# LuZWCHA/MLIC

Hardware: AMD Instinct MI355X
Metric: images/sec (enc+dec) at 1920×1088 MLICPP_L, 1/2/4/8 GPU; bpp/PSNR Δ vs ref (higher is better)
Workload: dtype f32 (dense convs: f32 via split-fp16 MFMA, 3 terms); 1 GPU; config 2: MLICPP_L compress+decompress of 1920x1088 images (full rANS bitstreams, inputs resident in HBM); model=MLICPP_L, global_batch=32, per_gpu_images=32, weights=rate set(s) [1] of synthetic.RATE_LAMBDAS, parallelism=image-sharded x1 (no cross-GPU context), request_streams=4, schedule=each request stream runs its K steps back to back (no per-step join)

## Files before the change

### include/mlic_hip.h

```cpp
#ifndef MLIC_HIP_H
#define MLIC_HIP_H
#include <stddef.h>
#include <stdint.h>

#ifdef __cplusplus
extern "C" {
#endif

typedef struct mlic_model mlic_model;

const char* mlic_last_error(void);
const char* mlic_version(void);

int mlic_create(const char* model_name, int n, const char* const* names, const float* const* ptrs,
                const int64_t* shapes, const int* ndims, void* stream, mlic_model** out);
int mlic_destroy(mlic_model* m);

int mlic_forward(mlic_model* m, void* stream, const float* x, int B, int H, int W, float* x_hat, float* y_lik,
                 float* z_lik, float vbr_scale);
int mlic_forward_v(mlic_model* m, void* stream, const float* x, int B, int H, int W, float* x_hat, float* y_lik,
                   float* z_lik, const float* vbr_scales);

int mlic_set_entropy_tables(mlic_model* m, const int32_t* gc_cdf, const int32_t* gc_len, const int32_t* gc_off,
                            int gc_n, int gc_stride, const int32_t* eb_cdf, const int32_t* eb_len,
                            const int32_t* eb_off, int eb_n, int eb_stride);

int mlic_set_lanes(mlic_model* m, int lanes);
int mlic_set_priority_base(mlic_model* m, int base);
int mlic_compress(mlic_model* m, void* stream, const float* x, int B, int H, int W, float vbr_scale);
int mlic_compress_v(mlic_model* m, void* stream, const float* x, int B, int H, int W, const float* vbr_scales);
int mlic_encoded_size(mlic_model* m, int b, size_t* y_len, size_t* z_len);
int mlic_encoded_copy(mlic_model* m, int b, uint8_t* y, uint8_t* z);
int mlic_encoded_streams(mlic_model* m, int b, int64_t* n_y, int64_t* n_z, int32_t* y_sym, int32_t* y_idx,
                         int32_t* z_sym);
int mlic_encoded_bits(mlic_model* m, int b, double* y_bits, double* z_bits);
int mlic_batch_stream(mlic_model* m, int first, int count, uint8_t* out, size_t cap, size_t* len);
int mlic_decompress_batch_stream(mlic_model* m, void* stream, const uint8_t* y, size_t y_len, const uint8_t* const* z,
                                 const size_t* z_len, int B, int hz, int wz, float* x_hat, const float* vbr_scales);
int mlic_decompress(mlic_model* m, void* stream, const uint8_t* const* y, const size_t* y_len,
                    const uint8_t* const* z, const size_t* z_len, int B, int hz, int wz, float* x_hat,
                    float vbr_scale);
int mlic_decompress_v(mlic_model* m, void* stream, const uint8_t* const* y, const size_t* y_len,
                      const uint8_t* const* z, const size_t* z_len, int B, int hz, int wz, float* x_hat,
                      const float* vbr_scales);

int mlic_layer_streams(mlic_model* m, int b, const uint8_t** ptrs, size_t* lens, int cap, int* n);
int mlic_decompress_prefix(mlic_model* m, void* stream, const uint8_t* const* y, const size_t* y_len,
                           int strings_per_image, const uint8_t* const* z, const size_t* z_len, int B, int hz, int wz,
                           int slices, int fill, const float* vbr_scales, float* x_hat);

int mlic_forward_g(mlic_model* m, void* stream, const float* x, int B, int H, int W, float* x_hat, float* y_lik,
                   float* z_lik, const float* gain_plane);
int mlic_compress_g(mlic_model* m, void* stream, const float* x, int B, int H, int W, const float* gain_plane);
int mlic_decompress_g(mlic_model* m, void* stream, const uint8_t* const* y, const size_t* y_len,
                      const uint8_t* const* z, const size_t* z_len, int B, int hz, int wz, float* x_hat,
                      const float* gain_plane);
int mlic_image_roi_levels_u8(void* stream, const uint8_t* mask, const int64_t* mask_strides, int B, int H, int W, int lo,
                             int hi, uint8_t* levels);
int mlic_roi_gain_plane(void* stream, const uint8_t* levels, int B, int hz, int wz, const float* gains_host,
                        int n_levels, float* g);
int mlic_image_sq_err_roi_u8(void* stream, const uint8_t* a, const int64_t* a_strides, const uint8_t* b,
                             const int64_t* b_strides, const uint8_t* mask, const int64_t* mask_strides, int B, int H,
                             int W, uint64_t* out);

int mlic_rate_map_run(void* stream, const float* y_lik, int64_t y_bs, const float* z_lik, int64_t z_bs, int B, int M,
                      int S, int h, int w, int N, double* y_map, double* z_map, double* cell_bits, double* slice_bits);
int mlic_image_sq_err_blocks_u8(void* stream, const uint8_t* a, const int64_t* a_strides, const uint8_t* b,
                                const int64_t* b_strides, int B, int H, int W, int block, uint32_t* out);
int mlic_image_heat_u8(void* stream, const double* plane, int B, int ph, int pw, int cell, double lo, double hi,
                       int cmap, int H, int W, uint8_t* dst, const int64_t* dst_strides, const uint8_t* under,
                       const int64_t* under_strides, int alpha);

int mlic_run_module(mlic_model* m, void* stream, const char* which, int idx, const float* in0, const float* in1,
                    int B, int Cin, int H, int W, float* out);
int mlic_workspace_bytes(mlic_model* m, size_t* arena, size_t* weights);

int mlic_set_precision(mlic_model* m, int precision);
int mlic_set_synthesis_precision(mlic_model* m, int mode);
int mlic_set_poison(mlic_model* m, int on);
int mlic_set_kernel_option(const char* name, int value);
int mlic_get_kernel_option(const char* name, int* value);
int mlic_ab_families(int* built);
int mlic_range_fallbacks(mlic_model* m, int64_t* forward_full, int64_t* forward_gs, int64_t* decompress_gs,
                         int reset);
int mlic_set_profiling(mlic_model* m, int on);
int mlic_profile_read(mlic_model* m, int cat, int64_t* launches, double* ms, double* flops, double* bytes);
int mlic_profile_layers(mlic_model* m, char* buf, size_t cap, size_t* written);

int mlic_profile_categories(int* n);
int mlic_host_stats(mlic_model* m, double* enc_ms, double* dec_ms, double* wait_ms, int reset);
int mlic_profile_category_name(int cat, char* buf, size_t cap);

int mlic_conv_run(void* stream, int impl, const float* x, const float* w, const float* bias, float* y, int B, int Cin,
                  int Cout, int H, int W, int K, int stride, int epi, const float* aux, const float* res);
int mlic_conv_choice(int B, int Cin, int Cout, int H, int W, int K, int stride, int epi, int* impl);
int mlic_dw_run(void* stream, const float* x, const float* w, const float* bias, float* y, int B, int C, int H, int W,
                int stride, int gelu);
int mlic_dwpw_run(void* stream, const float* x, const float* dww, const float* dwb, const float* w, const float* bias,
                  float* y, int B, int C, int Cout, int H, int W, int epi, const float* res);
int mlic_bench_conv(int impl, int B, int Cin, int Cout, int H, int W, int K, int stride, int epi, int iters,
                    double* ms_per, double* tflops);
int mlic_local_attn_mask(void* stream, float* out, int H, int W);
int mlic_local_attn_run(void* stream, int impl, const float* qkv, const float* rel_table, const int32_t* rel_index,
                        float* out, int C, int H, int W, int B, float scale);
int mlic_local_attn_packed_run(void* stream, const float* qkv, const float* rel_table, const int32_t* rel_index,
                               uint16_t* out, int H, int W, int B, float scale);
int mlic_local_attn_packed_half_run(void* stream, const float* qkv, const float* rel_table, const int32_t* rel_index,
                                    uint16_t* out, int H, int W, int B, float scale, int ckbd);
int mlic_linatt_splits(int HW, int* nsplit);
int mlic_linear_attention_run(void* stream, const float* k, const float* v, const float* q, float* out, float* ctx_out,
                              int B, int heads, int hd, int H, int W, int nsplit, int kmask, int qmask);
int mlic_linatt_pack_run(void* stream, const float* q, const float* ctx, uint16_t* out_halves, int B, int heads, int hd,
                         int H, int W, int K, int qmask);
int mlic_ln_channels_run(void* stream, const float* x, const float* gamma, const float* beta, float* y, int B, int C,
                         int HW);
int mlic_taps_gather_run(void* stream, const float* part, const float* bias, float* out, int B, int H, int W);

typedef struct mlic_quant_desc {
  const float* y;
  int64_t y_bs;
  const float* params;
  int64_t params_bs;
  const float* params_a;
  int64_t params_a_bs;
  float* yh;
  int64_t yh_bs;
  float* lik;
  int64_t lik_bs;
  int32_t* sym;
  int32_t* idx;
  int16_t* sym16;
  uint8_t* idx8;
  int32_t* ovf;
  int32_t nlim;
  int32_t ntable;
  const float* table;
  int32_t phase;
  int32_t vbr;
  const float* sc;
  const float* rs;
  const float* scp;
  const float* rsp;
  int32_t B, C, H, W;
} mlic_quant_desc;
int mlic_quant_phase_run(void* stream, const mlic_quant_desc* d);
int mlic_phase_indexes_run(void* stream, const mlic_quant_desc* d);
int mlic_phase_dequant_run(void* stream, const mlic_quant_desc* d);
int mlic_phase_fill_run(void* stream, const mlic_quant_desc* d);
int mlic_recip_plane_run(void* stream, const float* g, float* r, int64_t n);
int mlic_eb_forward_run(void* stream, const float* z, float* z_hat, float* lik, int32_t* sym, const float* quantiles,
                        const float* m0, const float* m1, const float* m2, const float* m3, const float* m4,
                        const float* b0, const float* b1, const float* b2, const float* b3, const float* b4,
                        const float* f0, const float* f1, const float* f2, const float* f3, int B, int C, int H,
                        int W);
int mlic_eb_dequant_run(void* stream, const int32_t* sym, const float* quantiles, float* z_hat, int B, int C, int H,
                        int W);
int mlic_ckbd_mask_run(void* stream, const float* x, int64_t x_bs, float* y, int64_t y_bs, int B, int C, int H, int W,
                       int keep_anchor);
int mlic_image_sq_err_u8(void* stream, const float* a, const float* b, int B, int64_t n_per, double* out);
int mlic_ms_ssim_scratch_bytes(int B, int C, int H, int W, size_t* bytes);
int mlic_image_ms_ssim_u8(void* stream, const float* a, const int64_t* a_strides, const float* b,
                          const int64_t* b_strides, int B, int C, int H, int W, void* scratch,
                          size_t scratch_bytes, double* out, double* terms);

typedef struct mlic_lpips mlic_lpips;
int mlic_lpips_create(int n, const char* const* names, const float* const* ptrs, const int64_t* shapes,
                      const int* ndims, void* stream, mlic_lpips** out);
int mlic_lpips_destroy(mlic_lpips* h);
int mlic_lpips_set_precision(mlic_lpips* h, int precision);
int mlic_lpips_scratch_bytes(int B, int H, int W, size_t* bytes);
int mlic_image_lpips_u8(mlic_lpips* h, void* stream, const float* a, const int64_t* a_strides, const float* b,
                        const int64_t* b_strides, int B, int H, int W, void* scratch, size_t scratch_bytes,
                        double* out, double* terms);
int mlic_lpips_profile(mlic_lpips* h, int on, double* ms3);
int mlic_lpips_range_fallbacks(mlic_lpips* h, int64_t* count, int reset);

typedef struct mlic_dists mlic_dists;
int mlic_dists_create(int n, const char* const* names, const float* const* ptrs, const int64_t* shapes,
                      const int* ndims, void* stream, mlic_dists** out);
int mlic_dists_destroy(mlic_dists* h);
int mlic_dists_set_precision(mlic_dists* h, int precision);
int mlic_dists_scratch_bytes(int B, int H, int W, size_t* bytes);
int mlic_image_dists_u8(mlic_dists* h, void* stream, const float* a, const int64_t* a_strides, const float* b,
                        const int64_t* b_strides, int B, int H, int W, void* scratch, size_t scratch_bytes,
                        double* out, double* terms);
int mlic_dists_profile(mlic_dists* h, int on, double* ms3);
int mlic_dists_range_fallbacks(mlic_dists* h, int64_t* count, int reset);

int mlic_image_ingest_u8(void* stream, const uint8_t* src, const int64_t* src_strides, int B, int H, int W, float* dst,
                         int Hp, int Wp);
int mlic_image_egress_u8(void* stream, const float* src, const int64_t* src_strides, int B, int H, int W, uint8_t* dst,
                         const int64_t* dst_strides, const uint8_t* ref, const int64_t* ref_strides, uint64_t* sq_err);
int mlic_image_blur3_pad(void* stream, const float* src, const int32_t* src_index, int n, int H, int W, int Hp, int Wp,
                         const float* w9, float* dst);

typedef struct mlic_container_info {
  uint32_t H, W;
  uint32_t hz, wz;
  int32_t level;
  int32_t reserved;
  uint64_t y_off, y_len;
  uint64_t z_off, z_len;
} mlic_container_info;
int mlic_container_bytes(size_t y_len, size_t z_len, int vbr, size_t* bytes);
int mlic_container_write(uint32_t H, uint32_t W, int level, uint32_t hz, uint32_t wz, const uint8_t* y, size_t y_len,
                         const uint8_t* z, size_t z_len, uint8_t* out, size_t cap, size_t* len);
int mlic_container_parse(const uint8_t* data, size_t n, int vbr, int n_levels, uint64_t max_pixels,
                         mlic_container_info* info);

typedef struct mlic_container_roi_info {
  mlic_container_info file;
  uint64_t map_off, map_len;
} mlic_container_roi_info;
int mlic_container_write_roi(uint32_t H, uint32_t W, int level, uint32_t hz, uint32_t wz, const uint8_t* y,
                             size_t y_len, const uint8_t* z, size_t z_len, const uint8_t* levels, uint8_t* out,
                             size_t cap, size_t* len);
int mlic_container_parse_roi(const uint8_t* data, size_t n, int n_levels, uint64_t max_pixels,
                             mlic_container_roi_info* info, uint8_t* levels, size_t levels_cap);

int mlic_tile_grid(uint32_t H, uint32_t W, uint32_t T, uint32_t V, uint32_t* ny, uint32_t* nx, uint32_t* rects,
                   size_t rects_cap);
int mlic_image_tile_blend_u8(void* stream, const float* const* tiles_dev, const float* const* tiles_host, int H, int W,
                             int T, int V, int y0, int x0, int h, int w, uint8_t* dst, const int64_t* dst_strides,
                             const uint8_t* ref, const int64_t* ref_strides, uint64_t* sq_err);
typedef struct mlic_container_tiled_info {
  uint32_t H, W, T, V, ny, nx;
  int32_t vbr;
  int32_t reserved;
  uint64_t table_off, payload_off, payload_len;
} mlic_container_tiled_info;
int mlic_container_write_tiled(uint32_t H, uint32_t W, uint32_t T, uint32_t V, int vbr, const uint8_t* payload,
                               const uint64_t* lens, size_t n_tiles, uint8_t* out, size_t cap, size_t* len);
int mlic_container_parse_tiled(const uint8_t* data, size_t n, uint64_t max_pixels, mlic_container_tiled_info* info);
int mlic_container_tiled_tile(const uint8_t* data, size_t n, const mlic_container_tiled_info* info, uint64_t k,
                              uint64_t* off, uint64_t* len);

int mlic_encode_image_u8(mlic_model* m, void* stream, const uint8_t* rgb_dev, const int64_t* strides, int H, int W,
                         float vbr_scale, int level, uint8_t* out, size_t cap, size_t* len);
int mlic_encode_image_u8_budget(mlic_model* m, void* stream, const uint8_t* rgb_dev, const int64_t* strides, int H,
                                int W, float vbr_scale, int level, double max_bpp, int max_passes, uint8_t* out,
                                size_t cap, size_t* len, int* passes);
int mlic_decode_image_u8(mlic_model* m, void* stream, const uint8_t* file, size_t n, int n_levels, uint64_t max_pixels,
                         const float* vbr_gains, uint8_t* rgb_dev, const int64_t* strides, size_t cap_bytes, int* H,
                         int* W, int* level);

int mlic_resample_table(int filter, int Li, int Lo, int32_t* start, int32_t* count, float* weights, int stride,
                        int* taps);
int mlic_image_ingest_u8_scaled(void* stream, const uint8_t* src, const int64_t* src_strides, int B, int Hi, int Wi,
                                int filter, int h, int w, float* dst, int Hp, int Wp);
int mlic_image_egress_u8_scaled(void* stream, const float* src, const int64_t* src_strides, int B, int h, int w,
                                int filter, int Ho, int Wo, uint8_t* dst, const int64_t* dst_strides, const uint8_t* ref,
                                const int64_t* ref_strides, uint64_t* sq_err);
typedef struct mlic_container_scaled_info {
  uint32_t H, W;
  int32_t filter;
  int32_t vbr;
  uint64_t inner_off, inner_len;
  mlic_container_info inner;
} mlic_container_scaled_info;
int mlic_container_write_scaled(uint32_t H, uint32_t W, int vbr, int filter, const uint8_t* inner, size_t inner_len,
                                uint8_t* out, size_t cap, size_t* len);
int mlic_container_parse_scaled(const uint8_t* data, size_t n, int n_levels, uint64_t max_pixels,
                                mlic_container_scaled_info* info);
typedef struct mlic_container_layered_info {
  uint32_t H, W, hz, wz;
  int32_t level;
  uint32_t S, layers_present;
  uint64_t z_off, z_len;
  uint64_t layer_off[32], layer_len[32];
} mlic_container_layered_info;
int mlic_container_layered_bytes(size_t z_len, const size_t* layer_lens, int S, int vbr, size_t* bytes);
int mlic_container_write_layered(uint32_t H, uint32_t W, int level, uint32_t hz, uint32_t wz, const uint8_t* z,
                                 size_t z_len, const uint8_t* const* layers, const size_t* layer_lens, int S,
                                 uint8_t* out, size_t cap, size_t* len);
int mlic_container_parse_layered(const uint8_t* data, size_t n, int n_levels, uint64_t max_pixels, int allow_truncated,
                                 mlic_container_layered_info* info);
int mlic_encode_image_u8_scaled(mlic_model* m, void* stream, const uint8_t* rgb_dev, const int64_t* strides, int H,
                                int W, int coded_H, int coded_W, int filter, float vbr_scale, int level, uint8_t* out,
                                size_t cap, size_t* len);
int mlic_decode_image_u8_sized(mlic_model* m, void* stream, const uint8_t* file, size_t n, int n_levels,
                               uint64_t max_pixels, const float* vbr_gains, int out_H, int out_W, int filter,
                               uint8_t* rgb_dev, const int64_t* strides, size_t cap_bytes, int* H, int* W, int* level,
                               int* coded_H, int* coded_W);

typedef struct mlic_yuv_desc {
  int32_t sub_x, sub_y;
  int32_t matrix;
  int32_t full_range;
  int32_t site_x;
  int32_t reserved[3];
} mlic_yuv_desc;
int mlic_image_ingest_yuv8(void* stream, const uint8_t* y, const int64_t* y_strides, const uint8_t* cb,
                           const int64_t* cb_strides, const uint8_t* cr, const int64_t* cr_strides,
                           const mlic_yuv_desc* desc, int B, int H, int W, float* dst, int Hp, int Wp);
int mlic_image_egress_yuv8(void* stream, const float* src, const int64_t* src_strides, int B, int H, int W,
                           const mlic_yuv_desc* desc, uint8_t* y, const int64_t* y_strides, uint8_t* cb,
                           const int64_t* cb_strides, uint8_t* cr, const int64_t* cr_strides, const uint8_t* ref_y,
                           const int64_t* ref_y_strides, const uint8_t* ref_cb, const int64_t* ref_cb_strides,
                           const uint8_t* ref_cr, const int64_t* ref_cr_strides, uint64_t* sq_err);
int mlic_encode_image_yuv8(mlic_model* m, void* stream, const uint8_t* y_dev, const int64_t* y_strides,
                           const uint8_t* cb_dev, const int64_t* cb_strides, const uint8_t* cr_dev,
                           const int64_t* cr_strides, const mlic_yuv_desc* desc, int H, int W, float vbr_scale,
                           int level, uint8_t* out, size_t cap, size_t* len);
int mlic_decode_image_yuv8(mlic_model* m, void* stream, const uint8_t* file, size_t n, int n_levels,
                           uint64_t max_pixels, const float* vbr_gains, const mlic_yuv_desc* desc, uint8_t* y_dev,
                           const int64_t* y_strides, size_t y_cap, uint8_t* cb_dev, const int64_t* cb_strides,
                           size_t cb_cap, uint8_t* cr_dev, const int64_t* cr_strides, size_t cr_cap, int* H, int* W,
                           int* level);

int mlic_image_ingest_u16(void* stream, const uint16_t* src, const int64_t* src_strides, int depth, int msb, int B,
                          int H, int W, float* dst, int Hp, int Wp);
int mlic_image_egress_u16(void* stream, const float* src, const int64_t* src_strides, int B, int H, int W, int depth,
                          int msb, uint16_t* dst, const int64_t* dst_strides, const uint16_t* ref,
                          const int64_t* ref_strides, uint64_t* sq_err);
int mlic_image_ingest_yuv16(void* stream, const uint16_t* y, const int64_t* y_strides, const uint16_t* cb,
                            const int64_t* cb_strides, const uint16_t* cr, const int64_t* cr_strides,
                            const mlic_yuv_desc* desc, int depth, int msb, int B, int H, int W, float* dst, int Hp,
                            int Wp);
int mlic_image_egress_yuv16(void* stream, const float* src, const int64_t* src_strides, int B, int H, int W,
                            const mlic_yuv_desc* desc, int depth, int msb, uint16_t* y, const int64_t* y_strides,
                            uint16_t* cb, const int64_t* cb_strides, uint16_t* cr, const int64_t* cr_strides,
                            const uint16_t* ref_y, const int64_t* ref_y_strides, const uint16_t* ref_cb,
                            const int64_t* ref_cb_strides, const uint16_t* ref_cr, const int64_t* ref_cr_strides,
                            uint64_t* sq_err);
int mlic_encode_image_yuv16(mlic_model* m, void* stream, const uint16_t* y_dev, const int64_t* y_strides,
                            const uint16_t* cb_dev, const int64_t* cb_strides, const uint16_t* cr_dev,
                            const int64_t* cr_strides, const mlic_yuv_desc* desc, int depth, int msb, int H, int W,
                            float vbr_scale, int level, uint8_t* out, size_t cap, size_t* len);
int mlic_decode_image_yuv16(mlic_model* m, void* stream, const uint8_t* file, size_t n, int n_levels,
                            uint64_t max_pixels, const float* vbr_gains, const mlic_yuv_desc* desc, int depth, int msb,
                            uint16_t* y_dev, const int64_t* y_strides, size_t y_cap, uint16_t* cb_dev,
                            const int64_t* cb_strides, size_t cb_cap, uint16_t* cr_dev, const int64_t* cr_strides,
                            size_t cr_cap, int* H, int* W, int* level);
int mlic_neglog2_sum(void* stream, const float* lik, int B, int64_t n_per, double* out);
int mlic_gaussian_likelihood(void* stream, const float* y, const float* scales, const float* means, int64_t n,
                             float vbr_scale, float* lik);
int mlic_scale_indexes(void* stream, const float* scales, int64_t n, const float* table, int ntable, int32_t* out);

int mlic_pmf_to_quantized_cdf(const float* pmf, int n, int precision, int32_t* cdf_out );
int mlic_rans_encode(const int32_t* symbols, const int32_t* indexes, int64_t n, const int32_t* cdf,
                     const int32_t* cdf_len, const int32_t* offset, int n_tables, int stride, uint8_t* out,
                     size_t cap, size_t* written);
int mlic_rans_decode(const uint8_t* data, size_t nbytes, const int32_t* indexes, int64_t n, const int32_t* cdf,
                     const int32_t* cdf_len, const int32_t* offset, int n_tables, int stride, int32_t* out);
int mlic_rans_decode_narrow(const uint8_t* data, size_t nbytes, const uint8_t* indexes, int64_t n, int nparts,
                            const int32_t* cdf, const int32_t* cdf_len, const int32_t* offset, int n_tables,
                            int stride, int32_t* out, int* widened);

#ifdef __cplusplus
}
#endif
#endif
```

### mlic_amd/_lib.py

```python
from __future__ import annotations

import ctypes as C
import os
import threading

_HERE = os.path.dirname(os.path.abspath(__file__))
LIB_PATH = os.environ.get("MLIC_HIP_LIB", os.path.join(_HERE, "libmlic_hip.so"))

_lock = threading.Lock()
_lib = None


class MlicError(RuntimeError):
    pass


class ContainerInfo(C.Structure):
    _fields_ = [("H", C.c_uint32), ("W", C.c_uint32), ("hz", C.c_uint32), ("wz", C.c_uint32), ("level", C.c_int32),
                ("reserved", C.c_int32), ("y_off", C.c_uint64), ("y_len", C.c_uint64), ("z_off", C.c_uint64),
                ("z_len", C.c_uint64)]


class ContainerRoiInfo(C.Structure):
    _fields_ = [("file", ContainerInfo), ("map_off", C.c_uint64), ("map_len", C.c_uint64)]


class ContainerTiledInfo(C.Structure):
    _fields_ = [("H", C.c_uint32), ("W", C.c_uint32), ("T", C.c_uint32), ("V", C.c_uint32), ("ny", C.c_uint32),
                ("nx", C.c_uint32), ("vbr", C.c_int32), ("reserved", C.c_int32), ("table_off", C.c_uint64),
                ("payload_off", C.c_uint64), ("payload_len", C.c_uint64)]


class ContainerScaledInfo(C.Structure):
    _fields_ = [("H", C.c_uint32), ("W", C.c_uint32), ("filter", C.c_int32), ("vbr", C.c_int32),
                ("inner_off", C.c_uint64), ("inner_len", C.c_uint64), ("inner", ContainerInfo)]


class ContainerLayeredInfo(C.Structure):
    _fields_ = [("H", C.c_uint32), ("W", C.c_uint32), ("hz", C.c_uint32), ("wz", C.c_uint32), ("level", C.c_int32),
                ("S", C.c_uint32), ("layers_present", C.c_uint32), ("z_off", C.c_uint64), ("z_len", C.c_uint64),
                ("layer_off", C.c_uint64 * 32), ("layer_len", C.c_uint64 * 32)]


class YuvDesc(C.Structure):
    _fields_ = [("sub_x", C.c_int32), ("sub_y", C.c_int32), ("matrix", C.c_int32), ("full_range", C.c_int32),
                ("site_x", C.c_int32), ("reserved", C.c_int32 * 3)]


class QuantDesc(C.Structure):
    _fields_ = [("y", C.c_void_p), ("y_bs", C.c_int64), ("params", C.c_void_p), ("params_bs", C.c_int64),
                ("params_a", C.c_void_p), ("params_a_bs", C.c_int64), ("yh", C.c_void_p), ("yh_bs", C.c_int64),
                ("lik", C.c_void_p), ("lik_bs", C.c_int64), ("sym", C.c_void_p), ("idx", C.c_void_p),
                ("sym16", C.c_void_p), ("idx8", C.c_void_p), ("ovf", C.c_void_p), ("nlim", C.c_int32),
                ("ntable", C.c_int32), ("table", C.c_void_p), ("phase", C.c_int32), ("vbr", C.c_int32),
                ("sc", C.c_void_p), ("rs", C.c_void_p), ("scp", C.c_void_p), ("rsp", C.c_void_p),
                ("B", C.c_int32), ("C", C.c_int32), ("H", C.c_int32), ("W", C.c_int32)]


def _sig(lib):
    p, i, i64, f, sz = C.c_void_p, C.c_int, C.c_int64, C.c_float, C.c_size_t
    P = C.POINTER
    lib.mlic_last_error.restype = C.c_char_p
    lib.mlic_version.restype = C.c_char_p
    sigs = {
        "mlic_create": [C.c_char_p, i, P(C.c_char_p), P(p), P(i64), P(i), p, P(p)],
        "mlic_destroy": [p],
        "mlic_forward": [p, p, p, i, i, i, p, p, p, f],
        "mlic_forward_v": [p, p, p, i, i, i, p, p, p, p],
        "mlic_compress_v": [p, p, p, i, i, i, p],
        "mlic_decompress_v": [p, p, P(p), P(sz), P(p), P(sz), i, i, i, p, p],
        "mlic_set_entropy_tables": [p, p, p, p, i, i, p, p, p, i, i],
        "mlic_compress": [p, p, p, i, i, i, f],
        "mlic_encoded_size": [p, i, P(sz), P(sz)],
        "mlic_encoded_copy": [p, i, p, p],
        "mlic_encoded_streams": [p, i, P(i64), P(i64), p, p, p],
        "mlic_decompress": [p, p, P(p), P(sz), P(p), P(sz), i, i, i, p, f],
        "mlic_run_module": [p, p, C.c_char_p, i, p, p, i, i, i, i, p],
        "mlic_workspace_bytes": [p, P(sz), P(sz)],
        "mlic_local_attn_mask": [p, p, i, i],
        "mlic_set_profiling": [p, i],
        "mlic_set_lanes": [p, i],
        "mlic_set_priority_base": [p, i],
        "mlic_set_precision": [p, i],
        "mlic_set_synthesis_precision": [p, i],
        "mlic_set_poison": [p, i],
        "mlic_set_kernel_option": [C.c_char_p, i],
        "mlic_get_kernel_option": [C.c_char_p, P(i)],
        "mlic_ab_families": [P(i)],
        "mlic_batch_stream": [p, i, i, p, sz, P(sz)],
        "mlic_decompress_batch_stream": [p, p, p, sz, P(p), P(sz), i, i, i, p, p],
        "mlic_range_fallbacks": [p, P(i64), P(i64), P(i64), i],
        "mlic_profile_layers": [p, p, sz, P(sz)],
        "mlic_bench_conv": [i, i, i, i, i, i, i, i, i, i, P(C.c_double), P(C.c_double)],
        "mlic_profile_read": [p, i, P(i64), P(C.c_double), P(C.c_double), P(C.c_double)],
        "mlic_profile_categories": [P(i)],
        "mlic_host_stats": [p, P(C.c_double), P(C.c_double), P(C.c_double), i],
        "mlic_profile_category_name": [i, p, sz],
        "mlic_conv_run": [p, i, p, p, p, p, i, i, i, i, i, i, i, i, p, p],
        "mlic_conv_choice": [i, i, i, i, i, i, i, i, P(i)],
        "mlic_dw_run": [p, p, p, p, p, i, i, i, i, i, i],
        "mlic_dwpw_run": [p, p, p, p, p, p, p, i, i, i, i, i, i, p],
        "mlic_local_attn_run": [p, i, p, p, p, p, i, i, i, i, f],
        "mlic_local_attn_packed_run": [p, p, p, p, p, i, i, i, f],
        "mlic_local_attn_packed_half_run": [p, p, p, p, p, i, i, i, f, i],
        "mlic_linatt_splits": [i, P(i)],
        "mlic_linear_attention_run": [p, p, p, p, p, p, i, i, i, i, i, i, i, i],
        "mlic_linatt_pack_run": [p, p, p, p, i, i, i, i, i, i, i],
        "mlic_ln_channels_run": [p, p, p, p, p, i, i, i],
        "mlic_taps_gather_run": [p, p, p, p, i, i, i],
        "mlic_quant_phase_run": [p, P(QuantDesc)],
        "mlic_phase_indexes_run": [p, P(QuantDesc)],
        "mlic_phase_dequant_run": [p, P(QuantDesc)],
        "mlic_phase_fill_run": [p, P(QuantDesc)],
        "mlic_layer_streams": [p, i, P(p), P(sz), i, P(i)],
        "mlic_decompress_prefix": [p, p, P(p), P(sz), i, P(p), P(sz), i, i, i, i, i, p, p],
        "mlic_container_layered_bytes": [sz, P(sz), i, i, P(sz)],
        "mlic_container_write_layered": [C.c_uint32, C.c_uint32, i, C.c_uint32, C.c_uint32, p, sz, P(p), P(sz), i, p,
                                         sz, P(sz)],
        "mlic_container_parse_layered": [p, sz, i, C.c_uint64, i, P(ContainerLayeredInfo)],
        "mlic_recip_plane_run": [p, p, p, i64],
        "mlic_eb_forward_run": [p] * 20 + [i, i, i, i],
        "mlic_eb_dequant_run": [p, p, p, p, i, i, i, i],
        "mlic_ckbd_mask_run": [p, p, i64, p, i64, i, i, i, i, i],
        "mlic_image_sq_err_u8": [p, p, p, i, i64, p],
        "mlic_ms_ssim_scratch_bytes": [i, i, i, i, P(sz)],
        "mlic_image_ms_ssim_u8": [p, p, P(i64), p, P(i64), i, i, i, i, p, sz, p, p],
        "mlic_lpips_create": [i, P(C.c_char_p), P(p), P(i64), P(i), p, P(p)],
        "mlic_lpips_destroy": [p],
        "mlic_lpips_set_precision": [p, i],
        "mlic_lpips_scratch_bytes": [i, i, i, P(sz)],
        "mlic_image_lpips_u8": [p, p, p, P(i64), p, P(i64), i, i, i, p, sz, p, p],
        "mlic_lpips_range_fallbacks": [p, P(i64), i],
        "mlic_lpips_profile": [p, i, P(C.c_double)],
        "mlic_dists_create": [i, P(C.c_char_p), P(p), P(i64), P(i), p, P(p)],
        "mlic_dists_destroy": [p],
        "mlic_dists_set_precision": [p, i],
        "mlic_dists_scratch_bytes": [i, i, i, P(sz)],
        "mlic_image_dists_u8": [p, p, p, P(i64), p, P(i64), i, i, i, p, sz, p, p],
        "mlic_dists_range_fallbacks": [p, P(i64), i],
        "mlic_dists_profile": [p, i, P(C.c_double)],
        "mlic_image_ingest_u8": [p, p, P(i64), i, i, i, p, i, i],
        "mlic_image_egress_u8": [p, p, P(i64), i, i, i, p, P(i64), p, P(i64), p],
        "mlic_image_blur3_pad": [p, p, p, i, i, i, i, i, p, p],
        "mlic_container_bytes": [sz, sz, i, P(sz)],
        "mlic_container_write": [C.c_uint32, C.c_uint32, i, C.c_uint32, C.c_uint32, p, sz, p, sz, p, sz, P(sz)],
        "mlic_container_parse": [p, sz, i, i, C.c_uint64, P(ContainerInfo)],
        "mlic_forward_g": [p, p, p, i, i, i, p, p, p, p],
        "mlic_compress_g": [p, p, p, i, i, i, p],
        "mlic_decompress_g": [p, p, P(p), P(sz), P(p), P(sz), i, i, i, p, p],
        "mlic_image_roi_levels_u8": [p, p, P(i64), i, i, i, i, i, p],
        "mlic_roi_gain_plane": [p, p, i, i, i, P(f), i, p],
        "mlic_image_sq_err_roi_u8": [p, p, P(i64), p, P(i64), p, P(i64), i, i, i, p],
        "mlic_rate_map_run": [p, p, i64, p, i64, i, i, i, i, i, i, p, p, p, p],
        "mlic_image_sq_err_blocks_u8": [p, p, P(i64), p, P(i64), i, i, i, i, p],
        "mlic_image_heat_u8": [p, p, i, i, i, i, C.c_double, C.c_double, i, i, i, p, P(i64), p, P(i64), i],
        "mlic_container_write_roi": [C.c_uint32, C.c_uint32, i, C.c_uint32, C.c_uint32, p, sz, p, sz, p, p, sz, P(sz)],
        "mlic_container_parse_roi": [p, sz, i, C.c_uint64, P(ContainerRoiInfo), p, sz],
        "mlic_tile_grid": [C.c_uint32, C.c_uint32, C.c_uint32, C.c_uint32, P(C.c_uint32), P(C.c_uint32), p, sz],
        "mlic_image_tile_blend_u8": [p, p, p, i, i, i, i, i, i, i, i, p, P(i64), p, P(i64), p],
        "mlic_container_write_tiled": [C.c_uint32, C.c_uint32, C.c_uint32, C.c_uint32, i, p, p, sz, p, sz, P(sz)],
        "mlic_container_parse_tiled": [p, sz, C.c_uint64, P(ContainerTiledInfo)],
        "mlic_container_tiled_tile": [p, sz, P(ContainerTiledInfo), C.c_uint64, P(C.c_uint64), P(C.c_uint64)],
        "mlic_encode_image_u8": [p, p, p, P(i64), i, i, f, i, p, sz, P(sz)],
        "mlic_encode_image_u8_budget": [p, p, p, P(i64), i, i, f, i, C.c_double, i, p, sz, P(sz), P(i)],
        "mlic_decode_image_u8": [p, p, p, sz, i, C.c_uint64, p, p, P(i64), sz, P(i), P(i), P(i)],
        "mlic_resample_table": [i, i, i, p, p, p, i, P(i)],
        "mlic_image_ingest_u8_scaled": [p, p, P(i64), i, i, i, i, i, i, p, i, i],
        "mlic_image_egress_u8_scaled": [p, p, P(i64), i, i, i, i, i, i, p, P(i64), p, P(i64), p],
        "mlic_container_write_scaled": [C.c_uint32, C.c_uint32, i, i, p, sz, p, sz, P(sz)],
        "mlic_container_parse_scaled": [p, sz, i, C.c_uint64, P(ContainerScaledInfo)],
        "mlic_encode_image_u8_scaled": [p, p, p, P(i64), i, i, i, i, i, f, i, p, sz, P(sz)],
        "mlic_decode_image_u8_sized": [p, p, p, sz, i, C.c_uint64, p, i, i, i, p, P(i64), sz, P(i), P(i), P(i), P(i),
                                       P(i)],
        "mlic_image_ingest_yuv8": [p, p, P(i64), p, P(i64), p, P(i64), P(YuvDesc), i, i, i, p, i, i],
        "mlic_image_egress_yuv8": [p, p, P(i64), i, i, i, P(YuvDesc), p, P(i64), p, P(i64), p, P(i64), p, P(i64), p,
                                   P(i64), p, P(i64), p],
        "mlic_encode_image_yuv8": [p, p, p, P(i64), p, P(i64), p, P(i64), P(YuvDesc), i, i, f, i, p, sz, P(sz)],
        "mlic_decode_image_yuv8": [p, p, p, sz, i, C.c_uint64, p, P(YuvDesc), p, P(i64), sz, p, P(i64), sz, p, P(i64),
                                   sz, P(i), P(i), P(i)],
        "mlic_image_ingest_u16": [p, p, P(i64), i, i, i, i, i, p, i, i],
        "mlic_image_egress_u16": [p, p, P(i64), i, i, i, i, i, p, P(i64), p, P(i64), p],
        "mlic_image_ingest_yuv16": [p, p, P(i64), p, P(i64), p, P(i64), P(YuvDesc), i, i, i, i, i, p, i, i],
        "mlic_image_egress_yuv16": [p, p, P(i64), i, i, i, P(YuvDesc), i, i, p, P(i64), p, P(i64), p, P(i64), p,
                                    P(i64), p, P(i64), p, P(i64), p],
        "mlic_encode_image_yuv16": [p, p, p, P(i64), p, P(i64), p, P(i64), P(YuvDesc), i, i, i, i, f, i, p, sz, P(sz)],
        "mlic_decode_image_yuv16": [p, p, p, sz, i, C.c_uint64, p, P(YuvDesc), i, i, p, P(i64), sz, p, P(i64), sz, p,
                                    P(i64), sz, P(i), P(i), P(i)],
        "mlic_neglog2_sum": [p, p, i, i64, p],
        "mlic_gaussian_likelihood": [p, p, p, p, i64, f, p],
        "mlic_scale_indexes": [p, p, i64, p, i, p],
        "mlic_encoded_bits": [p, i, P(C.c_double), P(C.c_double)],
        "mlic_pmf_to_quantized_cdf": [p, i, i, p],
        "mlic_rans_encode": [p, p, i64, p, p, p, i, i, p, sz, P(sz)],
        "mlic_rans_decode": [p, sz, p, i64, p, p, p, i, i, p],
        "mlic_rans_decode_narrow": [p, sz, p, i64, i, p, p, p, i, i, p, P(i)],
    }
    for name, args in sigs.items():
        fn = getattr(lib, name)
        fn.argtypes = args
        fn.restype = C.c_int
    return lib


def _check_build_record():
    import json
    from . import build as _build
    if os.environ.get("MLIC_HIP_LIB"):
        return
    rec_path = _build.RECORD
    if not os.path.exists(rec_path):
        raise MlicError(f"{rec_path} missing: rebuild with `python -m mlic_amd.build` (records the sources the "
                        f"library was built from)")
    with open(rec_path) as f:
        rec = json.load(f)
    if rec.get("sources_sha256") != _build.source_digest():
        raise MlicError("libmlic_hip.so was built from other sources than the ones in this tree (stale build): "
                        "rebuild with `python -m mlic_amd.build`")


def lib():
    global _lib
    with _lock:
        if _lib is None:
            if not os.path.exists(LIB_PATH):
                raise MlicError(f"libmlic_hip.so not found at {LIB_PATH}: build it with "
                                f"`python -c 'import __graft_entry__ as g; g.build()'` (hipcc, gfx950)")
            _check_build_record()
            _lib = _sig(C.CDLL(LIB_PATH))
    return _lib


def poison() -> bool:
    return os.environ.get("MLIC_POISON", "0") not in ("", "0")


def ab_families() -> bool:
    v = C.c_int()
    call("mlic_ab_families", C.byref(v))
    return bool(v.value)


def check(rc: int, what: str = ""):
    if rc != 0:
        msg = lib().mlic_last_error().decode(errors="replace")
        raise MlicError(f"{what}: {msg}" if what else msg)


def call(name: str, *args):
    check(getattr(lib(), name)(*args), name)
```

### mlic_amd/csrc/capi.cpp

```cpp
#include "../../include/mlic_hip.h"

#include <algorithm>
#include <cmath>
#include <cstring>
#include <string>
#include <vector>

#include "container.h"
#include "model.h"
#include "options.h"
#include "resample_table.h"

using namespace mlic;

struct mlic_model {
  Model* impl;
  float* stage = nullptr;
  size_t stage_bytes = 0;
  float* stage2 = nullptr;
  size_t stage2_bytes = 0;
  int enc_H = 0, enc_W = 0, enc_level = -1;
  int enc_passes = 0;
  int sc_H = 0, sc_W = 0, sc_filter = 0;
};
// ... 368 lines not shown
    *value = opt_get(name);
  });
}

int mlic_set_poison(mlic_model* m, int on) {
  return guard([&] { impl(m).set_poison(on != 0); });
}

int mlic_range_fallbacks(mlic_model* m, int64_t* forward_full, int64_t* forward_gs, int64_t* decompress_gs,
                         int reset) {
  return guard([&] {
    Model::Fallbacks& f = impl(m).fallbacks();
    if (forward_full) *forward_full = f.forward_full.load();
    if (forward_gs) *forward_gs = f.forward_gs.load();
    if (decompress_gs) *decompress_gs = f.decompress_gs.load();
    if (reset) {
      f.forward_full = 0;
      f.forward_gs = 0;
      f.decompress_gs = 0;
    }
  });
}

int mlic_set_synthesis_precision(mlic_model* m, int mode) {
  return guard([&] {
    MLIC_CHECK(mode == 0 || mode == 1, "synthesis precision must be 0 (fp32-faithful) or 1 (fp16 operands)");
    impl(m).set_synthesis_precision(mode);
  });
}

int mlic_set_lanes(mlic_model* m, int lanes) {
  return guard([&] { impl(m).set_lanes(lanes); });
}

int mlic_set_priority_base(mlic_model* m, int base) {
  return guard([&] {
    MLIC_CHECK(base >= 0, "priority base must be >= 0");
    impl(m).set_priority_base(base);
  });
}

int mlic_set_profiling(mlic_model* m, int on) {
  return guard([&] { impl(m).set_profiling(on != 0); });
}

int mlic_profile_read(mlic_model* m, int cat, int64_t* launches, double* ms, double* flops, double* bytes) {
  return guard([&] {
    MLIC_CHECK(cat >= 0 && cat < PCAT_COUNT, "profile category");
    ProfStat s = impl(m).profile_read(cat);
    *launches = s.launches;
    *ms = s.ms;
    *flops = s.flops;
    *bytes = s.bytes;
  });
}

int mlic_profile_layers(mlic_model* m, char* buf, size_t cap, size_t* written) {
  return guard([&] {
    std::string s = impl(m).profile_layers();
    *written = s.size();
    if (buf && cap) {
      const size_t n = std::min(cap - 1, s.size());
      std::memcpy(buf, s.data(), n);
      buf[n] = 0;
    }
  });
}

int mlic_bench_conv(int impl, int B, int Cin, int Cout, int H, int W, int K, int stride, int epi, int iters,
                    double* ms_per, double* tflops) {
  return guard([&] {
    const int pad = K / 2;
    const int Ho = (H + 2 * pad - K) / stride + 1, Wo = (W + 2 * pad - K) / stride + 1;
    const int64_t nx = (int64_t)B * Cin * H * W, ny = (int64_t)B * Cout * Ho * Wo, nw = (int64_t)Cout * Cin * K * K;
    const int cin_pad = (Cin + 31) / 32 * 32;
    const int64_t nh = (int64_t)Cout * K * K * cin_pad;
    float *x, *y, *w, *wp, *bias;
    _Float16 *wh, *wl;
    HIP_OK(hipMalloc(&x, nx * 4));
    HIP_OK(hipMalloc(&y, ny * 4));
    HIP_OK(hipMalloc(&w, nw * 4));
    HIP_OK(hipMalloc(&wp, nw * 4));
    HIP_OK(hipMalloc(&bias, Cout * 4));
    HIP_OK(hipMalloc(&wh, nh * 2));
    HIP_OK(hipMalloc(&wl, nh * 2));
    {
      std::vector<float> hx(std::max(nx, nw));
      uint32_t st = 12345;
      for (auto& v : hx) { st = st * 1664525u + 1013904223u; v = ((st >> 9) * (1.0f / 8388608.0f)) - 0.5f; }
      HIP_OK(hipMemcpy(x, hx.data(), nx * 4, hipMemcpyHostToDevice));
      HIP_OK(hipMemcpy(w, hx.data(), nw * 4, hipMemcpyHostToDevice));
      HIP_OK(hipMemset(bias, 0, Cout * 4));
    }
    pack_conv(w, wp, Cout, Cin, K * K, nullptr);
    const int wexp = split_weights(w, wh, wl, Cout, Cin, K * K, cin_pad, true, nullptr);
    ConvParams P{};
    P.nseg = 1;
    P.seg[0] = {x, Cin, (int64_t)Cin * H * W};
    P.Cin = Cin; P.H = H; P.W = W; P.Cout = Cout; P.Ho = Ho; P.Wo = Wo; P.K = K; P.stride = stride; P.pad = pad;
    P.wpk = wp; P.bias = bias; P.out = y; P.B = B;
    P.out_bs = (int64_t)Cout * Ho * Wo;
    P.out_cs = (int64_t)Ho * Wo;
    P.epi = epi;
    MLIC_CHECK(!(epi & (EPI_GDN | EPI_IGDN | EPI_SHUFFLE)) || !(epi & EPI_RES), "bench: unsupported epilogue");
    if (epi & (EPI_GDN | EPI_IGDN)) {
      MLIC_CHECK(Cin == Cout && stride == 1, "bench: GDN needs Cin == Cout");
      P.aux = x;
      P.aux_bs = (int64_t)Cin * H * W;
    }
    if (epi & EPI_RES) {
      P.res = y;
      P.res_bs = P.out_bs;
    }
    _Float16 *wx = nullptr, *wxh = nullptr;
    if (conv_x4_ok(P, cin_pad)) {
      HIP_OK(hipMalloc((void**)&wx, x4_weight_halves(Cout, K * K, cin_pad) * 2));
      x4_pack_weights(wh, wl, Cout, K * K, cin_pad, wx, nullptr);
      if (impl == CONV_X4H) {
        HIP_OK(hipMalloc((void**)&wxh, x4_weight_halves(Cout, K * K, cin_pad, true) * 2));
        x4_pack_weights(wh, wl, Cout, K * K, cin_pad, wxh, nullptr, true);
      }
    }
    ConvWeights cw{wp, wh, wl, cin_pad, wx, wexp};
    cw.wx4h = wxh;
    const int which = impl < 0 ? conv_select(P, cw, 2) : impl;
    if (which == CONV_X4H) MLIC_CHECK(conv_x4_ok(P, cin_pad), "x4: unsupported shape");
    if (which == CONV_PW) MLIC_CHECK(pw_resident_ok(P, cin_pad), "pw_resident: unsupported shape");
    if (which == CONV_X4) MLIC_CHECK(conv_x4_ok(P, cin_pad), "x4: unsupported shape");
    void* ws = nullptr;
    const int64_t wsb = conv_ws_bytes(which, P, cw);
    if (wsb > 0) HIP_OK(hipMalloc(&ws, wsb));
    auto launch = [&] { conv_run(which, P, cw, nullptr, ws); };
    launch();
    HIP_OK(hipDeviceSynchronize());
    hipEvent_t a, b;
    HIP_OK(hipEventCreate(&a));
    HIP_OK(hipEventCreate(&b));
    HIP_OK(hipEventRecord(a, nullptr));
    for (int i = 0; i < iters; ++i) launch();
    HIP_OK(hipEventRecord(b, nullptr));
    HIP_OK(hipEventSynchronize(b));
    float ms = 0;
    HIP_OK(hipEventElapsedTime(&ms, a, b));
    *ms_per = ms / iters;
    *tflops = 2.0 * (double)B * Cout * Ho * Wo * Cin * K * K / (*ms_per * 1e-3) / 1e12;
    (void)hipEventDestroy(a);
    (void)hipEventDestroy(b);
    for (void* p : {(void*)x, (void*)y, (void*)w, (void*)wp, (void*)bias, (void*)wh, (void*)wl, (void*)wx, (void*)wxh, ws})
      if (p) (void)hipFree(p);
  });
}

int mlic_host_stats(mlic_model* m, double* enc_ms, double* dec_ms, double* wait_ms, int reset) {
  return guard([&] {
    HostStats& h = impl(m).host_stats();
    *enc_ms = h.enc_ns.load() * 1e-6;
    *dec_ms = h.dec_ns.load() * 1e-6;
    *wait_ms = h.wait_ns.load() * 1e-6;
    if (reset) {
      h.enc_ns = 0;
      h.dec_ns = 0;
      h.wait_ns = 0;
    }
  });
}

int mlic_profile_categories(int* n) {
  return guard([&] { *n = PCAT_COUNT; });
}

int mlic_profile_category_name(int cat, char* buf, size_t cap) {
  return guard([&] {
    MLIC_CHECK(cat >= 0 && cat < PCAT_COUNT, "profile category");
    const std::string nm = prof_cat_name(cat);
    MLIC_CHECK(cap > nm.size(), "buffer too small");
    std::memcpy(buf, nm.c_str(), nm.size() + 1);
  });
}

int mlic_conv_choice(int B, int Cin, int Cout, int H, int W, int K, int stride, int epi, int* impl) {
  return guard([&] {
    MLIC_CHECK(impl && B > 0 && Cin > 0 && Cout > 0 && H > 0 && W > 0 && (K == 1 || K == 3 || K == 5) && stride > 0,
               "conv_choice: bad arguments");
    const int pad = K / 2;
    ConvParams P{};
    P.nseg = 1;
    P.seg[0] = {nullptr, Cin, (int64_t)Cin * H * W};
    P.Cin = Cin; P.H = H; P.W = W; P.Cout = Cout; P.K = K; P.stride = stride; P.pad = pad;
    P.Ho = (H + 2 * pad - K) / stride + 1;
    P.Wo = (W + 2 * pad - K) / stride + 1;
    P.B = B;
    P.epi = epi;
    const int cin_pad = (Cin + 31) / 32 * 32;
    static const _Float16 tag = 0;
    const bool split = Cin >= 16;
    const bool x4 = split && Cout >= 64;
    const ConvWeights cw{nullptr, split ? &tag : nullptr, split ? &tag : nullptr, cin_pad, x4 ? &tag : nullptr, 0};
    *impl = conv_select(P, cw, 2);
  });
}

int mlic_conv_run(void* stream, int impl, const float* x, const float* w, const float* bias, float* y, int B, int Cin,
                  int Cout, int H, int W, int K, int stride, int epi, const float* aux, const float* res) {
  return guard([&] {
    hipStream_t st = (hipStream_t)stream;
    const int pad = K / 2;
    const int Ho = (H + 2 * pad - K) / stride + 1, Wo = (W + 2 * pad - K) / stride + 1;
    const int cin_pad = (Cin + 31) / 32 * 32;
    const int64_t nw = (int64_t)Cout * Cin * K * K, nh = (int64_t)Cout * K * K * cin_pad;
    float* wp = nullptr;
    _Float16 *wh = nullptr, *wl = nullptr;
    HIP_OK(hipMallocAsync((void**)&wp, nw * 4, st));
    HIP_OK(hipMallocAsync((void**)&wh, nh * 2, st));
    HIP_OK(hipMallocAsync((void**)&wl, nh * 2, st));
    pack_conv(w, wp, Cout, Cin, K * K, st);
    const int wexp = split_weights(w, wh, wl, Cout, Cin, K * K, cin_pad, true, st);
    ConvParams P{};
    P.nseg = 1;
    P.seg[0] = {x, Cin, (int64_t)Cin * H * W};
    P.Cin = Cin; P.H = H; P.W = W; P.Cout = Cout; P.Ho = Ho; P.Wo = Wo; P.K = K; P.stride = stride; P.pad = pad;
    P.wpk = wp; P.bias = bias; P.out = y; P.B = B; P.epi = epi;
    const bool shuffle = (epi & EPI_SHUFFLE) != 0;
    MLIC_CHECK(!shuffle || Cout % 4 == 0, "shuffle needs Cout % 4 == 0");
    P.out_cs = shuffle ? (int64_t)4 * Ho * Wo : (int64_t)Ho * Wo;
    P.out_bs = (int64_t)Cout * Ho * Wo;
    MLIC_CHECK(!(epi & (EPI_GDN | EPI_IGDN)) || aux, "GDN epilogue needs aux");
    MLIC_CHECK(!(epi & EPI_RES) || res, "residual epilogue needs res");
    P.aux = aux; P.aux_bs = (int64_t)Cout * Ho * Wo;
    P.res = res; P.res_bs = P.out_bs;
    _Float16 *wx = nullptr, *wxh = nullptr;
    if (conv_x4_ok(P, cin_pad)) {
      HIP_OK(hipMallocAsync((void**)&wx, x4_weight_halves(Cout, K * K, cin_pad) * 2, st));
      x4_pack_weights(wh, wl, Cout, K * K, cin_pad, wx, st);
      if (impl == CONV_X4H) {
        HIP_OK(hipMallocAsync((void**)&wxh, x4_weight_halves(Cout, K * K, cin_pad, true) * 2, st));
        x4_pack_weights(wh, wl, Cout, K * K, cin_pad, wxh, st, true);
      }
    }
    ConvWeights cw{wp, wh, wl, cin_pad, wx, wexp};
    cw.wx4h = wxh;
    const int which = impl < 0 ? conv_select(P, cw, 2) : impl;
    if (which == CONV_X4H) MLIC_CHECK(conv_x4_ok(P, cin_pad), "x4: unsupported shape");
    if (which == CONV_PW) MLIC_CHECK(pw_resident_ok(P, cin_pad), "pw_resident: unsupported shape");
    if (which == CONV_NARROW) MLIC_CHECK(conv_narrow_ok(P), "narrow: unsupported shape");
    if (which == CONV_SMALLCIN) MLIC_CHECK(conv_smallcin_ok(P), "smallcin: unsupported shape");
    if (which == CONV_HALO) MLIC_CHECK(conv_halo_ok(P, cin_pad), "halo: unsupported shape");
    if (which == CONV_X4) MLIC_CHECK(conv_x4_ok(P, cin_pad), "x4: unsupported shape");
    void* ws = nullptr;
    const int64_t wsb = conv_ws_bytes(which, P, cw);
    if (wsb > 0) HIP_OK(hipMallocAsync(&ws, wsb, st));
    conv_run(which, P, cw, st, ws);
    if (ws) HIP_OK(hipFreeAsync(ws, st));
    if (wx) HIP_OK(hipFreeAsync(wx, st));
    if (wxh) HIP_OK(hipFreeAsync(wxh, st));
    HIP_OK(hipFreeAsync(wp, st));
    HIP_OK(hipFreeAsync(wh, st));
    HIP_OK(hipFreeAsync(wl, st));
    HIP_OK(hipStreamSynchronize(st));
  });
}

int mlic_dw_run(void* stream, const float* x, const float* w, const float* bias, float* y, int B, int C, int H, int W,
                int stride, int gelu) {
  return guard([&] {
    DwParams P{};
    P.nseg = 1;
    P.seg[0] = {x, C, (int64_t)C * H * W};
    P.C = C; P.H = H; P.W = W; P.stride = stride;
    P.Ho = (H - 1) / stride + 1;
    P.Wo = (W - 1) / stride + 1;
    P.w = w; P.bias = bias; P.out = y; P.out_bs = (int64_t)C * P.Ho * P.Wo; P.gelu = gelu; P.B = B;
    dw3x3(P, (hipStream_t)stream);
    HIP_OK(hipStreamSynchronize((hipStream_t)stream));
  });
}

int mlic_dwpw_run(void* stream, const float* x, const float* dww, const float* dwb, const float* w, const float* bias,
                  float* y, int B, int C, int Cout, int H, int W, int epi, const float* res) {
  return guard([&] {
    hipStream_t st = (hipStream_t)stream;
    const int cin_pad = (C + 31) / 32 * 32;
    const int64_t nh = (int64_t)Cout * cin_pad;
    _Float16 *wh = nullptr, *wl = nullptr;
    HIP_OK(hipMallocAsync((void**)&wh, nh * 2, st));
    HIP_OK(hipMallocAsync((void**)&wl, nh * 2, st));
    const int wexp = split_weights(w, wh, wl, Cout, C, 1, cin_pad, true, st);
    ConvParams P{};
    P.nseg = 1;
    P.seg[0] = {x, C, (int64_t)C * H * W};
    P.Cin = C; P.H = H; P.W = W; P.Cout = Cout; P.Ho = H; P.Wo = W; P.K = 1; P.stride = 1; P.pad = 0;
    P.wexp = wexp; P.bias = bias; P.out = y; P.B = B; P.epi = epi;
    P.out_cs = (int64_t)H * W;
    P.out_bs = (int64_t)Cout * H * W;
    MLIC_CHECK(!(epi & EPI_RES) || res, "residual epilogue needs res");
    P.res = res; P.res_bs = P.out_bs;
    MLIC_CHECK(dwpw_ok(P, cin_pad), "dwpw: unsupported shape");
    dwpw_forward(P, wh, wl, cin_pad, dww, dwb, st);
    HIP_OK(hipFreeAsync(wh, st));
    HIP_OK(hipFreeAsync(wl, st));
    HIP_OK(hipStreamSynchronize(st));
  });
}

int mlic_local_attn_run(void* stream, int impl, const float* qkv, const float* rel_table, const int32_t* rel_index,
                        float* out, int C, int H, int W, int B, float scale) {
  return guard([&] {
    LocalAttnParams A{};
    A.qkv = qkv;
    A.qkv_bs = (int64_t)3 * C * H * W;
    A.out = out;
    A.out_bs = (int64_t)25 * C * H * W;
    A.rel_table = rel_table;
    A.rel_index = rel_index;
    A.scale = scale;
    A.C = C; A.H = H; A.W = W; A.B = B;
    if (impl == 0) local_attn_valu(A, (hipStream_t)stream);
    else local_attn_mfma(A, (hipStream_t)stream);
    HIP_OK(hipStreamSynchronize((hipStream_t)stream));
  });
}

int mlic_local_attn_packed_run(void* stream, const float* qkv, const float* rel_table, const int32_t* rel_index,
                               uint16_t* out, int H, int W, int B, float scale) {
  return guard([&] {
    LocalAttnParams A{};
    A.qkv = qkv;
    A.qkv_bs = (int64_t)3 * 32 * H * W;
    A.rel_table = rel_table;
    A.rel_index = rel_index;
    A.scale = scale;
    A.C = 32; A.H = H; A.W = W; A.B = B;
    local_attn_packed(A, reinterpret_cast<_Float16*>(out), (H * W + 31) / 32 * 32, (hipStream_t)stream);
    HIP_OK(hipStreamSynchronize((hipStream_t)stream));
  });
}

int mlic_local_attn_packed_half_run(void* stream, const float* qkv, const float* rel_table, const int32_t* rel_index,
                                    uint16_t* out, int H, int W, int B, float scale, int ckbd) {
  return guard([&] {
    MLIC_CHECK(ckbd == 1 || ckbd == 2, "ckbd: 1 (anchors) or 2 (non-anchors)");
    LocalAttnParams A{};
    A.qkv = qkv;
    A.qkv_bs = (int64_t)3 * 32 * H * W;
    A.rel_table = rel_table;
    A.rel_index = rel_index;
    A.scale = scale;
    A.C = 32; A.H = H; A.W = W; A.B = B;
    A.ckbd = ckbd;
    local_attn_packed(A, reinterpret_cast<_Float16*>(out), (H * W / 2 + 31) / 32 * 32, (hipStream_t)stream);
    HIP_OK(hipStreamSynchronize((hipStream_t)stream));
  });
}

static void check_grid(int B, int H, int W, int rows) {
  MLIC_CHECK(B >= 1 && B <= 65535, "B must be in 1..65535");
  MLIC_CHECK(H >= 1 && W >= 1 && (int64_t)H * W <= (int64_t)1 << 30, "H, W must be >= 1 and H * W <= 2^30");
  MLIC_CHECK(rows >= 1 && (int64_t)rows * B <= 65535, "too many (image, head) rows for one launch");
}

int mlic_linatt_splits(int HW, int* nsplit) {
  return guard([&] {
    MLIC_CHECK(nsplit != nullptr, "null nsplit");
    MLIC_CHECK(HW >= 1, "HW must be >= 1");
    *nsplit = ctx_splits(HW);
  });
}

int mlic_linear_attention_run(void* stream, const float* k, const float* v, const float* q, float* out, float* ctx_out,
                              int B, int heads, int hd, int H, int W, int nsplit, int kmask, int qmask) {
  return guard([&] {
    MLIC_CHECK(k && v && q && out, "null tensor");
    MLIC_CHECK(hd == 16 || hd == 32, "hd must be 16 or 32");
    MLIC_CHECK(heads >= 1, "heads must be >= 1");
    check_grid(B, H, W, heads);
    MLIC_CHECK(nsplit <= 64, "nsplit must be <= 64 (<= 0: the model's choice)");
    MLIC_CHECK((kmask == 0 || kmask == 1) && (qmask == 0 || qmask == 1), "kmask, qmask must be 0 or 1");
    hipStream_t st = (hipStream_t)stream;
    const int HW = H * W;
    const int ns = nsplit <= 0 ? ctx_splits(HW) : nsplit;
    const int64_t bs = (int64_t)heads * hd * HW, nctx = (int64_t)B * heads * hd * hd;
    float *part = nullptr, *ctx = nullptr;
    HIP_OK(hipMallocAsync((void**)&part, linear_attention_part_floats(heads, hd, B, ns) * 4, st));
    HIP_OK(hipMallocAsync((void**)&ctx, nctx * 4, st));
    linear_attention(k, bs, v, bs, q, bs, out, bs, part, ctx, heads, hd, H, W, B, ns, kmask, qmask, st);
    if (ctx_out) HIP_OK(hipMemcpyAsync(ctx_out, ctx, nctx * 4, hipMemcpyDeviceToDevice, st));
    HIP_OK(hipFreeAsync(part, st));
    HIP_OK(hipFreeAsync(ctx, st));
    HIP_OK(hipStreamSynchronize(st));
  });
}

int mlic_linatt_pack_run(void* stream, const float* q, const float* ctx, uint16_t* out_halves, int B, int heads, int hd,
                         int H, int W, int K, int qmask) {
  return guard([&] {
    MLIC_CHECK(q && ctx && out_halves, "null tensor");
    MLIC_CHECK(hd == 16 || hd == 32, "hd must be 16 or 32");
    MLIC_CHECK(heads >= 1 && (heads * (int64_t)hd) % 32 == 0, "heads * hd must be a multiple of 32");
    MLIC_CHECK(K == 3 || K == 5, "K must be 3 or 5");
    check_grid(B, H, W, heads * hd / 32);
    check_grid(B, H + K - 1, W + K - 1, 1);
    MLIC_CHECK(qmask == 0 || qmask == 1, "qmask must be 0 or 1");
    ConvParams P{};
    P.nseg = 1;
    P.seg[0] = {nullptr, heads * hd, (int64_t)heads * hd * H * W};
    P.Cin = heads * hd; P.H = H; P.W = W; P.Cout = P.Cin; P.Ho = H; P.Wo = W; P.K = K; P.stride = 1; P.pad = K / 2;
    P.B = B;
    P.rflag = nullptr;
    linatt_pack(q, P.seg[0].bs, ctx, heads, hd, qmask, P, reinterpret_cast<_Float16*>(out_halves), (hipStream_t)stream);
    HIP_OK(hipStreamSynchronize((hipStream_t)stream));
  });
}

int mlic_ln_channels_run(void* stream, const float* x, const float* gamma, const float* beta, float* y, int B, int C,
                         int HW) {
  return guard([&] {
    MLIC_CHECK(x && gamma && beta && y, "null tensor");
    MLIC_CHECK(C == 32 || C == 64 || C == 128, "C must be 32, 64 or 128");
    check_grid(B, 1, HW, 1);
    ln_channels(x, (int64_t)C * HW, y, (int64_t)C * HW, gamma, beta, C, HW, B, (hipStream_t)stream);
    HIP_OK(hipStreamSynchronize((hipStream_t)stream));
  });
}

int mlic_taps_gather_run(void* stream, const float* part, const float* bias, float* out, int B, int H, int W) {
  return guard([&] {
    MLIC_CHECK(part && out, "null tensor");
    check_grid(B, H, W, 1);
    MLIC_CHECK((H + 3) / 4 <= 65535, "H too large for one launch");
    taps_gather(part, (int64_t)108 * H * W, bias, out, (int64_t)12 * H * W, H, W, B, (hipStream_t)stream);
    HIP_OK(hipStreamSynchronize((hipStream_t)stream));
  });
}

static QuantParams quant_params(const mlic_quant_desc* d) {
  MLIC_CHECK(d != nullptr, "null descriptor");
  MLIC_CHECK(d->params && d->table, "null tensor");
  check_grid(d->B, d->H, d->W, 1);
  MLIC_CHECK(d->C >= 1 && (int64_t)d->C * d->H * d->W <= (int64_t)1 << 30, "C must be >= 1 and C * H * W <= 2^30");
  MLIC_CHECK(d->W % 2 == 0, "W must be even");
  MLIC_CHECK(d->phase == 0 || d->phase == 1, "phase must be 0 (anchor) or 1 (non-anchor)");
  MLIC_CHECK(d->ntable >= 2 && d->ntable <= 256, "ntable must be in 2..256");
  MLIC_CHECK(d->vbr == 0 || d->vbr == 1, "vbr must be 0 or 1");
  MLIC_CHECK(d->vbr || (!d->scp && !d->rsp), "gain planes need vbr");
  const int64_t n = (int64_t)d->C * d->H * d->W;
  MLIC_CHECK(d->params_bs >= 2 * n, "params_bs smaller than [2C][H][W]");
  QuantParams Q{};
  Q.y = d->y; Q.y_bs = d->y_bs;
  Q.params = d->params; Q.params_bs = d->params_bs;
  Q.params_a = d->params_a; Q.params_a_bs = d->params_a_bs;
  Q.yh = d->yh; Q.yh_bs = d->yh_bs;
  Q.lik = d->lik; Q.lik_bs = d->lik_bs;
  Q.sym = d->sym; Q.idx = d->idx;
  Q.sym16 = d->sym16; Q.idx8 = d->idx8; Q.ovf = d->ovf;
  Q.nlim = d->nlim;
  Q.table = d->table; Q.ntable = d->ntable;
  Q.phase = d->phase; Q.vbr = d->vbr;
  Q.sc = d->sc; Q.rs = d->rs;
  Q.C = d->C; Q.H = d->H; Q.W = d->W; Q.B = d->B;
  Q.scp = d->scp; Q.rsp = d->rsp;
  return Q;
}

int mlic_quant_phase_run(void* stream, const mlic_quant_desc* d) {
  return guard([&] {
    const QuantParams Q = quant_params(d);
    const int64_t n = (int64_t)Q.C * Q.H * Q.W;
    MLIC_CHECK(Q.y && Q.yh, "null tensor");
    MLIC_CHECK(Q.y_bs >= n, "y_bs smaller than [C][H][W]");
    MLIC_CHECK(Q.yh_bs >= n, "yh_bs smaller than [C][H][W]");
    MLIC_CHECK(!Q.lik || Q.params_a, "lik needs params_a");
    MLIC_CHECK(!Q.lik || Q.lik_bs >= n, "lik_bs smaller than [C][H][W]");
    MLIC_CHECK(!Q.params_a || Q.params_a_bs >= 2 * n, "params_a_bs smaller than [2C][H][W]");
    MLIC_CHECK(!Q.sym16 || (Q.idx8 && Q.ovf), "sym16 needs idx8 and ovf");
    MLIC_CHECK(Q.sym16 || (!Q.idx8 && !Q.ovf), "idx8 and ovf need sym16");
    MLIC_CHECK(!Q.idx || Q.sym || Q.sym16, "idx needs sym or sym16");
    MLIC_CHECK((Q.scp != nullptr) == (Q.rsp != nullptr), "scp and rsp: both or neither");
    MLIC_CHECK(!Q.vbr || Q.scp || (Q.sc && Q.rs), "vbr needs sc and rs, or gain planes");
    MLIC_CHECK(Q.nlim >= 1 && Q.nlim <= 32767, "nlim must be in 1..32767");
    quant_phase(Q, (hipStream_t)stream);
    HIP_OK(hipStreamSynchronize((hipStream_t)stream));
  });
}

int mlic_phase_indexes_run(void* stream, const mlic_quant_desc* d) {
  return guard([&] {
    const QuantParams Q = quant_params(d);
    MLIC_CHECK(Q.idx8 || Q.idx, "null output: idx8 or idx");
    MLIC_CHECK(!Q.vbr || Q.scp || Q.sc, "vbr needs sc, or the gain plane scp");
    phase_indexes(Q, (hipStream_t)stream);
    HIP_OK(hipStreamSynchronize((hipStream_t)stream));
  });
}

int mlic_phase_dequant_run(void* stream, const mlic_quant_desc* d) {
  return guard([&] {
    const QuantParams Q = quant_params(d);
    const int64_t n = (int64_t)Q.C * Q.H * Q.W;
    MLIC_CHECK(Q.yh, "null tensor");
    MLIC_CHECK(Q.yh_bs >= n, "yh_bs smaller than [C][H][W]");
    MLIC_CHECK(Q.sym16 || Q.sym, "null input: sym16 or sym");
    MLIC_CHECK(!Q.vbr || Q.rsp || Q.rs, "vbr needs rs, or the reciprocal plane rsp");
    phase_dequant(Q, (hipStream_t)stream);
    HIP_OK(hipStreamSynchronize((hipStream_t)stream));
  });
}

int mlic_phase_fill_run(void* stream, const mlic_quant_desc* d) {
  return guard([&] {
    const QuantParams Q = quant_params(d);
    const int64_t n = (int64_t)Q.C * Q.H * Q.W;
    MLIC_CHECK(Q.yh, "null tensor");
    MLIC_CHECK(Q.yh_bs >= n, "yh_bs smaller than [C][H][W]");
    phase_fill(Q, (hipStream_t)stream);
    HIP_OK(hipStreamSynchronize((hipStream_t)stream));
  });
}

int mlic_recip_plane_run(void* stream, const float* g, float* r, int64_t n) {
  return guard([&] {
    MLIC_CHECK(g && r, "null tensor");
    MLIC_CHECK(n >= 1 && n <= (int64_t)1 << 31, "n must be in 1..2^31");
    recip_plane(g, r, n, (hipStream_t)stream);
    HIP_OK(hipStreamSynchronize((hipStream_t)stream));
  });
}

static void check_eb_grid(int B, int C, int H, int W) {
  check_grid(B, H, W, 1);
  MLIC_CHECK(C >= 1 && (int64_t)B * C * H * W <= (int64_t)1 << 31, "C must be >= 1 and B * C * H * W <= 2^31");
}

int mlic_eb_forward_run(void* stream, const float* z, float* z_hat, float* lik, int32_t* sym, const float* quantiles,
                        const float* m0, const float* m1, const float* m2, const float* m3, const float* m4,
                        const float* b0, const float* b1, const float* b2, const float* b3, const float* b4,
                        const float* f0, const float* f1, const float* f2, const float* f3, int B, int C, int H,
                        int W) {
  return guard([&] {
    MLIC_CHECK(z && quantiles, "null tensor");
    MLIC_CHECK(m0 && m1 && m2 && m3 && m4 && b0 && b1 && b2 && b3 && b4 && f0 && f1 && f2 && f3, "null parameter");
    MLIC_CHECK(z_hat || lik || sym, "null outputs: at least one of z_hat, lik, sym");
    check_eb_grid(B, C, H, W);
    EbParams P{};
    P.z = z; P.z_hat = z_hat; P.lik = lik; P.sym = sym;
    P.quantiles = quantiles;
    P.m0 = m0; P.m1 = m1; P.m2 = m2; P.m3 = m3; P.m4 = m4;
    P.b0 = b0; P.b1 = b1; P.b2 = b2; P.b3 = b3; P.b4 = b4;
    P.f0 = f0; P.f1 = f1; P.f2 = f2; P.f3 = f3;
    P.C = C; P.H = H; P.W = W; P.B = B;
    eb_forward(P, (hipStream_t)stream);
    HIP_OK(hipStreamSynchronize((hipStream_t)stream));
  });
}

int mlic_eb_dequant_run(void* stream, const int32_t* sym, const float* quantiles, float* z_hat, int B, int C, int H,
                        int W) {
  return guard([&] {
    MLIC_CHECK(sym && quantiles && z_hat, "null tensor");
    check_eb_grid(B, C, H, W);
    eb_dequant(sym, quantiles, z_hat, C, H * W, B, (hipStream_t)stream);
    HIP_OK(hipStreamSynchronize((hipStream_t)stream));
  });
}

int mlic_ckbd_mask_run(void* stream, const float* x, int64_t x_bs, float* y, int64_t y_bs, int B, int C, int H, int W,
                       int keep_anchor) {
  return guard([&] {
    MLIC_CHECK(x && y, "null tensor");
    check_grid(B, H, W, 1);
    MLIC_CHECK(C >= 1 && (int64_t)C * H * W <= (int64_t)1 << 30, "C must be >= 1 and C * H * W <= 2^30");
    MLIC_CHECK(keep_anchor == 0 || keep_anchor == 1, "keep_anchor must be 0 or 1");
    MLIC_CHECK(x_bs >= (int64_t)C * H * W, "x_bs smaller than [C][H][W]");
    MLIC_CHECK(y_bs >= (int64_t)C * H * W, "y_bs smaller than [C][H][W]");
    ckbd_mask(x, x_bs, y, y_bs, C, H, W, B, keep_anchor, (hipStream_t)stream);
    HIP_OK(hipStreamSynchronize((hipStream_t)stream));
  });
}

int mlic_local_attn_mask(void* stream, float* out, int H, int W) {
  return guard([&] { local_mask(out, H, W, (hipStream_t)stream); });
}

int mlic_image_sq_err_u8(void* stream, const float* a, const float* b, int B, int64_t n_per, double* out) {
  return guard([&] { sq_err_u8(a, n_per, b, n_per, out, n_per, B, (hipStream_t)stream); });
}

int mlic_ms_ssim_scratch_bytes(int B, int C, int H, int W, size_t* bytes) {
  return guard([&] {
    MLIC_CHECK(bytes != nullptr, "ms_ssim_scratch_bytes: null bytes");
    *bytes = ms_ssim_scratch_bytes(B, C, H, W);
  });
}

int mlic_image_ms_ssim_u8(void* stream, const float* a, const int64_t* a_strides, const float* b,
                          const int64_t* b_strides, int B, int C, int H, int W, void* scratch,
                          size_t scratch_bytes, double* out, double* terms) {
  return guard([&] {
    const size_t need = ms_ssim_scratch_bytes(B, C, H, W);
    MLIC_CHECK(a && b && a_strides && b_strides && out, "ms_ssim: null argument");
    MLIC_CHECK(scratch != nullptr && scratch_bytes >= need, "ms_ssim: scratch too small (mlic_ms_ssim_scratch_bytes)");
    MLIC_CHECK(reinterpret_cast<uintptr_t>(scratch) % 8 == 0, "ms_ssim: scratch must be 8-byte aligned");
    ms_ssim_u8(a, a_strides, b, b_strides, B, C, H, W, scratch, out, terms, (hipStream_t)stream);
  });
}

int mlic_lpips_create(int n, const char* const* names, const float* const* ptrs, const int64_t* shapes,
                      const int* ndims, void* stream, mlic_lpips** out) {
// ... 887 lines not shown
```

### mlic_amd/csrc/common.h

```cpp
#pragma once
#include <hip/hip_runtime.h>

#include <atomic>
#include <cstdint>
#include <cstdio>
#include <stdexcept>
#include <string>

namespace mlic {

struct Error : std::runtime_error {
  using std::runtime_error::runtime_error;
};

#define MLIC_CHECK(cond, msg)                                                                  \
  do {                                                                                          \
    if (!(cond)) throw ::mlic::Error(std::string("mlic: ") + (msg) + " [" #cond "] at " +       \
                                     __FILE__ + ":" + std::to_string(__LINE__));               \
  } while (0)

#define HIP_OK(expr)                                                                            \
  do {                                                                                          \
    hipError_t _e = (expr);                                                                     \
    if (_e != hipSuccess)                                                                       \
      throw ::mlic::Error(std::string("hip: ") + hipGetErrorString(_e) + " in " #expr " at " + \
                          __FILE__ + ":" + std::to_string(__LINE__));                           \
  } while (0)

struct View {
  float* p = nullptr;
  int C = 0, H = 0, W = 0;
  int64_t bs = 0;
  int64_t hw() const { return (int64_t)H * W; }
  View ch(int c0, int nc) const {
    View v = *this;
    v.p = p + (int64_t)c0 * hw();
    v.C = nc;
    return v;
  }
};

enum Epi : int {
  EPI_NONE = 0,
  EPI_GELU = 1,
  EPI_GDN = 2,
  EPI_IGDN = 4,
  EPI_TANH_HALF = 8,
  EPI_MASK_ANCHOR = 16,
  EPI_MASK_NONANCHOR = 32,
  EPI_RES = 64,
  EPI_SHUFFLE = 128,
  EPI_SQUARE_IN = 256,
  EPI_RELU_IN = 512,
};

constexpr int MAXSEG = 6;

struct Seg {
  const float* p;
  int C;
  int64_t bs;
};

struct ConvParams {
  Seg seg[MAXSEG];
  int nseg;
  int Cin, H, W;
  int Cout, Ho, Wo;
  int K, stride, pad;
  const float* wpk;
  int wexp;
  const float* bias;
  float* out;
  int64_t out_bs;
  int64_t out_cs;
  int epi;
  const float* aux;
  int64_t aux_bs;
  const float* res;
  int64_t res_bs;
  int B;
  int* rflag;
  int in_mask;
  int scatter;
  const float* skx;
  int64_t skx_bs;
  int sk_cin, sk_H, sk_W;
  const float* skw;
  const float* skb;
};

__device__ __forceinline__ float softmax_exp(float x) { return __builtin_amdgcn_exp2f(x * 1.44269504088896341f); }

template <int HD>
__device__ __forceinline__ void query_softmax(const float* qp, int HW, float (&q)[HD]) {
  float mx = -3.0e38f;
#pragma unroll
  for (int c = 0; c < HD; ++c) {
    q[c] = qp[(int64_t)c * HW];
    mx = fmaxf(mx, q[c]);
  }
  float sum = 0.0f;
#pragma unroll
  for (int c = 0; c < HD; ++c) {
    q[c] = softmax_exp(q[c] - mx);
    sum += q[c];
  }
  const float inv = 1.0f / sum;
#pragma unroll
  for (int c = 0; c < HD; ++c) q[c] *= inv;
}

__device__ __forceinline__ bool f16_unsafe(float v) { return (__float_as_uint(v) & 0x7fffffffu) >= 0x477ff000u; }
__device__ __forceinline__ void range_report(int* flag, bool bad) {
  if (bad && flag) atomicOr(flag, 1);
}
__device__ __forceinline__ float gelu_erf(float x) {
  const float ax = __builtin_fabsf(x);
  const float z = ax * 0.70710678118654752440f;
  const float t = __builtin_amdgcn_rcpf(__builtin_fmaf(0.3275911f, z, 1.0f));
  float q = __builtin_fmaf(0.5307027101516724f, t, -0.726576030254364f);
  q = __builtin_fmaf(q, t, 0.710706889629364f);
  q = __builtin_fmaf(q, t, -0.14224836230278015f);
  q = __builtin_fmaf(q, t, 0.1274147927761078f);
  q = q * t;
  const float e = __builtin_amdgcn_exp2f(z * (z * -1.44269504088896341f));
  return __builtin_fmaxf(x, 0.0f) - ax * (q * e);
}
typedef float mlic_float2 __attribute__((ext_vector_type(2)));
__device__ __forceinline__ mlic_float2 gelu_erf2(mlic_float2 x) {
  const mlic_float2 ax = {__builtin_fabsf(x.x), __builtin_fabsf(x.y)};
  const mlic_float2 z = ax * 0.70710678118654752440f;
  const mlic_float2 d = __builtin_elementwise_fma(mlic_float2{0.3275911f, 0.3275911f}, z, mlic_float2{1.0f, 1.0f});
  const mlic_float2 t = {__builtin_amdgcn_rcpf(d.x), __builtin_amdgcn_rcpf(d.y)};
  mlic_float2 q = __builtin_elementwise_fma(mlic_float2{0.5307027101516724f, 0.5307027101516724f}, t,
                                            mlic_float2{-0.726576030254364f, -0.726576030254364f});
  q = __builtin_elementwise_fma(q, t, mlic_float2{0.710706889629364f, 0.710706889629364f});
  q = __builtin_elementwise_fma(q, t, mlic_float2{-0.14224836230278015f, -0.14224836230278015f});
  q = __builtin_elementwise_fma(q, t, mlic_float2{0.1274147927761078f, 0.1274147927761078f});
  q = q * t;
  const mlic_float2 zz = z * (z * -1.44269504088896341f);
  const mlic_float2 e = {__builtin_amdgcn_exp2f(zz.x), __builtin_amdgcn_exp2f(zz.y)};
  const mlic_float2 m = {__builtin_fmaxf(x.x, 0.0f), __builtin_fmaxf(x.y, 0.0f)};
  return m - ax * (q * e);
}
__device__ __forceinline__ float gelu_erff(float x) { return 0.5f * x * (1.0f + erff(x * 0.70710678118654752440f)); }
__device__ __forceinline__ float gelu_epi(float x) {
#ifndef MLIC_GELU_EPI_ERFF
  return gelu_erf(x);
#else
  return gelu_erff(x);
#endif
}

__device__ __forceinline__ float gdn_apply(float x, float v, bool inverse) {
  return inverse ? x * __builtin_amdgcn_sqrtf(v) : x * __builtin_amdgcn_rsqf(v);
}

__device__ __forceinline__ bool is_anchor(int h, int w) { return ((h + w) & 1) == 1; }

__device__ __forceinline__ void conv_store(const ConvParams& P, int b, int co, int p, float v) {
  const int epi = P.epi;
  const int HWo = P.Ho * P.Wo;
  v = ldexpf(v, -P.wexp);
  if (P.bias) v += P.bias[co];
  if (epi & EPI_GELU) v = gelu_epi(v);
  if (epi & (EPI_GDN | EPI_IGDN)) {
    const float x = P.aux[(int64_t)b * P.aux_bs + (int64_t)co * HWo + p];
    v = gdn_apply(x, v, (epi & EPI_GDN) == 0);
  }
  if (epi & EPI_TANH_HALF) v = 0.5f * tanhf(v);
  int oh = 0, ow = 0;
  if (epi & (EPI_MASK_ANCHOR | EPI_MASK_NONANCHOR | EPI_SHUFFLE)) {
    oh = p / P.Wo;
    ow = p - oh * P.Wo;
  }
  if (epi & EPI_MASK_ANCHOR) v = is_anchor(oh, ow) ? v : 0.0f;
  if (epi & EPI_MASK_NONANCHOR) v = is_anchor(oh, ow) ? 0.0f : v;
  int64_t off;
  if (epi & EPI_SHUFFLE) {
    const int oc = co >> 2;
    const int y2 = 2 * oh + ((co >> 1) & 1), x2 = 2 * ow + (co & 1);
    off = (int64_t)oc * P.out_cs + (int64_t)y2 * (2 * P.Wo) + x2;
  } else {
    off = (int64_t)co * P.out_cs + p;
  }
  if (epi & EPI_RES) v = P.res[(int64_t)b * P.res_bs + off] + v;
  P.out[(int64_t)b * P.out_bs + off] = v;
}

__host__ __device__ __forceinline__ bool conv_vec_ok(const ConvParams& P) {
  const uintptr_t a = reinterpret_cast<uintptr_t>(P.out) | reinterpret_cast<uintptr_t>(P.aux) |
                      reinterpret_cast<uintptr_t>(P.res);
  return (a & 15) == 0 && ((P.out_bs | P.out_cs | P.aux_bs | P.res_bs) & 3) == 0 && (P.Wo & 3) == 0;
}

__device__ __forceinline__ void conv_store4(const ConvParams& P, int b, int co, int p, float4 v) {
  const int epi = P.epi;
  float a[4] = {v.x, v.y, v.z, v.w};
  const float bi = P.bias ? P.bias[co] : 0.0f;
#pragma unroll
  for (int e = 0; e < 4; ++e) {
    a[e] = ldexpf(a[e], -P.wexp) + bi;
    if (epi & EPI_GELU) a[e] = gelu_epi(a[e]);
  }
  if (epi & (EPI_GDN | EPI_IGDN)) {
    const float4 x = *reinterpret_cast<const float4*>(P.aux + (int64_t)b * P.aux_bs + (int64_t)co * P.Ho * P.Wo + p);
    const float xs[4] = {x.x, x.y, x.z, x.w};
#pragma unroll
    for (int e = 0; e < 4; ++e) a[e] = gdn_apply(xs[e], a[e], (epi & EPI_GDN) == 0);
  }
  if (epi & EPI_TANH_HALF) {
#pragma unroll
    for (int e = 0; e < 4; ++e) a[e] = 0.5f * tanhf(a[e]);
  }
  if (epi & (EPI_MASK_ANCHOR | EPI_MASK_NONANCHOR)) {
    const int oh = p / P.Wo, ow = p - oh * P.Wo;
#pragma unroll
    for (int e = 0; e < 4; ++e) {
      const bool anc = is_anchor(oh, ow + e);
      if ((epi & EPI_MASK_ANCHOR) && !anc) a[e] = 0.0f;
      if ((epi & EPI_MASK_NONANCHOR) && anc) a[e] = 0.0f;
    }
  }
  const int64_t off = (int64_t)co * P.out_cs + p;
  if (epi & EPI_RES) {
    const float4 r = *reinterpret_cast<const float4*>(P.res + (int64_t)b * P.res_bs + off);
    a[0] = r.x + a[0]; a[1] = r.y + a[1]; a[2] = r.z + a[2]; a[3] = r.w + a[3];
  }
  *reinterpret_cast<float4*>(P.out + (int64_t)b * P.out_bs + off) = make_float4(a[0], a[1], a[2], a[3]);
}

__device__ __forceinline__ void conv_store_shuf4(const ConvParams& P, int b, int co0, int p, float4 v) {
  const int epi = P.epi;
  float a[4] = {v.x, v.y, v.z, v.w};
  const float b0 = P.bias ? P.bias[co0] : 0.0f, b1 = P.bias ? P.bias[co0 + 1] : 0.0f;
  a[0] = ldexpf(a[0], -P.wexp) + b0; a[1] = ldexpf(a[1], -P.wexp) + b1;
  a[2] = ldexpf(a[2], -P.wexp) + b0; a[3] = ldexpf(a[3], -P.wexp) + b1;
#pragma unroll
  for (int e = 0; e < 4; ++e) {
    if (epi & EPI_GELU) a[e] = gelu_epi(a[e]);
    if (epi & EPI_TANH_HALF) a[e] = 0.5f * tanhf(a[e]);
  }
  const int oh = p / P.Wo, ow = p - oh * P.Wo;
  const int64_t off = (int64_t)(co0 >> 2) * P.out_cs + (int64_t)(2 * oh + ((co0 >> 1) & 1)) * (2 * P.Wo) + 2 * ow;
  if (epi & EPI_RES) {
    const float4 r = *reinterpret_cast<const float4*>(P.res + (int64_t)b * P.res_bs + off);
    a[0] = r.x + a[0]; a[1] = r.y + a[1]; a[2] = r.z + a[2]; a[3] = r.w + a[3];
  }
  *reinterpret_cast<float4*>(P.out + (int64_t)b * P.out_bs + off) = make_float4(a[0], a[1], a[2], a[3]);
}

inline int device_cu_count() {
  static std::atomic<int> cache[64];
  int dev = 0;
  HIP_OK(hipGetDevice(&dev));
  MLIC_CHECK(dev >= 0 && dev < 64, "device id");
  int n = cache[dev].load(std::memory_order_relaxed);
  if (n == 0) {
    HIP_OK(hipDeviceGetAttribute(&n, hipDeviceAttributeMultiprocessorCount, dev));
    cache[dev].store(n, std::memory_order_relaxed);
  }
  return n;
}

}
```

### mlic_amd/csrc/conv_dwpw.hip

```cpp
#include "common.h"
#include "kernels.h"

#include <type_traits>

namespace mlic {

namespace {
typedef float floatx16 __attribute__((ext_vector_type(16)));
typedef _Float16 half8 __attribute__((ext_vector_type(8)));
typedef unsigned int u32x4 __attribute__((ext_vector_type(4)));
typedef unsigned int u32x2 __attribute__((ext_vector_type(2)));

constexpr int DR_DWP = 12;
constexpr uint32_t DR_OOB = 0x80000000u;

__device__ __forceinline__ __amdgpu_buffer_rsrc_t dr_rsrc(const float* base, uint32_t bytes) {
  const uint64_t a = reinterpret_cast<uint64_t>(base);
  const uint32_t lo = __builtin_amdgcn_readfirstlane((uint32_t)a);
  const uint32_t hi = __builtin_amdgcn_readfirstlane((uint32_t)(a >> 32));
  float* pb = reinterpret_cast<float*>(((uint64_t)hi << 32) | lo);
  return __builtin_amdgcn_make_buffer_rsrc(pb, 0, bytes, 0x00020000);
}

__device__ __forceinline__ void dr_opaque(uint32_t& v) { asm volatile("" : "+s"(v)); }
// ... 28 lines not shown
  constexpr int KS = CIN / 16;
  constexpr int ROWS = CT * 32;
  constexpr int TAPB = CIN * DR_DWP * 4 + ROWS * 4;
  constexpr int LDS = TAPB + KS * ROWS * 64;
  static_assert(CIN % 16 == 0 && LDS <= 160 * 1024, "dwpw: LDS");
  __shared__ __attribute__((aligned(16))) char sm[LDS];
  float* sdw = reinterpret_cast<float*>(sm);
  float* sbias = sdw + CIN * DR_DWP;
  char* sa = sm + TAPB;

  const int tid = threadIdx.x;
  {
    constexpr int NG = KS * ROWS * 4;
    constexpr int NIT = (NG + DP_THREADS - 1) / DP_THREADS;
    u32x4 st[NIT];
#pragma unroll
    for (int it = 0; it < NIT; ++it) {
      const int id = tid + it * DP_THREADS;
      const int q = id & 3, row = (id >> 2) % ROWS, j = (id >> 2) / ROWS;
      st[it] = u32x4{0u, 0u, 0u, 0u};
      if (id < NG && row < P.Cout)
        st[it] = *reinterpret_cast<const u32x4*>((q < 2 ? wh : wl) + (int64_t)row * cin_pad + 16 * j + 8 * (q & 1));
    }
#pragma unroll
    for (int it = 0; it < NIT; ++it) {
      const int id = tid + it * DP_THREADS;
      const int q = id & 3, row = (id >> 2) % ROWS, j = (id >> 2) / ROWS;
      if (id < NG) *reinterpret_cast<u32x4*>(sa + (j * ROWS + row) * 64 + ((q ^ dr_swz(row)) << 4)) = st[it];
    }
  }
  for (int i = tid; i < CIN * DR_DWP; i += DP_THREADS) {
    const int c = i / DR_DWP, k = i - c * DR_DWP;
    sdw[i] = k < 9 ? dww[c * 9 + k] : (k == 9 && dwb ? dwb[c] : 0.0f);
  }
  for (int r = tid; r < ROWS; r += DP_THREADS) sbias[r] = (P.bias && r < P.Cout) ? P.bias[r] : 0.0f;
  __syncthreads();

  const int lane = tid & 63;
  const int wave = __builtin_amdgcn_readfirstlane(tid >> 6);
  const int n = lane & 31, h = lane >> 5;
  const int H = P.H, W = P.W, HW = H * W;
  const int nseg = (W + DP_SEG - 1) / DP_SEG;
  const int nyb = (H + DP_WAVES - 1) / DP_WAVES;
  const int tpi = nseg * nyb;
  const int ntiles = tpi * P.B;
  const int xcd = (int)blockIdx.x & 7, nslot = (int)gridDim.x >> 3;
  const int t_end = (int)((int64_t)(xcd + 1) * ntiles / 8);
  int tile = (int)((int64_t)xcd * ntiles / 8) + ((int)blockIdx.x >> 3);
  if (tile >= t_end) return;

  const uint32_t hw4 = (uint32_t)HW * 4u;
  const uint32_t img_bytes = (uint32_t)CIN * hw4;
  const float* xbase = P.seg[0].p;
  const int64_t xbs = P.seg[0].bs;

  struct Seg2 {
    __amdgpu_buffer_rsrc_t rs;
    uint32_t vo[3];
  };
  auto seg_of = [&](int t) {
    Seg2 s;
    const int b = t / tpi;
    const int r = t - b * tpi;
    const int yb = r / nseg;
    const int y = yb * DP_WAVES + wave;
    const int xl = (r - yb * nseg) * DP_SEG - 2 + 2 * n;
    s.rs = dr_rsrc(xbase + (int64_t)b * xbs, img_bytes);
    const uint32_t ch = (uint32_t)(8 * h) * hw4;
#pragma unroll
    for (int dy = 0; dy < 3; ++dy) {
      const int yy = y + dy - 1;
      s.vo[dy] = yy >= 0 && yy < H && xl >= 0 && xl < W ? (uint32_t)(yy * W + xl) * 4u + ch : DR_OOB;
    }
    if (MLIC_DPABL & 16) s.vo[0] = s.vo[2] = s.vo[1];
    return s;
  };
  auto load_ks = [&](float2v (&r)[8][3], const Seg2& s, uint32_t so) {
#pragma unroll
    for (int i = 0; i < 8; ++i) {
#pragma unroll
      for (int dy = 0; dy < 3; ++dy)
        r[i][dy] = __builtin_bit_cast(float2v, __builtin_amdgcn_raw_buffer_load_b64(s.rs, s.vo[dy], so, 0));
      so += hw4;
      dr_opaque(so);
    }
  };

  uint32_t tapo = 8 * h * DR_DWP;
  uint32_t abo = n * 64;
  auto dw_channel = [&](float2v (&rk)[3], int j, int i, const Seg2& s, uint32_t so) {
    const float4* tq = reinterpret_cast<const float4*>(sdw + tapo + (16 * j + i) * DR_DWP);
    const float4 w0 = tq[0], w1 = tq[1];
    const float2 w2 = *reinterpret_cast<const float2*>(tq + 2);
    const float tw[10] = {w0.x, w0.y, w0.z, w0.w, w1.x, w1.y, w1.z, w1.w, w2.x, w2.y};
    float a0 = 0.0f, a1 = 0.0f;
#pragma unroll
    for (int dy = 0; dy < 3; ++dy) {
      const float p0 = rk[dy].x, p1 = rk[dy].y;
      a0 = fmaf(tw[3 * dy + 0], wave_nb<DPP_WAVE_SHR1>(p1), a0);
      a0 = fmaf(tw[3 * dy + 1], p0, a0);
      a0 = fmaf(tw[3 * dy + 2], p1, a0);
      a1 = fmaf(tw[3 * dy + 0], p0, a1);
      a1 = fmaf(tw[3 * dy + 1], p1, a1);
      a1 = fmaf(tw[3 * dy + 2], wave_nb<DPP_WAVE_SHL1>(p0), a1);
    }
    float2v v = float2v{a0 + tw[9], a1 + tw[9]};
    if (MLIC_DPABL & 2) v = rk[1];
    __builtin_amdgcn_sched_barrier(0);
#pragma unroll
    for (int dy = 0; dy < 3; ++dy)
      rk[dy] = __builtin_bit_cast(float2v, __builtin_amdgcn_raw_buffer_load_b64(s.rs, s.vo[dy], so, 0));
    return v;
  };
  auto dw_pair = [&](float2v (&r0)[3], float2v (&r1)[3], int j, int i, half8 (&bh)[2], half8 (&bl)[2], const Seg2& s,
                     uint32_t so) {
    uint32_t so1 = so + hw4;
    dr_opaque(so1);
    const float2v c0 = dw_channel(r0, j, i, s, so);
    const float2v c1 = dw_channel(r1, j, i + 1, s, so1);
#pragma unroll
    for (int e = 0; e < 2; ++e) {
      const float2v v = {c0[e], c1[e]};
      const half2v hv = __builtin_convertvector(v, half2v);
      const half2v lv = __builtin_convertvector(v - __builtin_convertvector(hv, float2v), half2v);
      bh[e][i] = hv[0];
      bh[e][i + 1] = hv[1];
      bl[e][i] = lv[0];
      bl[e][i + 1] = lv[1];
    }
  };

  float2v ring[8][3];
  Seg2 cur = seg_of(tile);
  int nt = tile + nslot < t_end ? tile + nslot : tile;
  Seg2 nxt = seg_of(nt);
  load_ks(ring, cur, 0);
  half8 bh[2], bl[2];
#pragma unroll
  for (int i = 0; i < 8; i += 2)
    dw_pair(ring[i], ring[i + 1], 0, i, bh, bl, KS > 1 ? cur : nxt, (uint32_t)(KS > 1 ? 16 + i : i) * hw4);

  const int swz = dr_swz(n);
  const int gh = (h ^ swz) << 4, gl = ((2 + h) ^ swz) << 4;
  bool bad = false;
  floatx16 acc[CT][2];
  auto kstep = [&](int j, auto first) {
    const int j1 = (j + 1) % KS, j2 = j + 2;
    const Seg2& s2 = j2 < KS ? cur : nxt;
    const uint32_t so2 = (uint32_t)(16 * (j2 < KS ? j2 : j2 - KS)) * hw4;
    half8 nbh[2], nbl[2];
    if (MLIC_DPABL & 8) __builtin_amdgcn_s_barrier();
    asm volatile("" : "+v"(tapo), "+v"(abo));
    const char* ab = sa + abo + j * ROWS * 64;
    constexpr int NM = MLIC_DPABL & 1 ? 1 : CT * 6;
#pragma unroll
    for (int i = 0; i < 8; i += 2) {
      dw_pair(ring[i], ring[i + 1], j1, i, nbh, nbl, s2, so2 + (uint32_t)i * hw4);
#pragma unroll
      for (int t = (i / 2) * NM / 4; t < (i / 2 + 1) * NM / 4; ++t) {
        const int c = (MLIC_DPABL & 1) ? 0 : t / 6, r = t % 6, e = r & 1;
        const half8 av = *reinterpret_cast<const half8*>(ab + c * 32 * 64 + (r < 2 ? gl : gh));
        half8 bv = r >= 2 && r < 4 ? bl[e] : bh[e];
        if (MLIC_DPABL & 1) bv = bh[0] + bl[0] + bh[1] + bl[1];
        const bool zero = decltype(first)::value && r < 2;
        acc[c][e] = __builtin_amdgcn_mfma_f32_32x32x16_f16(av, bv, zero ? floatx16{} : acc[c][e], 0, 0, 0);
      }
    }
#pragma unroll
    for (int e = 0; e < 2; ++e) {
      bh[e] = nbh[e];
      bl[e] = nbl[e];
    }
  };
  for (;;) {
    kstep(0, std::true_type{});
    if constexpr (MODE == 0 && !RES && !MLIC_DWPW_ROLLED_ALL) {
#pragma unroll
      for (int j = 1; j < KS; ++j) kstep(j, std::false_type{});
    } else {
#pragma nounroll
      for (int j = 1; j < KS; ++j) kstep(j, std::false_type{});
    }

    {
      const int b = tile / tpi;
      const int r = tile - b * tpi;
      const int yb = r / nseg;
      const int y = yb * DP_WAVES + wave;
      const int xl = (r - yb * nseg) * DP_SEG - 2 + 2 * n;
      if (n >= 1 && n <= 30 && xl < W && y < H) {
        const uint32_t cs4 = (uint32_t)P.out_cs * 4u;
        const uint32_t vo_out = (uint32_t)(y * W + xl) * 4u + (uint32_t)(4 * h) * cs4;
        const auto rs_out = dr_rsrc(P.out + (int64_t)b * P.out_bs, (uint32_t)P.Cout * cs4);
        const auto rs_res = dr_rsrc(RES ? P.res + (int64_t)b * P.res_bs : P.out, RES ? (uint32_t)P.Cout * cs4 : 0u);
        const float* sb = sbias + 4 * h;
        const float unscale = ldexpf(1.0f, -P.wexp);
        bool keep[2] = {true, true};
        if (MODE == 4 && (P.epi & (EPI_MASK_ANCHOR | EPI_MASK_NONANCHOR))) {
#pragma unroll
          for (int e = 0; e < 2; ++e) keep[e] = is_anchor(y, xl + e) == ((P.epi & EPI_MASK_ANCHOR) != 0);
        }
        uint32_t so_o = 0;
#pragma unroll
        for (int c = 0; c < CT; ++c) {
          float2v xr[16];
          uint32_t oo = so_o;
#pragma unroll
          for (int q = 0; q < 16; ++q) {
            if (q > 0) {
              oo += (((q & 3) == 0) ? 5u : 1u) * cs4;
              dr_opaque(oo);
            }
            xr[q] = RES ? __builtin_bit_cast(float2v, __builtin_amdgcn_raw_buffer_load_b64(rs_res, vo_out, oo, 0))
                        : float2v{0.0f, 0.0f};
          }
          float4 bq[4];
#pragma unroll
          for (int g = 0; g < 4; ++g) bq[g] = *reinterpret_cast<const float4*>(sb + c * 32 + 8 * g);
          oo = so_o;
          float2v vv[16];
#pragma unroll
          for (int q = 0; q < 16; ++q) {
            const float4 b4 = bq[q >> 2];
            const float bv = (q & 3) == 0 ? b4.x : (q & 3) == 1 ? b4.y : (q & 3) == 2 ? b4.z : b4.w;
            float2v t = __builtin_elementwise_fma(float2v{acc[c][0][q], acc[c][1][q]}, float2v{unscale, unscale},
                                                  float2v{bv, bv});
            if constexpr (MODE == 1) t = gelu_erf2(t);
            if constexpr (MODE == 4) {
#pragma unroll
              for (int e = 0; e < 2; ++e) t[e] = keep[e] ? 0.5f * tanhf(t[e]) : 0.0f;
            }
            vv[q] = t + xr[q];
          }
          float2v sum = vv[0];
#pragma unroll
          for (int q = 1; q < 16; ++q) sum += vv[q];
          bad |= !(fabsf(sum.x) <= 3.4e38f) || !(fabsf(sum.y) <= 3.4e38f);
          if (MLIC_DPABL & 4) {
#pragma unroll
            for (int q = 0; q < 16; ++q) asm volatile("" ::"v"(vv[q][0]), "v"(vv[q][1]));
          } else if (c * 32 + 32 <= P.Cout) {
#pragma unroll
            for (int q = 0; q < 16; ++q) {
              if (q > 0) {
                oo += (((q & 3) == 0) ? 5u : 1u) * cs4;
                dr_opaque(oo);
              }
              __builtin_amdgcn_raw_buffer_store_b64(__builtin_bit_cast(u32x2, vv[q]), rs_out, vo_out, oo, 0);
            }
          } else {
#pragma unroll
            for (int q = 0; q < 16; ++q) {
              if (q > 0) {
                oo += (((q & 3) == 0) ? 5u : 1u) * cs4;
                dr_opaque(oo);
              }
              if (c * 32 + (q & 3) + 8 * (q >> 2) + 4 * h < P.Cout)
                __builtin_amdgcn_raw_buffer_store_b64(__builtin_bit_cast(u32x2, vv[q]), rs_out, vo_out, oo, 0);
            }
          }
          so_o += 32 * cs4;
          dr_opaque(so_o);
        }
      }
    }
    if (nt == tile) break;
    tile = nt;
    cur = nxt;
    nt = tile + nslot < t_end ? tile + nslot : tile;
    nxt = seg_of(nt);
  }
  range_report(P.rflag, bad);
}

static int dr_num_cus() { return device_cu_count(); }

static int dw_mode(const ConvParams& P) {
  const int e = P.epi & ~EPI_RES;
  if (e == EPI_NONE) return 0;
  if (e == EPI_GELU) return 1;
  if (e == EPI_TANH_HALF || e == (EPI_TANH_HALF | EPI_MASK_ANCHOR) || e == (EPI_TANH_HALF | EPI_MASK_NONANCHOR))
    return 4;
  return -1;
}

#define DR_ALL(X, CIN, CT) X(CIN, CT, 0, 0) X(CIN, CT, 0, 1) X(CIN, CT, 1, 0) X(CIN, CT, 1, 1)
#if MLIC_AB_BUILD
#define DR_EQ(X) DR_ALL(X, 192, 6) DR_ALL(X, 160, 5) DR_ALL(X, 128, 4) DR_ALL(X, 96, 3)
#else
#define DR_EQ(X)
#endif
#define DR_COMBOS(X) DR_EQ(X) DR_ALL(X, 48, 2) X(224, 4, 1, 0) X(128, 1, 4, 1) X(192, 4, 1, 0)

bool dwpw_grid_ok(const ConvParams& P) { return (int64_t)P.H * P.W >= 16384; }

bool dwpw_ok(const ConvParams& P, int cin_pad) {
  if (P.K != 1 || P.stride != 1 || P.pad != 0 || P.nseg != 1 || P.seg[0].C != P.Cin || cin_pad < P.Cin) return false;
  const int mode = dw_mode(P);
  if (mode < 0) return false;
  if (P.Ho != P.H || P.Wo != P.W || P.out_cs != (int64_t)P.H * P.W || (P.W % 2) != 0) return false;
  const int64_t HW = (int64_t)P.H * P.W;
  if ((int64_t)P.Cin * HW * 4 >= (1ll << 31) || (int64_t)P.Cout * HW * 4 >= (1ll << 31)) return false;
  if (dwpw2_ok(P, cin_pad)) return true;
  const int ct = (P.Cout + 31) / 32, res = (P.epi & EPI_RES) ? 1 : 0;
#define DR_OK(CIN, CT, M, R) \
  if (P.Cin == CIN && ct == CT && mode == M && res == R) return true;
  DR_COMBOS(DR_OK)
#undef DR_OK
  return false;
}

template <int CIN, int CT, int M, bool R>
static void launch_dwpw(const ConvParams& P, const _Float16* wh, const _Float16* wl, int cin_pad, const float* dww,
                        const float* dwb, hipStream_t st) {
  const int64_t want = (int64_t)((P.W + DP_SEG - 1) / DP_SEG) * ((P.H + DP_WAVES - 1) / DP_WAVES) * P.B;
  const int64_t g = std::min<int64_t>(want, (int64_t)dr_num_cus());
  const dim3 grid((unsigned)((g + 7) / 8 * 8));
  hipLaunchKernelGGL((dwpw_kernel<CIN, CT, M, R>), grid, dim3(DP_THREADS), 0, st, P, wh, wl, cin_pad, dww, dwb);
  HIP_OK(hipGetLastError());
}

void dwpw_forward(const ConvParams& P, const _Float16* wh, const _Float16* wl, int cin_pad, const float* dww,
                  const float* dwb, hipStream_t st) {
  MLIC_CHECK(dwpw_ok(P, cin_pad) && dww, "dwpw: unsupported shape");
  if (dwb && dwpw2_ok(P, cin_pad)) return dwpw2_forward(P, wh, wl, cin_pad, dww, dwb, st);
  const int ct = (P.Cout + 31) / 32, mode = dw_mode(P), res = (P.epi & EPI_RES) ? 1 : 0;
#define DR_RUN(CIN, CT, M, R)                                        \
  if (P.Cin == CIN && ct == CT && mode == M && res == R) {           \
    launch_dwpw<CIN, CT, M, R != 0>(P, wh, wl, cin_pad, dww, dwb, st); \
    return;                                                          \
  }
  DR_COMBOS(DR_RUN)
#undef DR_RUN
  throw Error("mlic: dwpw_kernel for this shape is an A/B-only instantiation (the dwpw2 option's form 0: make AB=1)");
}

}
```

### mlic_amd/csrc/conv_dwpw3.hip

```cpp
#include "common.h"
#include "kernels.h"


namespace mlic {

namespace {
typedef float floatx16 __attribute__((ext_vector_type(16)));
typedef _Float16 half8 __attribute__((ext_vector_type(8)));
typedef _Float16 half2v __attribute__((ext_vector_type(2)));
typedef float float2v __attribute__((ext_vector_type(2)));

constexpr int D3_TC = 64;
constexpr int D3_G = 8;

#ifndef MLIC_D3_FAKETAPS
#define MLIC_D3_FAKETAPS 0
#endif
#ifndef MLIC_D3_ABL
#define MLIC_D3_ABL 0
#endif
#ifndef MLIC_D3_ASYNC
#define MLIC_D3_ASYNC 0
#endif
#ifndef MLIC_D3_NBUF
#define MLIC_D3_NBUF (MLIC_D3_ASYNC ? 3 : 2)
#endif
#ifndef MLIC_D3_PK
#define MLIC_D3_PK 1
#endif
#ifndef MLIC_D3_PPK
#define MLIC_D3_PPK 0
#endif
#ifndef MLIC_D3_TPF
#define MLIC_D3_TPF 0
#endif
#ifndef MLIC_D3_TG
#define MLIC_D3_TG (MLIC_D3_TPF ? 2 : 4)
#endif
constexpr int D3_TG = MLIC_D3_TG;

__device__ __forceinline__ __amdgpu_buffer_rsrc_t d3_rsrc(const float* base, uint32_t bytes) {
  const uint64_t a = reinterpret_cast<uint64_t>(base);
  const uint32_t lo = __builtin_amdgcn_readfirstlane((uint32_t)a);
  const uint32_t hi = __builtin_amdgcn_readfirstlane((uint32_t)(a >> 32));
  return __builtin_amdgcn_make_buffer_rsrc(reinterpret_cast<float*>(((uint64_t)hi << 32) | lo), 0, bytes, 0x00020000);
}

__device__ __forceinline__ void d3_barrier() { asm volatile("s_waitcnt lgkmcnt(0)\n\ts_barrier" ::: "memory"); }

__device__ __forceinline__ void d3_signal(uint32_t* ctr) {
  asm volatile("s_waitcnt lgkmcnt(0)" ::: "memory");
  __hip_atomic_fetch_add(ctr, 1u, __ATOMIC_RELAXED, __HIP_MEMORY_SCOPE_WORKGROUP);
}
__device__ __forceinline__ bool d3_wait_geq(const uint32_t* ctr, uint32_t target) {
  uint32_t spins = 0;
  for (;;) {
    const uint32_t v = __builtin_amdgcn_readfirstlane(__hip_atomic_load(ctr, __ATOMIC_RELAXED, __HIP_MEMORY_SCOPE_WORKGROUP));
    if (v >= target) break;
    __builtin_amdgcn_s_sleep(1);
    if (++spins > (1u << 22)) return false;
  }
  asm volatile("" ::: "memory");
  return true;
}

__device__ __forceinline__ uint32_t d3_aoff(int n, int g) { return (uint32_t)(n * 32 + ((g ^ ((n >> 3) & 1)) << 4)); }

template <int K>
__device__ __forceinline__ void d3_neighbours(float e, float v, float& L, float& R) {
  const int ei = __builtin_bit_cast(int, e), vi = __builtin_bit_cast(int, v);
  int el = ei, er = ei;
  if constexpr (K > 0) {
    el = __builtin_amdgcn_mov_dpp(ei, 0x100 + K, 0xF, 0xF, true);
    er = __builtin_amdgcn_mov_dpp(ei, 0x110 + K, 0xF, 0xF, true);
  }
  L = __builtin_bit_cast(float, __builtin_amdgcn_update_dpp(el, vi, 0x138, 0xF, 0xF, false));
  R = __builtin_bit_cast(float, __builtin_amdgcn_update_dpp(er, vi, 0x130, 0xF, 0xF, false));
}
__device__ __forceinline__ void d3_neighbours_k(int k, float e, float v, float& L, float& R) {
  switch (k) {
#define D3_NB(K) \
  case K: return d3_neighbours<K>(e, v, L, R);
    D3_NB(0) D3_NB(1) D3_NB(2) D3_NB(3) D3_NB(4) D3_NB(5) D3_NB(6) D3_NB(7)
    D3_NB(8) D3_NB(9) D3_NB(10) D3_NB(11) D3_NB(12) D3_NB(13) D3_NB(14) D3_NB(15)
#undef D3_NB
  }
}
}

template <int N, int MODE, bool RES, bool PW = false, int SKIP = 0>
__global__ __launch_bounds__(N / 16 * 64) void dwpw3_kernel(ConvParams P, int R, const _Float16* __restrict__ wh,
                                                           const _Float16* __restrict__ wl, int cin_pad,
                                                           const float* __restrict__ dww,
                                                           const float* __restrict__ dwb) {
  constexpr int NC = N / 32;
  constexpr int KS = N / 16;
  constexpr int AB = KS * 4096;
  constexpr int NBUF = MLIC_D3_NBUF;
  constexpr int AIMG0 = 0, CTR0 = NBUF * AB, BIAS0 = CTR0 + 2 * NBUF * 4;
  constexpr int SKW0 = BIAS0 + N * 4;
  constexpr int LDS = SKW0 + (SKIP ? (SKIP + 1) * N * 4 : 0);
  static_assert(LDS <= 160 * 1024, "dwpw3: LDS");
  static_assert(!SKIP || (PW && MODE == 2 && RES), "dwpw3: the computed residual is the pointwise GDN's");
  static_assert(MLIC_D3_ASYNC || NBUF == 2, "dwpw3: the barrier form alternates two A images");
  __shared__ __attribute__((aligned(16))) char sm[LDS];
  float* sbias = reinterpret_cast<float*>(sm + BIAS0);
  uint32_t* filled = reinterpret_cast<uint32_t*>(sm + CTR0);
  uint32_t* freed = filled + NBUF;
  if (threadIdx.x < 2 * NBUF) filled[threadIdx.x] = 0;

  const int tid = threadIdx.x;
  const int lane = tid & 63;
  const int wave = __builtin_amdgcn_readfirstlane(tid >> 6);
  for (int r = tid; r < N; r += blockDim.x) sbias[r] = P.bias ? P.bias[r] : 0.0f;
  float* sskw = reinterpret_cast<float*>(sm + SKW0);
  if constexpr (SKIP) {
    for (int r = tid; r < SKIP * N; r += blockDim.x) sskw[r] = P.skw[r];
    for (int r = tid; r < N; r += blockDim.x) sskw[SKIP * N + r] = P.skb[r];
  }

  const int H = P.H, W = P.W, HW = H * W;
  const int nseg = (W + D3_TC - 1) / D3_TC;
  const int nys = (H + R - 1) / R;
  const int spi = nseg * nys;
  const int nstrips = spi * P.B;
  const int xcd = (int)blockIdx.x & 7, nslot = (int)gridDim.x >> 3;
  const int t_end = (int)((int64_t)(xcd + 1) * nstrips / 8);
  const int strip0 = (int)((int64_t)xcd * nstrips / 8) + ((int)blockIdx.x >> 3);
  const int nstrip = strip0 < t_end ? (t_end - strip0 + nslot - 1) / nslot : 0;
  if (nstrip == 0) return;
  auto strip_of = [&](int k, int& b, int& ys, int& x0) {
    const int t = strip0 + k * nslot;
    b = t / spi;
    const int r = t - b * spi;
    const int yb = r / nseg;
    b = __builtin_amdgcn_readfirstlane(b);
    ys = __builtin_amdgcn_readfirstlane(yb * R);
    x0 = __builtin_amdgcn_readfirstlane((r - yb * nseg) * D3_TC);
  };

  if (wave >= NC) {
    const int cb = 32 * (wave - NC);
    const uint32_t aw0 = AIMG0 + (uint32_t)(((cb >> 4) * 2 + (lane >> 5)) * 2048) + d3_aoff(lane & 31, 0);
    const uint32_t aw1 = aw0 - d3_aoff(lane & 31, 0) + d3_aoff(lane & 31, 1);
    float pa[32], pb[32];
    float sc[32], se[2];
    __amdgpu_buffer_rsrc_t rs;
    uint32_t cxo = 0, exo = 0;
    const uint32_t hw4 = (uint32_t)HW * 4u;
    auto load_ch = [&](int j, uint32_t& so) {
      asm volatile("" : "+s"(so));
      sc[j] = __builtin_bit_cast(float, __builtin_amdgcn_raw_buffer_load_b32(rs, cxo, so, 0));
      if (!PW && (j & 15) == 15)
        se[j >> 4] = __builtin_bit_cast(float, __builtin_amdgcn_raw_buffer_load_b32(rs, exo, so - 15u * hw4, 0));
      so += hw4;
    };
    auto row_off = [&](int Y) {
      return (uint32_t)__builtin_amdgcn_readfirstlane(Y >= 0 && Y < H ? Y * W * 4 : 0x40000000);
    };
    auto load_row = [&](int Y) {
      uint32_t so = row_off(Y);
#pragma unroll
      for (int j = 0; j < 32; ++j) load_ch(j, so);
    };
    bool pbad = false;
    auto feed = [&](float (&F)[32], float (&A)[32], int t, int ynext) {
      const int buf = t < 0 ? -1 : t % NBUF;
#if MLIC_D3_ASYNC
      if (t >= NBUF) pbad |= !d3_wait_geq(freed + buf, 64u * NC * (uint32_t)(t / NBUF));
#endif
      uint32_t so = row_off(ynext);
      uint32_t toff = (uint32_t)cb;
#if MLIC_D3_TPF
      float tcur[20], tnxt[20];
      auto load_taps = [&](uint32_t t, float (&d)[20]) {
        const float* tp = dww + t * 9;
#pragma unroll
        for (int k = 0; k < 18; ++k) d[k] = tp[k];
        d[18] = dwb[t];
        d[19] = dwb[t + 1];
      };
      asm volatile("" : "+s"(toff));
      load_taps(toff, tcur);
#endif
#pragma unroll
      for (int g = 0; g < 32; g += D3_G) {
        half8 hv8, lv8;
#pragma unroll
        for (int e = 0; e < D3_G; e += 2) {
          if (e % D3_TG == 0) __builtin_amdgcn_sched_barrier(0);
#if MLIC_D3_TPF
          uint32_t tnext = (g + e + 2 < 32) ? toff + 2 : (uint32_t)cb;
          asm volatile("" : "+s"(tnext));
          load_taps(tnext, tnxt);
          const float* tg = tcur;
          const float* bg = tcur + 18;
#else
          asm volatile("" : "+s"(toff));
#if MLIC_D3_FAKETAPS
          static constexpr float fk[20] = {.1f, .2f, .3f, .4f, .5f, .6f, .7f, .8f, .9f, .11f,
                                           .12f, .13f, .14f, .15f, .16f, .17f, .18f, .19f, .21f, .22f};
          const float* tg = fk;
          const float* bg = fk + 18;
#else
          const float* tg = dww + toff * 9;
          const float* bg = dwb + toff;
#endif
#endif
#if MLIC_D3_PPK
          const int j = g + e;
          float Ls[2], Rs[2];
          d3_neighbours_k(j & 15, se[j >> 4], sc[j], Ls[0], Rs[0]);
          d3_neighbours_k((j + 1) & 15, se[(j + 1) >> 4], sc[j + 1], Ls[1], Rs[1]);
          const mlic_float2 L2 = {Ls[0], Ls[1]}, C2 = {sc[j], sc[j + 1]}, R2 = {Rs[0], Rs[1]};
          auto tap = [&](int k) { return mlic_float2{tg[k], tg[9 + k]}; };
          mlic_float2 a2 = {F[j], F[j + 1]}, b2 = {A[j], A[j + 1]}, n2 = {0.0f, 0.0f};
          a2 = __builtin_elementwise_fma(tap(6), L2, a2);
          a2 = __builtin_elementwise_fma(tap(7), C2, a2);
          a2 = __builtin_elementwise_fma(tap(8), R2, a2);
          b2 = __builtin_elementwise_fma(tap(3), L2, b2);
          b2 = __builtin_elementwise_fma(tap(4), C2, b2);
          b2 = __builtin_elementwise_fma(tap(5), R2, b2);
          n2 = __builtin_elementwise_fma(tap(0), L2, n2);
          n2 = __builtin_elementwise_fma(tap(1), C2, n2);
          n2 = __builtin_elementwise_fma(tap(2), R2, n2);
          mlic_float2 o2 = a2 + mlic_float2{bg[0], bg[1]};
          asm volatile("" : "+v"(o2), "+v"(b2), "+v"(n2));
          A[j] = b2[0];
          A[j + 1] = b2[1];
          F[j] = n2[0];
          F[j + 1] = n2[1];
          load_ch(j, so);
          load_ch(j + 1, so);
          const float o[2] = {o2[0], o2[1]};
#else
          float o[2];
#pragma unroll
          for (int f = 0; f < 2; ++f) {
            const int j = g + e + f;
            const float C = sc[j];
            float L, Rr;
            d3_neighbours_k(j & 15, se[j >> 4], C, L, Rr);
            const float* tp = tg + f * 9;
            float a = F[j], bs = A[j], nw = 0.0f;
#if MLIC_D3_ABL & 8
            a = C; bs = L; nw = Rr;
#else
            a = fmaf(tp[6], L, a);
            a = fmaf(tp[7], C, a);
            a = fmaf(tp[8], Rr, a);
            bs = fmaf(tp[3], L, bs);
            bs = fmaf(tp[4], C, bs);
            bs = fmaf(tp[5], Rr, bs);
            nw = fmaf(tp[0], L, nw);
            nw = fmaf(tp[1], C, nw);
            nw = fmaf(tp[2], Rr, nw);
#endif
            o[f] = a + bg[f];
            asm volatile("" : "+v"(o[f]), "+v"(bs), "+v"(nw));
            A[j] = bs;
            F[j] = nw;
#if !(MLIC_D3_ABL & 1)
            load_ch(j, so);
#endif
          }
#endif
          const float2v vv = {o[0], o[1]};
          const half2v hv = __builtin_convertvector(vv, half2v);
          const half2v lv = __builtin_convertvector(vv - __builtin_convertvector(hv, float2v), half2v);
          hv8[e] = hv[0];
          hv8[e + 1] = hv[1];
          lv8[e] = lv[0];
          lv8[e + 1] = lv[1];
          toff += 2;
#if MLIC_D3_TPF
#pragma unroll
          for (int k = 0; k < 20; k += 4)
            asm volatile("" ::"s"(tnxt[k]), "s"(tnxt[k + 1]), "s"(tnxt[k + 2]), "s"(tnxt[k + 3]));
#pragma unroll
          for (int k = 0; k < 20; ++k) tcur[k] = tnxt[k];
#endif
        }
        if (buf >= 0) {
          char* a = sm + buf * AB + (g >> 4) * 4096 + ((g >> 3) & 1 ? aw1 : aw0);
#if MLIC_D3_ABL & 16
          if (hv8[0] == (_Float16)12345.0f)
#endif
          {
            *reinterpret_cast<half8*>(a) = hv8;
            *reinterpret_cast<half8*>(a + 1024) = lv8;
          }
        }
      }
#if MLIC_D3_ASYNC
      if (buf >= 0) d3_signal(filled + buf);
#endif
    };
    auto feed_pw = [&](int t, int ynext) {
      const int buf = t % NBUF;
      uint32_t so = row_off(ynext);
#pragma unroll
      for (int g = 0; g < 32; g += D3_G) {
        __builtin_amdgcn_sched_barrier(0);
        half8 hv8, lv8;
#pragma unroll
        for (int e = 0; e < D3_G; e += 2) {
          float o[2];
#pragma unroll
          for (int f = 0; f < 2; ++f) {
            const int j = g + e + f;
            float v = sc[j];
            if constexpr (MODE == 2 || MODE == 3) v *= v;
            o[f] = v;
            load_ch(j, so);
          }
          const float2v vv = {o[0], o[1]};
          const half2v hv = __builtin_convertvector(vv, half2v);
          const half2v lv = __builtin_convertvector(vv - __builtin_convertvector(hv, float2v), half2v);
          hv8[e] = hv[0];
          hv8[e + 1] = hv[1];
          lv8[e] = lv[0];
          lv8[e + 1] = lv[1];
        }
        char* a = sm + buf * AB + (g >> 4) * 4096 + ((g >> 3) & 1 ? aw1 : aw0);
        *reinterpret_cast<half8*>(a) = hv8;
        *reinterpret_cast<half8*>(a + 1024) = lv8;
      }
    };
    d3_barrier();
    if constexpr (PW) {
      for (int k = 0; k < nstrip; ++k) {
        int b, ys, x0;
        strip_of(k, b, ys, x0);
        rs = d3_rsrc(P.seg[0].p + (int64_t)b * P.seg[0].bs + (int64_t)cb * HW, 32u * hw4);
        const int xl = x0 + lane;
        cxo = xl < W ? (uint32_t)xl * 4u : 0x80000000u;
        load_row(ys);
        for (int u = 0; u <= R; ++u) {
          if (u < R) feed_pw(k * R + u, u + 1 < R ? ys + u + 1 : -1);
          d3_barrier();
        }
      }
      return;
    }
    for (int k = 0; k < nstrip; ++k) {
      int b, ys, x0;
      strip_of(k, b, ys, x0);
      rs = d3_rsrc(P.seg[0].p + (int64_t)b * P.seg[0].bs + (int64_t)cb * HW, 32u * hw4);
      const int xl = x0 + lane;
      cxo = xl < W ? (uint32_t)xl * 4u : 0x80000000u;
      const int xe = lane < 16 ? x0 - 1 : (lane >= 48 ? x0 + D3_TC : -1);
      const int ek = lane < 16 ? lane : 63 - lane;
      exo = xe >= 0 && xe < W ? (uint32_t)ek * hw4 + (uint32_t)xe * 4u : 0x80000000u;
      load_row(ys - 1);
      auto step = [&](int u, float (&F)[32], float (&A)[32]) {
        if (u <= R + 1) feed(F, A, u >= 2 ? k * R + u - 2 : -1, u + 1 <= R + 1 ? ys + u : -1);
#if !MLIC_D3_ASYNC
        if (u >= 2) d3_barrier();
#endif
      };
      for (int u = 0; u < R + 3; u += 2) {
        step(u, pa, pb);
        if (u + 1 < R + 3) step(u + 1, pb, pa);
      }
    }
    range_report(P.rflag, pbad);
    return;
  }

  const int cw = wave;
  const int n = lane & 31, h = lane >> 5;
  half8 bwh[KS], bwl[KS];
  {
    const _Float16* ph = wh + (int64_t)(32 * cw + n) * cin_pad + 8 * h;
    const _Float16* pl = wl + (int64_t)(32 * cw + n) * cin_pad + 8 * h;
#pragma unroll
    for (int k = 0; k < KS; ++k) {
      bwh[k] = *reinterpret_cast<const half8*>(ph + 16 * k);
      bwl[k] = *reinterpret_cast<const half8*>(pl + 16 * k);
    }
  }
  __builtin_amdgcn_s_waitcnt(0);
  d3_barrier();
  const float unscale = ldexpf(1.0f, -P.wexp);
  const uint32_t aoff = d3_aoff(n, h);
  const float* sb = sbias + 32 * cw + 4 * h;
  bool bad = false;
  const uint32_t hw4 = (uint32_t)HW * 4u;
  for (int k = 0; k < nstrip; ++k) {
    int b, ys, x0;
    strip_of(k, b, ys, x0);
    const auto rs_o = d3_rsrc(P.out + (int64_t)b * P.out_bs + (int64_t)(32 * cw) * HW, 32u * hw4);
    const auto rs_r =
        RES && SKIP == 0 ? d3_rsrc(P.res + (int64_t)b * P.res_bs + (int64_t)(32 * cw) * HW, 32u * hw4) : rs_o;
    const uint32_t shw4 = SKIP ? (uint32_t)(P.sk_H * P.sk_W) * 4u : 0u;
    const auto rs_s = SKIP ? d3_rsrc(P.skx + (int64_t)b * P.skx_bs, (uint32_t)SKIP * shw4) : rs_o;
    constexpr bool GDN = MODE == 2 || MODE == 3;
    const auto rs_x = GDN ? d3_rsrc(P.aux + (int64_t)b * P.aux_bs + (int64_t)(32 * cw) * HW, 32u * hw4) : rs_o;
#if !MLIC_D3_ASYNC
    d3_barrier();
#endif
    for (int s = 0; s < R; ++s) {
      const int y = ys + s;
      const int t = k * R + s, buf = t % NBUF;
#if MLIC_D3_ASYNC
      bad |= !d3_wait_geq(filled + buf, 64u * NC * (uint32_t)(t / NBUF + 1));
#endif
#pragma unroll
      for (int bk = 0; bk < 2; ++bk) {
        __builtin_amdgcn_sched_barrier(0);
        const int px = x0 + 32 * bk + n;
        const bool ok = y < H && px < W;
        const uint32_t vo = ok ? (uint32_t)(y * W + px) * 4u + (uint32_t)(4 * h) * hw4 : 0x80000000u;
        float xr[16], xa[16];
        if constexpr (GDN) {
          uint32_t so = 0;
#pragma unroll
          for (int q = 0; q < 16; ++q) {
            asm volatile("" : "+s"(so));
            xa[q] = __builtin_bit_cast(float, __builtin_amdgcn_raw_buffer_load_b32(rs_x, vo, so, 0));
            so += (q & 3) == 3 ? 5u * hw4 : hw4;
          }
        }
        float xs[SKIP ? SKIP : 1];
        if constexpr (SKIP != 0) {
          const uint32_t vs = ok ? (uint32_t)(2 * y * P.sk_W + 2 * px) * 4u : 0x80000000u;
          uint32_t so = 0;
#pragma unroll
          for (int c = 0; c < SKIP; ++c) {
            asm volatile("" : "+s"(so));
            xs[c] = __builtin_bit_cast(float, __builtin_amdgcn_raw_buffer_load_b32(rs_s, vs, so, 0));
            so += shw4;
          }
        } else if constexpr (RES) {
          uint32_t so = 0;
#pragma unroll
          for (int q = 0; q < 16; ++q) {
            asm volatile("" : "+s"(so));
            xr[q] = __builtin_bit_cast(float, __builtin_amdgcn_raw_buffer_load_b32(rs_r, vo, so, 0));
            so += (q & 3) == 3 ? 5u * hw4 : hw4;
          }
        }
        const char* a = sm + AIMG0 + buf * AB + bk * 2048 + aoff;
        floatx16 acc;
        half8 ah = *reinterpret_cast<const half8*>(a);
        half8 al = *reinterpret_cast<const half8*>(a + 1024);
#pragma unroll
        for (int ks = 0; ks < KS; ++ks) {
          half8 nh = ah, nl = al;
          if (ks + 1 < KS) {
            nh = *reinterpret_cast<const half8*>(a + (ks + 1) * 4096);
            nl = *reinterpret_cast<const half8*>(a + (ks + 1) * 4096 + 1024);
          }
#if MLIC_D3_ABL & 4
          if (ks == 0) acc = floatx16{};
          acc[ks & 15] += (float)ah[0] + (float)al[1] + (float)bwh[ks][0] + (float)bwl[ks][1];
#else
          acc = __builtin_amdgcn_mfma_f32_32x32x16_f16(bwl[ks], ah, ks == 0 ? floatx16{} : acc, 0, 0, 0);
          acc = __builtin_amdgcn_mfma_f32_32x32x16_f16(bwh[ks], al, acc, 0, 0, 0);
          acc = __builtin_amdgcn_mfma_f32_32x32x16_f16(bwh[ks], ah, acc, 0, 0, 0);
#endif
          ah = nh;
          al = nl;
        }
        uint32_t so = 0;
#pragma unroll
        for (int g = 0; g < 4; ++g) {
          const float4 b4 = *reinterpret_cast<const float4*>(sb + 8 * g);
          const float bq[4] = {b4.x, b4.y, b4.z, b4.w};
          if constexpr (GDN) {
            if constexpr (SKIP != 0) {
              const float* sw = sskw + 32 * cw + 4 * h + 8 * g;
              const float4 kb = *reinterpret_cast<const float4*>(sw + SKIP * N);
              mlic_float2 s01 = {0.0f, 0.0f}, s23 = {0.0f, 0.0f};
#pragma unroll
              for (int c = 0; c < SKIP; ++c) {
                const float4 w4 = *reinterpret_cast<const float4*>(sw + c * N);
                const mlic_float2 x2 = {xs[c], xs[c]};
                s01 = __builtin_elementwise_fma(x2, mlic_float2{w4.x, w4.y}, s01);
                s23 = __builtin_elementwise_fma(x2, mlic_float2{w4.z, w4.w}, s23);
              }
              s01 = s01 + mlic_float2{kb.x, kb.y};
              s23 = s23 + mlic_float2{kb.z, kb.w};
              xr[4 * g] = s01[0];
              xr[4 * g + 1] = s01[1];
              xr[4 * g + 2] = s23[0];
              xr[4 * g + 3] = s23[1];
            }
#pragma unroll
            for (int e = 0; e < 4; ++e) {
              const int q = 4 * g + e;
              asm volatile("" : "+s"(so));
              float tv = __builtin_fmaf(acc[q], unscale, bq[e]);
              bad |= ok && !(__builtin_fabsf(tv) <= 3.4e38f);
              tv = gdn_apply(xa[q], tv, MODE == 3);
              if constexpr (RES) tv = tv + xr[q];
              __builtin_amdgcn_raw_buffer_store_b32(__builtin_bit_cast(uint32_t, tv), rs_o, vo, so, 0);
              so += hw4;
            }
          } else {
#if MLIC_D3_PK
#pragma unroll
          for (int e = 0; e < 4; e += 2) {
            const int q = 4 * g + e;
            mlic_float2 t2 = __builtin_elementwise_fma(mlic_float2{acc[q], acc[q + 1]}, mlic_float2{unscale, unscale},
                                                       mlic_float2{bq[e], bq[e + 1]});
            if constexpr (MODE == 1) t2 = gelu_erf2(t2);
            if constexpr (RES) t2 = t2 + mlic_float2{xr[q], xr[q + 1]};
#pragma unroll
            for (int f = 0; f < 2; ++f) {
              asm volatile("" : "+s"(so));
              const float tv = t2[f];
              bad |= ok && !(__builtin_fabsf(tv) <= 3.4e38f);
#if MLIC_D3_ABL & 2
              if (tv == 12345.0f)
#endif
              __builtin_amdgcn_raw_buffer_store_b32(__builtin_bit_cast(uint32_t, tv), rs_o, vo, so, 0);
              so += hw4;
            }
          }
#else
#pragma unroll
          for (int e = 0; e < 4; ++e) {
            const int q = 4 * g + e;
            asm volatile("" : "+s"(so));
            float tv = __builtin_fmaf(acc[q], unscale, bq[e]);
            if constexpr (MODE == 1) tv = gelu_erf(tv);
            if constexpr (RES) tv = tv + xr[q];
            bad |= ok && !(__builtin_fabsf(tv) <= 3.4e38f);
            __builtin_amdgcn_raw_buffer_store_b32(__builtin_bit_cast(uint32_t, tv), rs_o, vo, so, 0);
            so += hw4;
          }
#endif
          }
          so += 4u * hw4;
        }
      }
#if MLIC_D3_ASYNC
      d3_signal(freed + buf);
#else
      d3_barrier();
#endif
    }
  }
  range_report(P.rflag, bad);
}

static int d3_num_cus() { return device_cu_count(); }

static int d3_rows(int B, int H, int W) {
  const int64_t ncu = d3_num_cus(), nseg = (W + D3_TC - 1) / D3_TC;
  int best = std::min(H, 32);
  int64_t best_cost = INT64_MAX;
  for (int R = std::min(H, 34); R >= std::min(H, 8); --R) {
    const int64_t strips = (int64_t)B * nseg * ((H + R - 1) / R);
    const int64_t cost = (strips + ncu - 1) / ncu * (R + 3);
    if (cost < best_cost) {
      best_cost = cost;
      best = R;
    }
  }
  return best;
}

bool dwpw3_shape_ok(const ConvParams& P, int cin_pad) {
  if (P.K != 1 || P.stride != 1 || P.pad != 0 || P.nseg != 1 || P.seg[0].C != P.Cin || cin_pad < P.Cin) return false;
  if (P.Cin != P.Cout || (P.Cin != 96 && P.Cin != 128 && P.Cin != 160 && P.Cin != 192)) return false;
  const int e = P.epi & ~EPI_RES;
  if (e != EPI_NONE && e != EPI_GELU) return false;
  if (P.Ho != P.H || P.Wo != P.W || P.out_cs != (int64_t)P.H * P.W) return false;
  if ((int64_t)P.Cin * P.H * P.W * 4 >= (1ll << 31)) return false;
  return true;
}
static bool d3_args_ok(const float* dww, const float* dwb) { return dww && dwb; }

template <int N, int M, bool RS>
static void launch_dwpw3(const ConvParams& P, const _Float16* wh, const _Float16* wl, int cin_pad, const float* dww,
                         const float* dwb, hipStream_t st) {
  const int R = d3_rows(P.B, P.H, P.W);
  const int64_t want = (int64_t)((P.W + D3_TC - 1) / D3_TC) * ((P.H + R - 1) / R) * P.B;
  const int64_t g = std::min<int64_t>(want, (int64_t)d3_num_cus());
  const dim3 grid((unsigned)((g + 7) / 8 * 8));
  hipLaunchKernelGGL((dwpw3_kernel<N, M, RS>), grid, dim3(N / 16 * 64), 0, st, P, R, wh, wl, cin_pad, dww, dwb);
  HIP_OK(hipGetLastError());
}

void dwpw3_forward(const ConvParams& P, const _Float16* wh, const _Float16* wl, int cin_pad, const float* dww,
                   const float* dwb, hipStream_t st) {
  MLIC_CHECK(dwpw3_shape_ok(P, cin_pad) && d3_args_ok(dww, dwb), "dwpw3: unsupported shape");
  const int mode = (P.epi & EPI_GELU) ? 1 : 0, res = (P.epi & EPI_RES) ? 1 : 0;
#define D3_RUN(NN)                                                                               \
  if (P.Cin == NN) {                                                                             \
    if (mode == 0 && !res) return launch_dwpw3<NN, 0, false>(P, wh, wl, cin_pad, dww, dwb, st); \
    if (mode == 0 && res) return launch_dwpw3<NN, 0, true>(P, wh, wl, cin_pad, dww, dwb, st);   \
    if (mode == 1 && !res) return launch_dwpw3<NN, 1, false>(P, wh, wl, cin_pad, dww, dwb, st); \
    return launch_dwpw3<NN, 1, true>(P, wh, wl, cin_pad, dww, dwb, st);                          \
  }
  D3_RUN(192) D3_RUN(160) D3_RUN(128) D3_RUN(96)
#undef D3_RUN
}

bool dwpw2_ok(const ConvParams& P, int cin_pad) {
  const int f = opt(OPT_DWPW2);
  if (f == 2) return dwpw3_shape_ok(P, cin_pad);
  if (f == 1) return dwpw2_lds_ok(P, cin_pad);
  return false;
}
void dwpw2_forward(const ConvParams& P, const _Float16* wh, const _Float16* wl, int cin_pad, const float* dww,
                   const float* dwb, hipStream_t st) {
  if (opt(OPT_DWPW2) == 2) return dwpw3_forward(P, wh, wl, cin_pad, dww, dwb, st);
  dwpw2_lds_forward(P, wh, wl, cin_pad, dww, dwb, st);
}

static int pw3_mode(const ConvParams& P) {
  const int e = P.epi & ~EPI_RES;
  if (e == EPI_NONE) return 0;
  if (e == EPI_GELU) return 1;
  if (e == (EPI_GDN | EPI_SQUARE_IN)) return 2;
  if (e == (EPI_IGDN | EPI_SQUARE_IN)) return 3;
  return -1;
}
bool pw3_ok(const ConvParams& P, int cin_pad) {
  const int mode = pw3_mode(P), setting = opt(OPT_PW3);
  if (setting == 0 || mode < 0 || (mode >= 2 && !P.aux)) return false;
  if (setting == 1 && (int64_t)P.H * P.W < 262144) return false;
  if (P.K != 1 || P.stride != 1 || P.pad != 0 || P.nseg != 1 || P.seg[0].C != P.Cin || cin_pad < P.Cin) return false;
  if (P.Cin != P.Cout || (P.Cin != 96 && P.Cin != 128 && P.Cin != 160 && P.Cin != 192)) return false;
  if (P.Ho != P.H || P.Wo != P.W || P.out_cs != (int64_t)P.H * P.W) return false;
  if ((int64_t)P.Cin * P.H * P.W * 4 >= (1ll << 31)) return false;
  if (P.skx) {
    if (mode != 2 || (P.epi & EPI_RES) || P.sk_cin != 3 || !P.skw || !P.skb) return false;
    if (P.H != (P.sk_H - 1) / 2 + 1 || P.W != (P.sk_W - 1) / 2 + 1) return false;
    if ((int64_t)P.sk_cin * P.sk_H * P.sk_W * 4 >= (1ll << 31)) return false;
  }
  return true;
}
template <int N, int M, bool RS, int SK = 0>
static void launch_pw3(const ConvParams& P, const _Float16* wh, const _Float16* wl, int cin_pad, hipStream_t st) {
  const int R = d3_rows(P.B, P.H, P.W);
  const int64_t want = (int64_t)((P.W + D3_TC - 1) / D3_TC) * ((P.H + R - 1) / R) * P.B;
  const int64_t g = std::min<int64_t>(want, (int64_t)d3_num_cus());
  const dim3 grid((unsigned)((g + 7) / 8 * 8));
  hipLaunchKernelGGL((dwpw3_kernel<N, M, RS, true, SK>), grid, dim3(N / 16 * 64), 0, st, P, R, wh, wl, cin_pad,
                     (const float*)nullptr, (const float*)nullptr);
  HIP_OK(hipGetLastError());
}
void pw3_forward(const ConvParams& P, const _Float16* wh, const _Float16* wl, int cin_pad, hipStream_t st) {
  MLIC_CHECK(pw3_ok(P, cin_pad), "pw3: unsupported shape");
  const int mode = pw3_mode(P), res = (P.epi & EPI_RES) ? 1 : 0;
#define P3_RUN(NN)                                                                \
  if (P.Cin == NN) {                                                              \
    if (P.skx) return launch_pw3<NN, 2, true, 3>(P, wh, wl, cin_pad, st);           \
    if (mode == 0 && !res) return launch_pw3<NN, 0, false>(P, wh, wl, cin_pad, st); \
    if (mode == 0 && res) return launch_pw3<NN, 0, true>(P, wh, wl, cin_pad, st);   \
    if (mode == 1 && !res) return launch_pw3<NN, 1, false>(P, wh, wl, cin_pad, st); \
    if (mode == 1 && res) return launch_pw3<NN, 1, true>(P, wh, wl, cin_pad, st);   \
    if (mode == 2 && !res) return launch_pw3<NN, 2, false>(P, wh, wl, cin_pad, st); \
    if (mode == 2 && res) return launch_pw3<NN, 2, true>(P, wh, wl, cin_pad, st);   \
    if (mode == 3 && !res) return launch_pw3<NN, 3, false>(P, wh, wl, cin_pad, st); \
    return launch_pw3<NN, 3, true>(P, wh, wl, cin_pad, st);                          \
  }
  P3_RUN(192) P3_RUN(160) P3_RUN(128) P3_RUN(96)
#undef P3_RUN
}

}
```

### mlic_amd/csrc/model.cpp

```cpp
#include "model.h"


#include <algorithm>
#include <cmath>
#include <cstdio>
#include <cstring>
#include <thread>

namespace mlic {

static bool gs_subpel(const std::string& name, const ConvW& w) {
  return name.rfind("g_s.", 0) == 0 && w.K == 3 && w.wh != nullptr;
}

Cfg config_for(const std::string& name) {
  Cfg c;
  c.name = name;
  if (name == "MLICPP_L" || name == "MLICPP_L_VBR") { c.N = 192; c.M = 320; c.S = 10; }
  else if (name == "MLICPP_S" || name == "MLICPP_S_VBR") { c.N = 96; c.M = 160; c.S = 5; }
  else if (name == "MLICPP_M") { c.N = 160; c.M = 256; c.S = 8; }
  else if (name == "MLICPP_S2") { c.N = 128; c.M = 128; c.S = 2; }
  else if (name == "MLICPP_M_SMALL_DEC" || name == "MLICPP_M_SMALL_DEC_VBR") { c.N = 192; c.M = 320; c.S = 10; c.sd = true; }
  else throw Error("mlic: unknown model name " + name);
  c.vbr = name.size() > 4 && name.substr(name.size() - 4) == "_VBR";
// ... 428 lines not shown
    lanes_.push_back(std::move(l));
  }
  return *lanes_[i];
}

void Model::set_lanes(int n) {
  MLIC_CHECK(n >= 1 && n <= 16, "lanes must be in [1, 16]");
  nlanes_ = n;
}

void Model::set_profiling(bool on) {
  prof_ = on;
  for (auto& l : lanes_) l->prof = on;
}

size_t Model::arena_bytes() const {
  size_t s = 0;
  for (auto& l : lanes_) s += l->arena.capacity();
  return s;
}

const ConvW& Model::cw(const std::string& k) const {
  auto it = convs_.find(k);
  if (it == convs_.end()) throw Error("mlic: missing conv weight " + k);
  return it->second;
}
const DwW& Model::dww(const std::string& k) const {
  auto it = dws_.find(k);
  if (it == dws_.end()) throw Error("mlic: missing depthwise weight " + k);
  return it->second;
}
const float* Model::rw(const std::string& k) const {
  auto it = raw_.find(k);
  if (it == raw_.end()) throw Error("mlic: missing tensor " + k);
  return it->second;
}

View Model::alloc(int C, int H, int W) {
  View v;
  v.p = L().arena.alloc((int64_t)L().B * C * H * W);
  v.C = C;
  v.H = H;
  v.W = W;
  v.bs = (int64_t)C * H * W;
  return v;
}

void Model::conv(const std::vector<View>& ins, const ConvW& w, int stride, int pad, const View& out, int epi,
                 const View* aux, const View* res) {
  const ConvParams P = conv_params(ins, w, stride, pad, out, epi, aux, res);
  run_conv(P, w, nullptr);
}

void Model::conv_pair(const std::vector<View>& ins, const ConvW& w1, const View& out1, int epi1, const ConvW& w2,
                      const View& out2, int epi2) {
  const ConvParams P1 = conv_params(ins, w1, 1, w1.K / 2, out1, epi1, nullptr, nullptr);
  const ConvParams P2 = conv_params(ins, w2, 1, w2.K / 2, out2, epi2, nullptr, nullptr);
  const ConvWeights c1{w1.w, w1.wh, w1.wl, w1.cin_pad, w1.wx4, w1.wexp}, c2{w2.w, w2.wh, w2.wl, w2.cin_pad, w2.wx4, w2.wexp};
  if (conv_select(P1, c1, prec()) != CONV_X4 || conv_select(P2, c2, prec()) != CONV_X4 ||
      w1.cin_pad != w2.cin_pad || w1.K != w2.K) {
    run_conv(P1, w1, nullptr);
    run_conv(P2, w2, nullptr);
    return;
  }
  const bool hi = gs_fp16_ && w1.wx4h && w2.wx4h;
  const size_t m = L().arena.mark();
  _Float16* act = reinterpret_cast<_Float16*>(L().arena.alloc((2 * x4_act_halves(P1, w1.cin_pad, hi) + 3) / 4));
  timed(PCAT_ELEM, 0.0, (hi ? 6.0 : 8.0) * L().B * P1.Cin * P1.H * P1.W,
        [&] { x4_pack_act(P1, w1.cin_pad, act, L().st, hi); }, w1.name + ".__x4_pack");
  run_conv(P1, w1, act, hi);
  run_conv(P2, w2, act, hi);
  L().arena.release(m);
}

void Model::run_conv(const ConvParams& P, const ConvW& w, const _Float16* packed, bool hi, bool split) {
  const ConvWeights cw{w.w, w.wh, w.wl, w.cin_pad, w.wx4, w.wexp};
  const int impl = packed ? (hi ? CONV_X4H : CONV_X4) : conv_select(P, cw, prec());
  const double outn = (double)P.B * w.Cout * P.Ho * P.Wo;
  const double flops = 2.0 * outn * P.Cin * w.K * w.K;
  const double bytes = 4.0 * ((double)P.B * P.Cin * P.H * P.W + (double)w.Cout * P.Cin * w.K * w.K +
                              outn * (1 + (P.aux ? 1 : 0) + (P.res ? 1 : 0)));
  std::string tag;
  if (L().prof) {
    char sh[96];
    std::snprintf(sh, sizeof sh, " [%d>%d k%d s%d e%x n%d]", P.Cin, P.Cout, P.K, P.stride, P.epi, P.nseg);
    tag = w.name + sh;
  }
  if (packed) {
    const int64_t pb = split ? x4_part_bytes(P, w.cin_pad, hi) : 0;
    const size_t m = L().arena.mark();
    float* part = pb > 0 ? L().arena.alloc((pb + 3) / 4) : nullptr;
    timed(conv_prof_cat(impl, P), flops, bytes,
          [&] { conv_x4_forward(P, packed, hi ? w.wx4h : w.wx4, w.cin_pad, L().st, part, hi); }, tag);
    L().arena.release(m);
    return;
  }
  const int64_t wsb = conv_ws_bytes(impl, P, cw);
  const size_t m = L().arena.mark();
  void* ws = wsb > 0 ? static_cast<void*>(L().arena.alloc((wsb + 3) / 4)) : nullptr;
  timed(conv_prof_cat(impl, P), flops, bytes, [&] { conv_run(impl, P, cw, L().st, ws); }, tag);
  L().arena.release(m);
}

ConvParams Model::conv_params(const std::vector<View>& ins, const ConvW& w, int stride, int pad, const View& out,
                              int epi, const View* aux, const View* res) {
  ConvParams P{};
  MLIC_CHECK(!ins.empty() && (int)ins.size() <= MAXSEG, "conv inputs");
  P.nseg = (int)ins.size();
  int cin = 0;
  for (int s = 0; s < P.nseg; ++s) {
    MLIC_CHECK(ins[s].H == ins[0].H && ins[s].W == ins[0].W, "concat inputs must share H, W");
    P.seg[s] = {ins[s].p, ins[s].C, ins[s].bs};
    cin += ins[s].C;
  }
  MLIC_CHECK(cin == w.Cin, "conv Cin mismatch");
  P.Cin = cin;
  P.H = ins[0].H;
  P.W = ins[0].W;
  P.Cout = w.Cout;
  P.K = w.K;
  P.stride = stride;
  P.pad = pad;
  P.Ho = (P.H + 2 * pad - w.K) / stride + 1;
  P.Wo = (P.W + 2 * pad - w.K) / stride + 1;
  P.wpk = w.w;
  P.wexp = w.wexp;
  P.rflag = L().rflag;
  P.bias = w.b;
  P.epi = epi;
  if (epi & EPI_SHUFFLE) {
    MLIC_CHECK(out.C * 4 == w.Cout && out.H == 2 * P.Ho && out.W == 2 * P.Wo, "shuffle output shape");
  } else {
    MLIC_CHECK(out.C == w.Cout && out.H == P.Ho && out.W == P.Wo, "conv output shape");
  }
  P.out = out.p;
  P.out_bs = out.bs;
  P.out_cs = out.hw();
  if (aux) {
    MLIC_CHECK(aux->C == w.Cout && aux->H == P.Ho && aux->W == P.Wo, "aux shape");
    P.aux = aux->p;
    P.aux_bs = aux->bs;
  }
  if (res) {
    MLIC_CHECK(res->C == out.C && res->H == out.H && res->W == out.W, "residual shape");
    P.res = res->p;
    P.res_bs = res->bs;
    P.epi |= EPI_RES;
  }
  P.B = L().B;
  return P;
}

DwParams Model::dw_params(const std::vector<View>& ins, const DwW& w, int stride, const View& out, bool gelu,
                          int ckbd) {
  DwParams P{};
  P.nseg = (int)ins.size();
  int c = 0;
  for (int s = 0; s < P.nseg; ++s) {
    P.seg[s] = {ins[s].p, ins[s].C, ins[s].bs};
    c += ins[s].C;
  }
  MLIC_CHECK(c == w.C && out.C == w.C, "depthwise channels");
  P.C = c;
  P.H = ins[0].H;
  P.W = ins[0].W;
  P.stride = stride;
  P.Ho = (P.H - 1) / stride + 1;
  P.Wo = (P.W - 1) / stride + 1;
  MLIC_CHECK(out.H == P.Ho && out.W * (ckbd ? 2 : 1) == P.Wo, "depthwise output shape");
  P.w = w.w;
  P.bias = w.b;
  P.out = out.p;
  P.out_bs = out.bs;
  P.gelu = gelu ? 1 : 0;
  P.B = L().B;
  P.ckbd = ckbd;
  return P;
}

void Model::dw(const std::vector<View>& ins, const DwW& w, int stride, const View& out, bool gelu, int ckbd) {
  const DwParams P = dw_params(ins, w, stride, out, gelu, ckbd);
  const double outn = (double)L().B * P.C * out.H * out.W;
  timed(PCAT_DW, 18.0 * outn, 4.0 * ((double)L().B * P.C * P.H * P.W + outn), [&] { dw3x3(P, L().st); }, w.name);
}

bool Model::dw_pw_half(const std::vector<View>& ins, const DwW& d, bool gelu, const ConvW& w, int epi, int mask_epi,
                       const View& out, const View* res, int ckbd, bool fusable) {
  const int H = ins[0].H, W = ins[0].W;
  if (W % 2 != 0 || !w.wh) return false;
  const View geo{nullptr, d.C, H, W, (int64_t)d.C * H * W};
  const ConvParams PF = conv_params({geo}, w, 1, 0, out, epi | mask_epi, nullptr, res);
  const ConvWeights cwt{w.w, w.wh, w.wl, w.cin_pad, w.wx4, w.wexp};
  if (fusable && dwpw_on() && ins.size() == 1 && dwpw_ok(PF, w.cin_pad) && dwpw_grid_ok(PF)) return false;
  if (conv_select(PF, cwt, prec()) != CONV_PW || pw3_ok(PF, w.cin_pad)) return false;
  const size_t m = L().arena.mark();
  const View sq = alloc(d.C, H, W / 2);
  const View og{out.p, out.C, H, W / 2, out.bs};
  View rg;
  if (res) rg = View{res->p, res->C, H, W / 2, res->bs};
  ConvParams PX = conv_params({sq}, w, 1, 0, og, epi, nullptr, res ? &rg : nullptr);
  PX.out_cs = out.hw();
  PX.scatter = ckbd;
  const bool ok = dw_half_ok(dw_params(ins, d, 1, sq, gelu, ckbd)) && pw_resident_ok(PX, w.cin_pad);
  if (ok) {
    dw(ins, d, 1, sq, gelu, ckbd);
    run_conv(PX, w, nullptr);
  }
  L().arena.release(m);
  return ok;
}

void Model::run_chain(const ChainW& c, const std::vector<View>& ins, const View& out, const View* res,
                      const View* aux, int H, int W, int ckbd, bool sq_in) {
  ChainParams P{};
  MLIC_CHECK((int)ins.size() <= MAXSEG && (!ins.empty() || aux), "chain inputs");
  if (!ins.empty()) {
    H = ins[0].H;
    W = ins[0].W;
  }
  P.nseg = (int)ins.size();
  int cin = 0;
  for (int s = 0; s < P.nseg; ++s) {
    MLIC_CHECK(ins[s].H == H && ins[s].W == W, "chain inputs must share H, W");
    P.seg[s] = {ins[s].p, ins[s].C, ins[s].bs};
    cin += ins[s].C;
  }
  MLIC_CHECK(cin == c.cin0, "chain Cin mismatch");
  MLIC_CHECK(!sq_in || (ckbd && !aux), "chain: squeezed inputs need a checkerboard half");
  if (sq_in) W *= 2;
  MLIC_CHECK(out.C == c.cout[c.nl - 1] && out.H == H && out.W == W, "chain output shape");
  if (aux) {
    MLIC_CHECK(aux->C == c.cout[0] && aux->H == H && aux->W == W, "chain aux shape");
    P.aux = aux->p;
    P.aux_bs = aux->bs;
  }
  P.cin0 = cin;
  P.HW = H * W;
  P.W = W;
  P.ckbd = ckbd;
  P.sq_in = sq_in ? 1 : 0;
  P.B = L().B;
  for (int l = 0; l < 4; ++l) {
    P.bias[l] = c.bias[l];
    P.wexp[l] = c.wexp[l];
  }
  P.wimg = c.wimg;
  P.rflag = L().rflag;
  P.out = out.p;
  P.out_bs = out.bs;
  if (res) {
    MLIC_CHECK(res->C == out.C && res->H == out.H && res->W * (sq_in ? 2 : 1) == out.W, "chain residual shape");
    P.res = res->p;
    P.res_bs = res->bs;
  }
  double mac = (double)c.cin0 * c.cout[0];
  for (int l = 1; l < c.nl; ++l) mac += (double)c.cout[l - 1] * c.cout[l];
  const double pix = (double)P.B * (ckbd ? P.HW / 2 : P.HW);
  const double bytes = 4.0 * (pix * (cin + out.C * (res ? 2 : 1) + (aux ? c.cout[0] : 0)) + mac);
  timed(PCAT_CHAIN, 2.0 * mac * pix, bytes, [&] { chain_forward(P, c.nl, c.cout, L().st); }, c.name);
}

View Model::conv3x3(const std::vector<View>& ins, const std::string& p, int stride, bool dwsep, int epi,
                    const View* res, const View* out_opt) {
  const int H = ins[0].H, W = ins[0].W;
  const int Ho = (H - 1) / stride + 1, Wo = (W - 1) / stride + 1;
  if (!dwsep) {
    const ConvW& w = cw(p);
    View out = out_opt ? *out_opt : alloc(w.Cout, Ho, Wo);
    conv(ins, w, stride, 1, out, epi, nullptr, res);
    return out;
  }
  const DwW& d = dww(p + ".depth_conv");
  const ConvW& w = cw(p + ".point_conv");
  View out = out_opt ? *out_opt : alloc(w.Cout, Ho, Wo);
  if (stride == 1 && dwpw_on() && w.wh && ins.size() == 1) {
    ConvParams P = conv_params(ins, w, 1, 0, out, epi, nullptr, res);
    if (dwpw_ok(P, w.cin_pad) && dwpw_grid_ok(P)) {
      const double pix = (double)P.B * H * W;
      const double flops = 2.0 * pix * P.Cin * (9 + w.Cout);
      const double bytes = 4.0 * (pix * (P.Cin + w.Cout * (res ? 2 : 1)) + (double)w.Cout * P.Cin + 10.0 * P.Cin);
      timed(PCAT_DWPW, flops, bytes, [&] { dwpw_forward(P, w.wh, w.wl, w.cin_pad, d.w, d.b, L().st); }, w.name);
      return out;
    }
  }
  const size_t m = L().arena.mark();
  View t = alloc(d.C, Ho, Wo);
  dw(ins, d, stride, t, false);
  conv({t}, w, 1, 0, out, epi, nullptr, res);
  L().arena.release(m);
  return out;
}

View Model::conv1x1(const View& in, const std::string& p, int stride, int epi, const View* res) {
  const ConvW& w = cw(p);
  View out = alloc(w.Cout, (in.H - 1) / stride + 1, (in.W - 1) / stride + 1);
  conv({in}, w, stride, 0, out, epi, nullptr, res);
  return out;
}

void Model::gdn(const View& x, const std::string& p, bool inverse, const View& out, const View* res) {
  conv({x}, cw(p + ".__gdn"), 1, 0, out, EPI_SQUARE_IN | (inverse ? EPI_IGDN : EPI_GDN), &x, res);
}

View Model::rbws(const View& x, const std::string& p, bool dwsep) {
  const int Ho = (x.H - 1) / 2 + 1, Wo = (x.W - 1) / 2 + 1;
  const ConvW& sk = cw(p + ".skip");
  View out = alloc(sk.Cout, Ho, Wo);
  const size_t m = L().arena.mark();
  View t1 = conv3x3({x}, p + ".conv1", 2, dwsep, EPI_GELU);
  View t2 = conv3x3({t1}, p + ".conv2", 1, dwsep, EPI_NONE);
  const ConvW& gw = cw(p + ".gdn.__gdn");
  ConvParams PG = conv_params({t2}, gw, 1, 0, out, EPI_SQUARE_IN | EPI_GDN, &t2, nullptr);
  PG.skx = x.p;
  PG.skx_bs = x.bs;
  PG.sk_cin = sk.Cin;
  PG.sk_H = x.H;
  PG.sk_W = x.W;
  PG.skw = sk.w;
  PG.skb = sk.b;
  const ConvWeights gwt{gw.w, gw.wh, gw.wl, gw.cin_pad, gw.wx4, gw.wexp};
  if (opt(OPT_GDN_SKIP) && sk.K == 1 && sk.Cin <= 4 && x.C == sk.Cin && sk.Cout == gw.Cout && gw.wh &&
      conv_select(PG, gwt, prec()) == CONV_PW && pw3_ok(PG, gw.cin_pad)) {
    run_conv(PG, gw, nullptr);
  } else {
    View s = alloc(sk.Cout, Ho, Wo);
    conv({x}, sk, 2, 0, s, EPI_NONE);
    gdn(t2, p + ".gdn", false, out, &s);
  }
  L().arena.release(m);
  return out;
}

View Model::rb(const View& x, const std::string& p, bool dwsep) {
  const bool has_skip = convs_.count(p + ".skip") > 0;
  const int Cout = dwsep ? cw(p + ".conv2.point_conv").Cout : cw(p + ".conv2").Cout;
  View out = alloc(Cout, x.H, x.W);
  const size_t m = L().arena.mark();
  View t1 = conv3x3({x}, p + ".conv1", 1, dwsep, EPI_GELU);
  View id = x;
  if (has_skip) {
    id = alloc(Cout, x.H, x.W);
    conv({x}, cw(p + ".skip"), 1, 0, id, EPI_NONE);
  }
  conv3x3({t1}, p + ".conv2", 1, dwsep, EPI_GELU, &id, &out);
  L().arena.release(m);
  return out;
}

View Model::rbu(const View& x, const std::string& p) {
  const ConvW& a = cw(p + ".subpel_conv.0");
  const ConvW& u = cw(p + ".upsample.0");
  const int C = a.Cout / 4;
  View out = alloc(C, 2 * x.H, 2 * x.W);
  const size_t m = L().arena.mark();
  View ta = alloc(C, 2 * x.H, 2 * x.W);
  View tu = alloc(C, 2 * x.H, 2 * x.W);
  conv_pair({x}, a, ta, EPI_GELU | EPI_SHUFFLE, u, tu, EPI_SHUFFLE);
  View tc = conv3x3({ta}, p + ".conv", 1, true, EPI_NONE);
  gdn(tc, p + ".igdn", true, out, &tu);
  L().arena.release(m);
  return out;
}

View Model::g_a(const View& x) {
  const bool dwsep = !cfg_.sd;
  const std::string g = "g_a.analysis_transform";
  const int M = cfg_.M;
  View y = alloc(M, (x.H + 15) / 16, (x.W + 15) / 16);
  const size_t m = L().arena.mark();
  View a = rbws(x, g + ".0", dwsep);
  View b = rb(a, g + ".1", dwsep);
  View c = rbws(b, g + ".2", dwsep);
  View d = rb(c, g + ".3", dwsep);
  View e = rbws(d, g + ".4", dwsep);
  View f = rb(e, g + ".5", dwsep);
  conv3x3({f}, g + ".6", 2, dwsep, EPI_NONE, nullptr, &y);
  L().arena.release(m);
  return y;
}

View Model::h_a(const View& y) {
  const bool dwsep = !cfg_.sd;
  const std::string h = "h_a.reduction";
  View z = alloc(cfg_.N, (y.H + 3) / 4, (y.W + 3) / 4);
  const size_t m = L().arena.mark();
  View a = conv3x3({y}, h + ".0", 1, dwsep, EPI_GELU);
  View b = conv3x3({a}, h + ".2", 1, dwsep, EPI_GELU);
  View c = conv3x3({b}, h + ".4", 2, dwsep, EPI_GELU);
  View d = conv3x3({c}, h + ".6", 1, dwsep, EPI_GELU);
  conv3x3({d}, h + ".8", 2, dwsep, EPI_NONE, nullptr, &z);
  L().arena.release(m);
  return z;
}

View Model::h_s(const View& z) {
  const std::string h = "h_s.increase";
  const int hM = cfg_.hM();
  View out = alloc(2 * hM, 4 * z.H, 4 * z.W);
  const size_t m = L().arena.mark();
  View a = conv3x3({z}, h + ".0", 1, true, EPI_GELU);
  View b = alloc(hM, 2 * z.H, 2 * z.W);
  conv({a}, cw(h + ".2.0"), 1, 1, b, EPI_GELU | EPI_SHUFFLE);
  View c = conv3x3({b}, h + ".4", 1, true, EPI_GELU);
  View d = alloc(hM * 3 / 2, 4 * z.H, 4 * z.W);
  conv({c}, cw(h + ".6.0"), 1, 1, d, EPI_GELU | EPI_SHUFFLE);
  conv3x3({d}, h + ".8", 1, true, EPI_NONE, nullptr, &out);
  L().arena.release(m);
  return out;
}

void Model::g_s(const View& yh, const View& out) {
  const std::string g = "g_s.synthesis_transform";
  const size_t m = L().arena.mark();
  View a = rb(yh, g + ".0", true);
  View b = rbu(a, g + ".1");
  View c = rb(b, g + ".2", true);
  View d = rbu(c, g + ".3");
  View e = rb(d, g + ".4", true);
  View f = rbu(e, g + ".5");
  View h = rb(f, g + ".6", true);
  auto tp = convs_.find(g + ".7.0.__taps");
  const ConvW& w7 = cw(g + ".7.0");
  if (tp != convs_.end() && taps_on()) {
    const size_t m2 = L().arena.mark();
    View part = alloc(tp->second.Cout, h.H, h.W);
    conv({h}, tp->second, 1, 0, part, EPI_NONE);
    const double pix = (double)L().B * h.H * h.W;
    timed(PCAT_CONV_NARROW, pix * 9 * 12, 4.0 * pix * (9 * 12 + 12), [&] {
      taps_gather(part.p, part.bs, w7.b, out.p, out.bs, h.H, h.W, L().B, L().st);
    }, g + ".7.0.__gather");
    L().arena.release(m2);
  } else {
    conv({h}, w7, 1, 1, out, EPI_SHUFFLE);
  }
  L().arena.release(m);
}

View Model::local_context(const View& x, int i, bool half) {
  const std::string p = "local_context." + std::to_string(i);
  const int C = x.C, H = x.H, W = x.W;
  View out = alloc(2 * C, H, W);
  const size_t m = L().arena.mark();
  const bool packed = opt(OPT_LA_PACKED) && prec() == PREC_F16X3_V2 && C == 32 && convs_.count(p + ".fusion.__x4perm");
  auto cit = chains_.find(p + ".mlp");
  half = half && packed && W % 2 == 0 && chain_on() && cit != chains_.end() && (H * W) % 8 == 0;
  const int Wq = half ? W / 2 : W;
  View n1 = alloc(C, H, W);
  const double pix = (double)L().B * H * W;
  timed(PCAT_ELEM, 8.0 * pix * C, 8.0 * pix * C, [&] {
    ln_channels(x.p, x.bs, n1.p, n1.bs, rw(p + ".norm1.weight"), rw(p + ".norm1.bias"), C, H * W, L().B, L().st);
  }, p + ".norm1");
  View qkv = conv1x1(n1, p + ".qkv_proj", 1, EPI_NONE);
  View f = alloc(2 * C, H, Wq);
  if (packed) {
    const ConvW& fw = cw(p + ".fusion.__x4perm");
    const int npos = (H * Wq + 31) / 32 * 32;
    _Float16* tp = reinterpret_cast<_Float16*>(L().arena.alloc((int64_t)L().B * 25 * npos * 32));
    LocalAttnParams A{};
    A.qkv = qkv.p;
    A.qkv_bs = qkv.bs;
    A.rel_table = rw(p + ".relative_position_table");
    A.rel_index = rel_index_;
    A.scale = (float)std::pow((double)(C / 2), -0.5);
    A.C = C;
    A.H = H;
    A.W = W;
    A.B = L().B;
    A.ckbd = half ? 2 : 0;
    const double fl = (half ? 0.5 : 1.0) * pix * 2.0 * 2 * 25 * 25 * (C / 2) * 2;
    timed(PCAT_LOCAL, fl, 4.0 * pix * (3 * C + (half ? 0.5 : 1.0) * 25 * C), [&] { local_attn_packed(A, tp, npos, L().st); },
          p + ".attn");
    const View tv{nullptr, 25 * C, H, Wq, (int64_t)25 * C * H * Wq};
    run_conv(conv_params({tv}, fw, 1, 0, f, EPI_NONE, nullptr, nullptr), fw, tp);
  } else {
  View t = alloc(25 * C, H, W);
  {
    LocalAttnParams A{};
    A.qkv = qkv.p;
    A.qkv_bs = qkv.bs;
    A.out = t.p;
    A.out_bs = t.bs;
    A.rel_table = rw(p + ".relative_position_table");
    A.rel_index = rel_index_;
    A.scale = (float)std::pow((double)(C / 2), -0.5);
    A.C = C;
    A.H = H;
    A.W = W;
    A.B = L().B;
    const double fl = pix * 2.0 * 2 * 25 * 25 * (C / 2) * 2;
    timed(PCAT_LOCAL, fl, 4.0 * pix * (3 * C + 25 * C), [&] { local_attn(A, L().st); }, p + ".attn");
  }
  conv({t}, cw(p + ".fusion"), 1, 0, f, EPI_NONE);
  }
  View pj = conv1x1(f, p + ".proj", 1, EPI_NONE);
  View n2 = alloc(2 * C, H, Wq);
  const double pq = (double)L().B * H * Wq;
  timed(PCAT_ELEM, 16.0 * pq * C, 16.0 * pq * C, [&] {
    ln_channels(pj.p, pj.bs, n2.p, n2.bs, rw(p + ".norm2.weight"), rw(p + ".norm2.bias"), 2 * C, H * Wq, L().B, L().st);
  }, p + ".norm2");
  auto ch = cit;
  if (half) {
    run_chain(ch->second, {n2}, out, &pj, nullptr, 0, 0, 2, true);
  } else if (chain_on() && ch != chains_.end() && (H * W) % 4 == 0) {
    run_chain(ch->second, {n2}, out, &pj);
  } else {
    View h1 = conv1x1(n2, p + ".mlp.fc1", 1, EPI_GELU);
    conv({h1}, cw(p + ".mlp.fc2"), 1, 0, out, EPI_NONE, nullptr, &pj);
  }
  L().arena.release(m);
  return out;
}

View Model::channel_context(const View& x, int i) {
  const std::string p = "channel_context." + std::to_string(i) + ".fushion";
  const bool dwsep = !cfg_.sd;
  const int Cout = dwsep ? cw(p + ".4.point_conv").Cout : cw(p + ".4").Cout;
  View out = alloc(Cout, x.H, x.W);
  const size_t m = L().arena.mark();
  View a = conv3x3({x}, p + ".0", 1, dwsep, EPI_GELU);
  View b = conv3x3({a}, p + ".2", 1, dwsep, EPI_GELU);
  conv3x3({b}, p + ".4", 1, dwsep, EPI_NONE, nullptr, &out);
  L().arena.release(m);
  return out;
}

View Model::qkv_branch(const View& x, const std::string& p) {
  const DwW& d = dww(p + ".1");
  View out = alloc(d.C, x.H, x.W);
  const size_t m = L().arena.mark();
  View t = conv1x1(x, p + ".0", 1, EPI_NONE);
  dw({t}, d, 1, out, false);
  L().arena.release(m);
  return out;
}

View Model::inter_context(const View& x, int i) {
  const std::string p = "global_inter_context." + std::to_string(i);
  const int D = x.C, H = x.H, W = x.W, HW = H * W;
  const int heads = D / 32, hd = 32;
  const ConvW& sk = cw(p + ".skip");
  View out = alloc(sk.Cout, H, W);
  const size_t m = L().arena.mark();
  View q = qkv_branch(x, p + ".queries");
  View k = qkv_branch(x, p + ".keys");
  View v = qkv_branch(x, p + ".values");
  const ConvW& rp = cw(p + ".reprojection");
  View a = alloc(rp.Cout, H, W);
  linatt_reproject(k, v, q, heads, hd, 0, 0, rp, a, p + ".attn");
  View m1 = conv1x1(a, p + ".mlp.0", 1, EPI_GELU);
  View m2 = alloc(m1.C, H, W);
  dw({m1}, dww(p + ".mlp.2"), 1, m2, true);
  View s = conv1x1(a, p + ".skip", 1, EPI_NONE);
  conv({m2}, cw(p + ".mlp.4"), 1, 0, out, EPI_NONE, nullptr, &s);
  L().arena.release(m);
  return out;
}

void Model::linatt_reproject(const View& k, const View& v, const View& q, int heads, int hd, int kmask, int qmask,
                             const ConvW& rp, const View& a, const std::string& tag) {
  const int H = q.H, W = q.W, HW = H * W, D = heads * hd, B = L().B;
  const int nsplit = ctx_splits(HW);
  const size_t m = L().arena.mark();
  float* part = L().arena.alloc(linear_attention_part_floats(heads, hd, B, nsplit));
  float* ctx = L().arena.alloc((int64_t)B * heads * hd * hd);
  const double fl = (double)B * HW * D * hd * 4.0, by = 4.0 * B * HW * D * 4.0;
  const View geo{nullptr, D, H, W, (int64_t)D * HW};
  const ConvParams P = conv_params({geo}, rp, 1, 2, a, EPI_NONE, nullptr, nullptr);
  const ConvWeights cwt{rp.w, rp.wh, rp.wl, rp.cin_pad, rp.wx4, rp.wexp};
  if (opt(OPT_LINATT_FUSED) && rp.cin_pad == D && D % 32 == 0 && conv_select(P, cwt, prec()) == CONV_X4) {
    timed(PCAT_LINATT, fl * 0.5, 4.0 * B * HW * D * 2.0, [&] {
      linear_attention_ctx(k.p, k.bs, v.p, v.bs, part, ctx, heads, hd, H, W, B, nsplit, kmask, L().st);
    }, tag);
    _Float16* act = reinterpret_cast<_Float16*>(L().arena.alloc((2 * x4_act_halves(P, rp.cin_pad) + 3) / 4));
    timed(PCAT_LINATT, fl * 0.5, 4.0 * B * HW * D * 2.0, [&] {
      linatt_pack(q.p, q.bs, ctx, heads, hd, qmask, P, act, L().st);
    }, tag + ".pack");
    run_conv(P, rp, act, false, true);
  } else {
    View att = alloc(D, H, W);
    timed(PCAT_LINATT, fl, by, [&] {
      linear_attention(k.p, k.bs, v.p, v.bs, q.p, q.bs, att.p, att.bs, part, ctx, heads, hd, H, W, B, nsplit, kmask, qmask,
                       L().st);
    }, tag);
    conv({att}, rp, 1, 2, a, EPI_NONE);
  }
  L().arena.release(m);
}

View Model::intra_context(const View& x1, const View& x2, int i, bool half) {
  const std::string p = "global_intra_context." + std::to_string(i);
  const int D = x1.C, H = x1.H, W = x1.W, HW = H * W;
  const int heads = 2, hd = D / 2;
  const bool on = opt(OPT_INTRA_HALF) != 0;
  View out = alloc(2 * D, H, W);
  const size_t m = L().arena.mark();
  auto masked_branch = [&](const std::string& bp, int parity, View& o) {
    const ConvW& w = cw(bp + ".0");
    const DwW& d = dww(bp + ".1");
    const View geo{nullptr, w.Cout, H, W, (int64_t)w.Cout * HW};
    const ConvParams P0 = conv_params({x1}, w, 1, 0, geo, EPI_NONE, nullptr, nullptr);
    const ConvWeights cwt{w.w, w.wh, w.wl, w.cin_pad, w.wx4, w.wexp};
    ConvParams PX = P0;
    PX.in_mask = parity;
    if (!on || !w.wh || conv_select(P0, cwt, prec()) != CONV_PW || pw3_ok(P0, w.cin_pad) ||
        !pw_resident_ok(PX, w.cin_pad))
      return false;
    o = alloc(d.C, H, W);
    const size_t m3 = L().arena.mark();
    const View t = alloc(w.Cout, H, W);
    PX.out = t.p;
    PX.out_bs = t.bs;
    run_conv(PX, w, nullptr);
    dw({t}, d, 1, o, false);
// ... 832 lines not shown
```

### mlic_amd/csrc/model.h

```cpp
#pragma once
#include <atomic>
#include <chrono>
#include <map>
#include <memory>
#include <cstring>
#include <string>
#include <vector>

#include "common.h"
#include "kernels.h"
#include "pool.h"
#include "rans.h"

namespace mlic {

struct Cfg {
  std::string name;
  int N = 0, M = 0, S = 0, C = 0, win = 5;
  bool sd = false, vbr = false;
  int hM() const { return sd ? M / 4 : M; }
  int gN() const { return sd ? N / 4 : N; }
};
Cfg config_for(const std::string& name);

struct ConvW {
  float* w = nullptr;
  const float* b = nullptr;
  int Cin = 0, Cout = 0, K = 0;
  _Float16* wh = nullptr;
  _Float16* wl = nullptr;
  int cin_pad = 0;
  _Float16* wx4 = nullptr;
  _Float16* wx4h = nullptr;
  int wexp = 0;
  std::string name;
};

struct ChainW {
  _Float16* wimg = nullptr;
  int nl = 0, cin0 = 0;
  int cout[4] = {0, 0, 0, 0};
  const float* bias[4] = {nullptr, nullptr, nullptr, nullptr};
  int wexp[4] = {0, 0, 0, 0};
  std::string name;
};

enum Precision : int { PREC_F32 = 0, PREC_F16X3 = 1, PREC_F16X3_V2 = 2 };
struct DwW {
  const float* w = nullptr;
  const float* b = nullptr;
  int C = 0;
  std::string name;
};

class Arena {
 public:
  ~Arena();
  void ensure(size_t bytes);
  float* alloc(int64_t nfloats);
  size_t mark() const { return top_; }
  void release(size_t m) { top_ = m; }
  void begin(bool dry) { dry_ = dry; top_ = 0; peak_ = 0; }
  size_t peak() const { return peak_; }
  size_t capacity() const { return cap_; }
  void poison_on(hipStream_t st) { poison_st_ = st; poison_ = true; }
  void poison_off() { poison_ = false; }

 private:
  char* base_ = nullptr;
  size_t cap_ = 0, top_ = 0, peak_ = 0;
  bool dry_ = false;
  bool poison_ = false;
  hipStream_t poison_st_ = nullptr;
};

struct ProfStat {
  int64_t launches = 0;
  double ms = 0, flops = 0, bytes = 0;
};

struct CoderView {
  const int32_t* sym = nullptr;
  const int16_t* sym16 = nullptr;
  const uint8_t* idx = nullptr;
  int64_t n_per = 0, stride = 0;
  int nph = 0;
  int64_t size() const { return n_per * nph; }
  void gather(int32_t* s, int32_t* i) const {
    for (int k = 0; k < nph; ++k) {
      for (int64_t j = 0; j < n_per; ++j) {
        if (s) s[k * n_per + j] = sym16 ? (int32_t)sym16[k * stride + j] : sym[k * stride + j];
        if (i) i[k * n_per + j] = (int32_t)idx[k * stride + j];
      }
    }
  }
  template <class E, class T>
  void put_phase(E& e, int k, const T& tables) const {
    if (sym16) e.put_reverse(sym16 + k * stride, idx + k * stride, n_per, tables);
    else e.put_reverse(sym + k * stride, idx + k * stride, n_per, tables);
  }
};

struct CoderBufs {
  int32_t* sym = nullptr;
  int16_t* sym16 = nullptr;
  uint8_t* idx8 = nullptr;
  int* ovf = nullptr;
};

struct Prefix {
  int slices = -1;
  int fill = 0;
  int strings = 1;
};

struct EncodedImage {
  std::string y;
  std::string z;
  CoderView y_in;
  std::vector<int32_t> z_sym;
  double y_bits = 0, z_bits = 0;
};

class PhaseDecoder;

struct HostStats {
  std::atomic<int64_t> enc_ns{0}, dec_ns{0}, wait_ns{0};
  struct Scope {
    std::atomic<int64_t>& acc;
    std::chrono::steady_clock::time_point t0 = std::chrono::steady_clock::now();
    ~Scope() {
      acc += std::chrono::duration_cast<std::chrono::nanoseconds>(std::chrono::steady_clock::now() - t0).count();
    }
  };
};

struct Lane {
  Arena arena;
  hipStream_t st = nullptr;
  bool own_stream = false;
  int B = 0;
  bool dry = false;
  std::vector<float> vbr_host;
  bool vbr_on = false;
  const float* gplane = nullptr;
  std::vector<EncodedImage> enc;
  int32_t* h_sym = nullptr;
  int16_t* h_sym16 = nullptr;
  uint8_t* h_idx8 = nullptr;
  size_t h_cap = 0;
  hipStream_t cst = nullptr;
  hipEvent_t cev = nullptr;
  int32_t* hc_sym = nullptr;
  int16_t* hc_sym16 = nullptr;
  uint8_t* hc_idx8 = nullptr;
  size_t hc_cap = 0;
  bool phase_d2h = false;
  struct ProfRec {
    hipEvent_t a, b;
    int cat;
    double flops, bytes;
    std::string tag;
  };
  bool prof = false;
  int* rflag = nullptr;
  int prec_force = -1;
  std::vector<ProfRec> recs;
  std::vector<hipEvent_t> ev_pool;
  size_t ev_used = 0;
  ~Lane();
};

class Model {
 public:
  Model(const std::string& name, int n, const char* const* names, const float* const* ptrs, const int64_t* shapes,
        const int* ndims, hipStream_t st);
  ~Model();
  const Cfg& cfg() const { return cfg_; }
  HostStats& host_stats() { return hstats_; }
  HostPool& host_pool();

  void forward(const float* x, int B, int H, int W, float* x_hat, float* y_lik, float* z_lik, const float* vbr_scales,
               hipStream_t st, const float* gain_plane = nullptr);
  void compress(const float* x, int B, int H, int W, const float* vbr_scales, hipStream_t st,
                const float* gain_plane = nullptr);
  const EncodedImage& encoded(int b) const { return enc_all_.at(b); }
  void decompress(const uint8_t* const* y, const size_t* ylen, const uint8_t* const* z, const size_t* zlen, int B,
                  int hz, int wz, float* x_hat, const float* vbr_scales, hipStream_t st, bool batch_stream = false,
                  const float* gain_plane = nullptr, const Prefix& prefix = Prefix{});
  std::string batch_stream(int first, int count) const;
  const std::vector<std::string>& layer_streams(int b);
  void set_tables(const CdfTables& gc, const CdfTables& eb) {
    gc_ = gc;
    eb_ = eb;
  }
  size_t arena_bytes() const;
  void set_profiling(bool on);
  void set_lanes(int n);
  void set_precision(int p) { precision_ = p; }
  int precision() const { return precision_; }
  void set_synthesis_precision(int p) { gs_fp16_ = p == 1; }
  int synthesis_precision() const { return gs_fp16_ ? 1 : 0; }
  int lanes() const { return nlanes_; }
  void set_priority_base(int b) { prio_base_ = b; }
  void set_poison(bool on) { poison_ = on; }
  struct Fallbacks {
    std::atomic<int64_t> forward_full{0}, forward_gs{0}, decompress_gs{0};
  };
  Fallbacks& fallbacks() { return fb_; }
  ProfStat profile_read(int cat);
  std::string profile_layers();
  size_t weight_bytes() const { return wbytes_; }
  void run_module(const std::string& which, int idx, const float* in0, const float* in1, int B, int Cin, int H, int W,
                  float* out, hipStream_t st);

 private:
  enum class Mode { Forward, Encode, Decode };
  Cfg cfg_;
  std::map<std::string, ConvW> convs_;
  std::map<std::string, ChainW> chains_;
  std::map<std::string, ChainW> chains_ctx_;
  ConvW hoist_;
  int hoist_rows_ = 0;
  bool hoist_on() const;
  void add_hoist(const std::map<std::string, std::pair<const float*, int>>& ep0, hipStream_t st);
  ConvW make_conv(const float* w_dev, int Cout, int Cin, int K, const std::string& name, hipStream_t st);
  void add_chains(hipStream_t st);
  bool range_hit(Lane& l);
  void range_clear(Lane& l);
  int prec() const { return L().prec_force >= 0 ? L().prec_force : precision_; }
  void run_chain(const ChainW& c, const std::vector<View>& ins, const View& out, const View* res,
                 const View* aux = nullptr, int H = 0, int W = 0, int ckbd = 0, bool sq_in = false);
  bool chain_on() const;
  bool dwpw_on() const;
  std::map<std::string, DwW> dws_;
  std::map<std::string, const float*> raw_;
  std::vector<void*> owned_;
  size_t wbytes_ = 0;
  float* scale_table_ = nullptr;
  int* rel_index_ = nullptr;
  CdfTables gc_, eb_;
  std::vector<EncodedImage> enc_all_;
  std::vector<std::unique_ptr<Lane>> lanes_;
  int nlanes_ = 4;
  int prio_base_ = 0;
  int precision_ = PREC_F16X3_V2;
  bool gs_fp16_ = false;
  HostStats hstats_;
  bool prof_ = false;
  bool poison_ = false;
  Fallbacks fb_;
  void gs_fp32_rerun(Lane& l, const View& yhat, const View& out, int B);
  static thread_local Lane* tl_lane_;
  Lane& L() const { return *tl_lane_; }
  Lane& lane(int i);
  hipEvent_t next_event();
  template <class F>
  void timed(int cat, double flops, double bytes, F&& launch, const std::string& tag = std::string());
  template <class F>
  void over_lanes(int B, hipStream_t caller, F&& fn, int max_lanes = 16);
  void compress_lane(const float* x, int B, int H, int W);
  void decompress_lane(const uint8_t* const* y, const size_t* ylen, const uint8_t* const* z, const size_t* zlen,
                       int B, int hz, int wz, float* x_hat, bool batch_stream, const Prefix& prefix);

  const ConvW& cw(const std::string& k) const;
  const DwW& dww(const std::string& k) const;
  const float* rw(const std::string& k) const;
  bool has(const std::string& k) const { return convs_.count(k) || dws_.count(k) || raw_.count(k); }

  View alloc(int C, int H, int W);
  void conv(const std::vector<View>& ins, const ConvW& w, int stride, int pad, const View& out, int epi,
            const View* aux = nullptr, const View* res = nullptr);
  ConvParams conv_params(const std::vector<View>& ins, const ConvW& w, int stride, int pad, const View& out, int epi,
                         const View* aux, const View* res);
  void run_conv(const ConvParams& P, const ConvW& w, const _Float16* packed, bool hi = false, bool split = false);
  void linatt_reproject(const View& k, const View& v, const View& q, int heads, int hd, int kmask, int qmask,
                        const ConvW& rp, const View& a, const std::string& tag);
  void add_fusion_x4(const std::string& base, const float* w_dev, int Cout, hipStream_t st);
  void add_taps(const std::string& base, const float* w_dev, int Cin, hipStream_t st);
  bool taps_on() const;
  void conv_pair(const std::vector<View>& ins, const ConvW& w1, const View& out1, int epi1, const ConvW& w2,
                 const View& out2, int epi2);
  DwParams dw_params(const std::vector<View>& ins, const DwW& w, int stride, const View& out, bool gelu, int ckbd);
  void dw(const std::vector<View>& ins, const DwW& w, int stride, const View& out, bool gelu, int ckbd = 0);
  bool dw_pw_half(const std::vector<View>& ins, const DwW& d, bool gelu, const ConvW& w, int epi, int mask_epi,
                  const View& out, const View* res, int ckbd, bool fusable);
  View conv3x3(const std::vector<View>& ins, const std::string& p, int stride, bool dwsep, int epi,
               const View* res = nullptr, const View* out = nullptr);
  View conv1x1(const View& in, const std::string& p, int stride, int epi, const View* res = nullptr);
  void gdn(const View& x, const std::string& p, bool inverse, const View& out, const View* res);
  View rbws(const View& x, const std::string& p, bool dwsep);
  View rb(const View& x, const std::string& p, bool dwsep);
  View rbu(const View& x, const std::string& p);
  View g_a(const View& x);
  View h_a(const View& y);
  View h_s(const View& z_hat);
  void g_s(const View& y_hat, const View& out);
  View local_context(const View& x, int i, bool half = false);
  bool ep_half_chain(const std::string& kind, int i, int H, int W, bool hoisted) const;
  View channel_context(const View& x, int i);
  View inter_context(const View& x, int i);
  View intra_context(const View& x1, const View& x2, int i, bool half = false);
  View entropy_parameters(const std::vector<View>& ctx, const View* hyper, const std::string& kind, int i,
                          const View* hoisted = nullptr, bool phase_only = false);
  void lrp(const std::vector<View>& ins, const std::string& kind, int i, const View& yh_slice, bool anchor);
  View qkv_branch(const View& x, const std::string& p);
  void slice_loop(Mode mode, const View& hyper, const View* y, const View& yhat, float* y_lik, const CoderBufs* cb,
                  class PhaseDecoder* dec, int n_dec = -1, int fill = 0);
  void eb(const View& z, const View& z_hat, float* z_lik, int32_t* z_sym);

  template <class F>
  void planned(int B, hipStream_t st, F&& body);
  void ensure_host(size_t n);
  void ensure_chost(size_t n);
  static int phase_d2h_mode();
  void set_vbr(const float* scales, int B, const float* gain_plane = nullptr);
  bool enc_plane_ = false;
  std::vector<std::vector<std::string>> layers_;
};

}
```

### mlic_amd/csrc/options.cpp

```cpp
#include "options.h"

#include <atomic>
#include <cstdlib>
#include <cstring>
#include <stdexcept>
#include <string>

namespace mlic {
namespace {

int env_int(const char* e, int d) { return e ? std::atoi(e) : d; }
int raw(int v, const char* e, int d) { return v >= 0 ? v : env_int(e, d); }
int flag(int v, const char* e, int d) { return v >= 0 ? v != 0 : env_int(e, d) != 0; }
int lead0(int, const char* e, int) { return !(e && e[0] == '0'); }
int is1(int, const char* e, int d) { return env_int(e, d) == 1; }
int str(int, const char* e, int) { return e != nullptr; }
int halo(int v, const char* e, int d) { return v >= 0 ? (v == 0 ? 0 : 2) : env_int(e, d); }
int nj(int v, const char* e, int d) { return (v > 0 ? v : env_int(e, d)) == 2 ? 2 : 1; }
int narrow(int v, const char*, int d) { return v <= 0 || v > d ? d : v; }

struct Row {
  const char* name;
  const char* env;
  int dflt;
  int (*rule)(int v, const char* e, int d);
};
const Row kRows[] = {
    {"x4_halo", "MLIC_X4_HALO", 1, halo},
    {"x4_splitk", "MLIC_X4_SPLITK", 0, flag},
    {"linatt_fused", "MLIC_LINATT_FUSED", 1, flag},
    {"dw_strip", "MLIC_DW_STRIP", 1, flag},
    {"ep_half", "MLIC_EP_HALF", 1, flag},
    {"chain_nj", "MLIC_CHAIN_NJ", 1, nj},
    {"dwpw2", "MLIC_DWPW2", 2, raw},
    {"pw3", "MLIC_PW3", 1, raw},
    {"narrow_limit", nullptr, 32767, narrow},
    {"image_io_path", nullptr, -1, raw},
    {"lrp_half", "MLIC_LRP_HALF", 0, flag},
    {"intra_half", "MLIC_INTRA_HALF", 0, raw},
    {"gdn_skip", "MLIC_GDN_SKIP", 1, flag},
    {nullptr, "MLIC_X4", 1, flag},           {nullptr, "MLIC_X4_K", 0, str},
    {nullptr, "MLIC_X4_BM_FOR", 0, str},     {nullptr, "MLIC_X4_BM96", 1, lead0},
    {nullptr, "MLIC_X4_BM224", 1, lead0},    {nullptr, "MLIC_X4_RS", 1, flag},
    {nullptr, "MLIC_X4_DIRECT", 1, flag},    {nullptr, "MLIC_X4_ABL", 0, raw},
    {nullptr, "MLIC_V2_WIDE", 1, flag},      {nullptr, "MLIC_LOCAL_ATTN_VALU", 0, flag},
    {nullptr, "MLIC_TAPS", 1, flag},         {nullptr, "MLIC_HOIST", -1, raw},
    {nullptr, "MLIC_DWPW", 1, flag},         {nullptr, "MLIC_CHAIN", 1, flag},
    {nullptr, "MLIC_LA_PACKED", 1, flag},    {nullptr, "MLIC_LANE_PRIORITY", 1, flag},
    {nullptr, "MLIC_PHASE_D2H", 0, raw},     {nullptr, "MLIC_HOST_THREADS", 0, raw},
    {nullptr, "MLIC_POOL_PRIO", 2, raw},     {nullptr, "MLIC_LANES", 0, raw},
    {nullptr, "MLIC_PRECISION", 0, raw},     {nullptr, "MLIC_SYNTH_FP16", 0, is1},
    {nullptr, "MLIC_POISON", 0, flag},
};
static_assert(sizeof(kRows) / sizeof(kRows[0]) == OPT_COUNT, "one row per Opt");

struct {
  std::atomic<int> v{-1};
} g_set[OPT_SETTABLE];

struct Env {
  bool has[OPT_COUNT];
  std::string text[OPT_COUNT];
  int frozen[OPT_COUNT];
  Env() {
    for (int i = 0; i < OPT_COUNT; ++i) {
      const char* e = kRows[i].env ? std::getenv(kRows[i].env) : nullptr;
      has[i] = e != nullptr;
      if (e) text[i] = e;
      frozen[i] = kRows[i].rule(-1, e, kRows[i].dflt);
    }
  }
  const char* get(int i) const { return has[i] ? text[i].c_str() : nullptr; }
};
const Env& env() {
  static const Env e;
  return e;
}

Opt find(const char* name) {
  for (int i = 0; i < OPT_SETTABLE; ++i)
    if (std::strcmp(name, kRows[i].name) == 0) return (Opt)i;
  throw std::runtime_error(std::string("mlic: unknown kernel option ") + name);
}

}

int opt_live(Opt o) {
  const Env& e = env();
  if (o >= OPT_SETTABLE) return e.frozen[o];
  return kRows[o].rule(g_set[o].v.load(std::memory_order_relaxed), e.get(o), kRows[o].dflt);
}

const char* opt_str(Opt o) { return env().get(o); }

void opt_set(const char* name, int value) {
  const Opt o = find(name);
  if (o == OPT_IMAGE_IO_PATH && (value < -1 || value > 2))
    throw std::runtime_error("mlic: image_io_path must be -1 (by layout), 0, 1 or 2");
  g_set[o].v.store(value, std::memory_order_relaxed);
}

int opt_get(const char* name) { return opt_live(find(name)); }

OptionScope::OptionScope() : owner_(tl_opt_snap == nullptr) {
  if (!owner_) return;
  for (int i = 0; i < OPT_COUNT; ++i) vals_[i] = opt_live((Opt)i);
  tl_opt_snap = vals_;
}

OptionScope::OptionScope(const int* snap) : owner_(tl_opt_snap == nullptr && snap != nullptr) {
  if (owner_) tl_opt_snap = snap;
}

}
```

### mlic_amd/csrc/options.h

```cpp
#pragma once

namespace mlic {

enum Opt : int {
  OPT_X4_HALO, OPT_X4_SPLITK, OPT_LINATT_FUSED, OPT_DW_STRIP, OPT_EP_HALF, OPT_CHAIN_NJ, OPT_DWPW2, OPT_PW3,
  OPT_NARROW_LIMIT, OPT_IMAGE_IO_PATH, OPT_LRP_HALF, OPT_INTRA_HALF, OPT_GDN_SKIP,
  OPT_SETTABLE,
  OPT_X4 = OPT_SETTABLE, OPT_X4_K, OPT_X4_BM_FOR, OPT_X4_BM96, OPT_X4_BM224, OPT_X4_RS, OPT_X4_DIRECT, OPT_X4_ABL,
  OPT_V2_WIDE, OPT_LOCAL_ATTN_VALU, OPT_TAPS, OPT_HOIST, OPT_DWPW, OPT_CHAIN, OPT_LA_PACKED, OPT_LANE_PRIORITY,
  OPT_PHASE_D2H, OPT_HOST_THREADS, OPT_POOL_PRIO, OPT_LANES, OPT_PRECISION, OPT_SYNTH_FP16, OPT_POISON,
  OPT_COUNT
};

int opt_live(Opt o);
const char* opt_str(Opt o);
void opt_set(const char* name, int value);
int opt_get(const char* name);

inline thread_local const int* tl_opt_snap = nullptr;

inline int opt(Opt o) {
  const int* s = tl_opt_snap;
  return s ? s[o] : opt_live(o);
}

class OptionScope {
 public:
  OptionScope();
  explicit OptionScope(const int* snap);
  ~OptionScope() { if (owner_) tl_opt_snap = nullptr; }
  OptionScope(const OptionScope&) = delete;
  OptionScope& operator=(const OptionScope&) = delete;
  static const int* current() { return tl_opt_snap; }

 private:
  int vals_[OPT_COUNT];
  bool owner_;
};

}
```

Baseline: 115.2 images/sec.

## Fuse g_a first block's 3-channel pointwise+GELU into the dwpw3 kernel

For the first residual-with-stride block of the analysis transform, the 3-channel pointwise conv plus GELU that produces the wide intermediate is now computed on the fly inside the depthwise+pointwise kernel from the strided 3-channel depthwise output. This avoids writing and re-reading a full-width intermediate tensor and drops one launch. In exchange the fused kernel does redundant GELU/FMA work per halo column and holds more registers and LDS. The path is gated by a new option that is on by default.

```diff
diff --git a/include/mlic_hip.h b/include/mlic_hip.h
--- a/include/mlic_hip.h
+++ b/include/mlic_hip.h
@@ -98,6 +98,9 @@
                 int stride, int gelu);
 int mlic_dwpw_run(void* stream, const float* x, const float* dww, const float* dwb, const float* w, const float* bias,
                   float* y, int B, int C, int Cout, int H, int W, int epi, const float* res);
+int mlic_dwpw_front_run(void* stream, const float* d, const float* fw, const float* fb, const float* dww,
+                        const float* dwb, const float* w, const float* bias, float* y, int B, int Cf, int C, int H,
+                        int W);
 int mlic_bench_conv(int impl, int B, int Cin, int Cout, int H, int W, int K, int stride, int epi, int iters,
                     double* ms_per, double* tflops);
 int mlic_local_attn_mask(void* stream, float* out, int H, int W);
diff --git a/mlic_amd/_lib.py b/mlic_amd/_lib.py
--- a/mlic_amd/_lib.py
+++ b/mlic_amd/_lib.py
@@ -100,6 +100,7 @@
         "mlic_conv_choice": [i, i, i, i, i, i, i, i, P(i)],
         "mlic_dw_run": [p, p, p, p, p, i, i, i, i, i, i],
         "mlic_dwpw_run": [p, p, p, p, p, p, p, i, i, i, i, i, i, p],
+        "mlic_dwpw_front_run": [p, p, p, p, p, p, p, p, p, i, i, i, i, i],
         "mlic_local_attn_run": [p, i, p, p, p, p, i, i, i, i, f],
         "mlic_local_attn_packed_run": [p, p, p, p, p, i, i, i, f],
         "mlic_local_attn_packed_half_run": [p, p, p, p, p, i, i, i, f, i],
diff --git a/mlic_amd/csrc/capi.cpp b/mlic_amd/csrc/capi.cpp
--- a/mlic_amd/csrc/capi.cpp
+++ b/mlic_amd/csrc/capi.cpp
@@ -694,6 +694,54 @@
   });
 }
 
+int mlic_dwpw_front_run(void* stream, const float* d, const float* fw, const float* fb, const float* dww,
+                        const float* dwb, const float* w, const float* bias, float* y, int B, int Cf, int C, int H,
+                        int W) {
+  return guard([&] {
+    hipStream_t st = (hipStream_t)stream;
+    MLIC_CHECK(d && fw && fb && dww && dwb && w && y && B > 0 && Cf > 0 && C > 0 && H > 0 && W > 0,
+               "dwpw_front: bad arguments");
+    const int cin_pad = (C + 31) / 32 * 32;
+    const int64_t nh = (int64_t)C * cin_pad, HW = (int64_t)H * W;
+    _Float16 *wh = nullptr, *wl = nullptr;
+    float* fwp = nullptr;
+    HIP_OK(hipMallocAsync((void**)&wh, nh * 2, st));
+    HIP_OK(hipMallocAsync((void**)&wl, nh * 2, st));
+    HIP_OK(hipMallocAsync((void**)&fwp, (int64_t)C * Cf * 4, st));
+    pack_conv(fw, fwp, C, Cf, 1, st);
+    const int wexp = split_weights(w, wh, wl, C, C, 1, cin_pad, true, st);
+    ConvParams P{};
+    P.nseg = 1;
+    P.seg[0] = {nullptr, C, C * HW};
+    P.Cin = C; P.H = H; P.W = W; P.Cout = C; P.Ho = H; P.Wo = W; P.K = 1; P.stride = 1; P.pad = 0;
+    P.wexp = wexp; P.bias = bias; P.out = y; P.B = B; P.epi = EPI_NONE;
+    P.out_cs = HW;
+    P.out_bs = C * HW;
+    float* t1 = nullptr;
+    if (opt(OPT_GA_FRONT)) {
+      P.fx = d; P.fx_bs = Cf * HW; P.f_cin = Cf; P.fw = fwp; P.fb = fb;
+    } else {
+      HIP_OK(hipMallocAsync((void**)&t1, (int64_t)B * C * HW * 4, st));
+      ConvParams Q{};
+      Q.nseg = 1;
+      Q.seg[0] = {d, Cf, Cf * HW};
+      Q.Cin = Cf; Q.H = H; Q.W = W; Q.Cout = C; Q.Ho = H; Q.Wo = W; Q.K = 1; Q.stride = 1; Q.pad = 0;
+      Q.wpk = fwp; Q.bias = fb; Q.out = t1; Q.B = B; Q.epi = EPI_GELU;
+      Q.out_cs = HW;
+      Q.out_bs = C * HW;
+      conv_smallcin_forward(Q, st);
+      P.seg[0].p = t1;
+    }
+    MLIC_CHECK(dwpw_ok(P, cin_pad), "dwpw_front: unsupported shape");
+    dwpw_forward(P, wh, wl, cin_pad, dww, dwb, st);
+    if (t1) HIP_OK(hipFreeAsync(t1, st));
+    HIP_OK(hipFreeAsync(fwp, st));
+    HIP_OK(hipFreeAsync(wh, st));
+    HIP_OK(hipFreeAsync(wl, st));
+    HIP_OK(hipStreamSynchronize(st));
+  });
+}
+
 int mlic_local_attn_run(void* stream, int impl, const float* qkv, const float* rel_table, const int32_t* rel_index,
                         float* out, int C, int H, int W, int B, float scale) {
   return guard([&] {
diff --git a/mlic_amd/csrc/common.h b/mlic_amd/csrc/common.h
--- a/mlic_amd/csrc/common.h
+++ b/mlic_amd/csrc/common.h
@@ -88,6 +88,11 @@
   int sk_cin, sk_H, sk_W;
   const float* skw;
   const float* skb;
+  const float* fx;
+  int64_t fx_bs;
+  int f_cin;
+  const float* fw;
+  const float* fb;
 };
 
 __device__ __forceinline__ float softmax_exp(float x) { return __builtin_amdgcn_exp2f(x * 1.44269504088896341f); }
diff --git a/mlic_amd/csrc/conv_dwpw.hip b/mlic_amd/csrc/conv_dwpw.hip
--- a/mlic_amd/csrc/conv_dwpw.hip
+++ b/mlic_amd/csrc/conv_dwpw.hip
@@ -354,6 +354,7 @@
   const int64_t HW = (int64_t)P.H * P.W;
   if ((int64_t)P.Cin * HW * 4 >= (1ll << 31) || (int64_t)P.Cout * HW * 4 >= (1ll << 31)) return false;
   if (dwpw2_ok(P, cin_pad)) return true;
+  if (P.fx) return false;
   const int ct = (P.Cout + 31) / 32, res = (P.epi & EPI_RES) ? 1 : 0;
 #define DR_OK(CIN, CT, M, R) \
   if (P.Cin == CIN && ct == CT && mode == M && res == R) return true;
@@ -374,7 +375,7 @@
 
 void dwpw_forward(const ConvParams& P, const _Float16* wh, const _Float16* wl, int cin_pad, const float* dww,
                   const float* dwb, hipStream_t st) {
-  MLIC_CHECK(dwpw_ok(P, cin_pad) && dww, "dwpw: unsupported shape");
+  MLIC_CHECK(dwpw_ok(P, cin_pad) && dww && (dwb || !P.fx), "dwpw: unsupported shape");
   if (dwb && dwpw2_ok(P, cin_pad)) return dwpw2_forward(P, wh, wl, cin_pad, dww, dwb, st);
   const int ct = (P.Cout + 31) / 32, mode = dw_mode(P), res = (P.epi & EPI_RES) ? 1 : 0;
 #define DR_RUN(CIN, CT, M, R)                                        \
diff --git a/mlic_amd/csrc/conv_dwpw3.hip b/mlic_amd/csrc/conv_dwpw3.hip
--- a/mlic_amd/csrc/conv_dwpw3.hip
+++ b/mlic_amd/csrc/conv_dwpw3.hip
@@ -88,19 +88,22 @@
 }
 }
 
-template <int N, int MODE, bool RES, bool PW = false, int SKIP = 0>
+template <int N, int MODE, bool RES, bool PW = false, int SKIP = 0, int FRONT = 0>
 __global__ __launch_bounds__(N / 16 * 64) void dwpw3_kernel(ConvParams P, int R, const _Float16* __restrict__ wh,
                                                            const _Float16* __restrict__ wl, int cin_pad,
                                                            const float* __restrict__ dww,
-                                                           const float* __restrict__ dwb) {
+                                                           const float* __restrict__ dwb,
+                                                           const float* __restrict__ frw = nullptr,
+                                                           const float* __restrict__ frb = nullptr) {
   constexpr int NC = N / 32;
   constexpr int KS = N / 16;
   constexpr int AB = KS * 4096;
   constexpr int NBUF = MLIC_D3_NBUF;
   constexpr int AIMG0 = 0, CTR0 = NBUF * AB, BIAS0 = CTR0 + 2 * NBUF * 4;
   constexpr int SKW0 = BIAS0 + N * 4;
-  constexpr int LDS = SKW0 + (SKIP ? (SKIP + 1) * N * 4 : 0);
+  constexpr int LDS = SKW0 + (SKIP ? (SKIP + 1) * N * 4 : 0) + (FRONT ? (FRONT + 1) * N * 4 : 0);
   static_assert(LDS <= 160 * 1024, "dwpw3: LDS");
+  static_assert(!FRONT || (!PW && !RES && SKIP == 0), "dwpw3: the computed input is the plain depthwise forms'");
   static_assert(!SKIP || (PW && MODE == 2 && RES), "dwpw3: the computed residual is the pointwise GDN's");
   static_assert(MLIC_D3_ASYNC || NBUF == 2, "dwpw3: the barrier form alternates two A images");
   __shared__ __attribute__((aligned(16))) char sm[LDS];
@@ -117,6 +120,10 @@
   if constexpr (SKIP) {
     for (int r = tid; r < SKIP * N; r += blockDim.x) sskw[r] = P.skw[r];
     for (int r = tid; r < N; r += blockDim.x) sskw[SKIP * N + r] = P.skb[r];
+  }
+  if constexpr (FRONT != 0) {
+    for (int r = tid; r < FRONT * N; r += blockDim.x) sskw[r] = frw[r];
+    for (int r = tid; r < N; r += blockDim.x) sskw[FRONT * N + r] = frb[r];
   }
 
   const int H = P.H, W = P.W, HW = H * W;
@@ -164,13 +171,57 @@
       for (int j = 0; j < 32; ++j) load_ch(j, so);
     };
     bool pbad = false;
-    auto feed = [&](float (&F)[32], float (&A)[32], int t, int ynext) {
+    constexpr int FR = FRONT ? FRONT : 1;
+    float fc[FR], fe[FR], fn[FR], fg[FR], few[2][FR + 1];
+    bool cin = false, ein = false;
+    auto load_front = [&](int Y, float (&dc)[FR], float (&de)[FR]) {
+      uint32_t so = row_off(Y);
+#pragma unroll
+      for (int c = 0; c < FR; ++c) {
+        asm volatile("" : "+s"(so));
+        dc[c] = __builtin_bit_cast(float, __builtin_amdgcn_raw_buffer_load_b32(rs, cxo, so, 0));
+        de[c] = __builtin_bit_cast(float, __builtin_amdgcn_raw_buffer_load_b32(rs, exo, so, 0));
+        so += hw4;
+      }
+    };
+    auto feed = [&](float (&F)[32], float (&A)[32], int t, int ynext, bool rowin) {
       const int buf = t < 0 ? -1 : t % NBUF;
 #if MLIC_D3_ASYNC
       if (t >= NBUF) pbad |= !d3_wait_geq(freed + buf, 64u * NC * (uint32_t)(t / NBUF));
 #endif
       uint32_t so = row_off(ynext);
       uint32_t toff = (uint32_t)cb;
+      const bool cok = cin && rowin;
+      float fv[32];
+      auto front_group = [&](uint32_t t, int j) {
+#pragma unroll
+        for (int q = 0; q < D3_TG; q += 2) {
+          const float* fwp = frw + t + q;
+          const float* fbp = frb + t + q;
+          mlic_float2 v2 = {0.0f, 0.0f};
+#pragma unroll
+          for (int c = 0; c < FR; ++c)
+            v2 = __builtin_elementwise_fma(mlic_float2{fc[c], fc[c]}, mlic_float2{fwp[c * N], fwp[c * N + 1]}, v2);
+          v2 = gelu_erf2(v2 + mlic_float2{fbp[0], fbp[1]});
+          const float c0 = v2[0], c1 = v2[1];
+          fv[j + q] = cok ? c0 : 0.0f;
+          fv[j + q + 1] = cok ? c1 : 0.0f;
+        }
+      };
+      if constexpr (FRONT != 0) {
+        asm volatile("" : "+s"(toff));
+        front_group(toff, 0);
+        load_front(ynext, fn, fg);
+        mlic_float2 v2 = {0.0f, 0.0f};
+#pragma unroll
+        for (int c = 0; c < FRONT; ++c)
+          v2 = __builtin_elementwise_fma(mlic_float2{fe[c], fe[c]}, mlic_float2{few[0][c], few[1][c]}, v2);
+        v2 = gelu_erf2(v2 + mlic_float2{few[0][FRONT], few[1][FRONT]});
+        const float e0 = v2[0], e1 = v2[1];
+        const bool eok = ein && rowin;
+        se[0] = eok ? e0 : 0.0f;
+        se[1] = eok ? e1 : 0.0f;
+      }
 #if MLIC_D3_TPF
       float tcur[20], tnxt[20];
       auto load_taps = [&](uint32_t t, float (&d)[20]) {
@@ -207,12 +258,21 @@
           const float* bg = dwb + toff;
 #endif
 #endif
+          float cv[2];
+          if constexpr (FRONT != 0) {
+            if (e % D3_TG == 0 && g + e + D3_TG < 32) front_group(toff + D3_TG, g + e + D3_TG);
+            cv[0] = fv[g + e];
+            cv[1] = fv[g + e + 1];
+          } else {
+            cv[0] = sc[g + e];
+            cv[1] = sc[g + e + 1];
+          }
 #if MLIC_D3_PPK
           const int j = g + e;
           float Ls[2], Rs[2];
-          d3_neighbours_k(j & 15, se[j >> 4], sc[j], Ls[0], Rs[0]);
-          d3_neighbours_k((j + 1) & 15, se[(j + 1) >> 4], sc[j + 1], Ls[1], Rs[1]);
-          const mlic_float2 L2 = {Ls[0], Ls[1]}, C2 = {sc[j], sc[j + 1]}, R2 = {Rs[0], Rs[1]};
+          d3_neighbours_k(j & 15, se[j >> 4], cv[0], Ls[0], Rs[0]);
+          d3_neighbours_k((j + 1) & 15, se[(j + 1) >> 4], cv[1], Ls[1], Rs[1]);
+          const mlic_float2 L2 = {Ls[0], Ls[1]}, C2 = {cv[0], cv[1]}, R2 = {Rs[0], Rs[1]};
           auto tap = [&](int k) { return mlic_float2{tg[k], tg[9 + k]}; };
           mlic_float2 a2 = {F[j], F[j + 1]}, b2 = {A[j], A[j + 1]}, n2 = {0.0f, 0.0f};
           a2 = __builtin_elementwise_fma(tap(6), L2, a2);
@@ -230,15 +290,17 @@
           A[j + 1] = b2[1];
           F[j] = n2[0];
           F[j + 1] = n2[1];
-          load_ch(j, so);
-          load_ch(j + 1, so);
+          if constexpr (FRONT == 0) {
+            load_ch(j, so);
+            load_ch(j + 1, so);
+          }
           const float o[2] = {o2[0], o2[1]};
 #else
           float o[2];
 #pragma unroll
           for (int f = 0; f < 2; ++f) {
             const int j = g + e + f;
-            const float C = sc[j];
+            const float C = cv[f];
             float L, Rr;
             d3_neighbours_k(j & 15, se[j >> 4], C, L, Rr);
             const float* tp = tg + f * 9;
@@ -261,7 +323,7 @@
             A[j] = bs;
             F[j] = nw;
 #if !(MLIC_D3_ABL & 1)
-            load_ch(j, so);
+            if constexpr (FRONT == 0) load_ch(j, so);
 #endif
           }
 #endif
@@ -292,6 +354,13 @@
           }
         }
       }
+      if constexpr (FRONT != 0) {
+#pragma unroll
+        for (int c = 0; c < FRONT; ++c) {
+          fc[c] = fn[c];
+          fe[c] = fg[c];
+        }
+      }
 #if MLIC_D3_ASYNC
       if (buf >= 0) d3_signal(filled + buf);
 #endif
@@ -328,6 +397,13 @@
       }
     };
     d3_barrier();
+    if constexpr (FRONT != 0) {
+      const int ek = lane < 16 ? lane : (lane >= 48 ? 63 - lane : 0);
+#pragma unroll
+      for (int i = 0; i < 2; ++i)
+#pragma unroll
+        for (int c = 0; c <= FRONT; ++c) few[i][c] = sskw[c * N + cb + 16 * i + ek];
+    }
     if constexpr (PW) {
       for (int k = 0; k < nstrip; ++k) {
         int b, ys, x0;
@@ -346,15 +422,20 @@
     for (int k = 0; k < nstrip; ++k) {
       int b, ys, x0;
       strip_of(k, b, ys, x0);
-      rs = d3_rsrc(P.seg[0].p + (int64_t)b * P.seg[0].bs + (int64_t)cb * HW, 32u * hw4);
+      if constexpr (FRONT != 0) rs = d3_rsrc(P.fx + (int64_t)b * P.fx_bs, (uint32_t)FRONT * hw4);
+      else rs = d3_rsrc(P.seg[0].p + (int64_t)b * P.seg[0].bs + (int64_t)cb * HW, 32u * hw4);
       const int xl = x0 + lane;
       cxo = xl < W ? (uint32_t)xl * 4u : 0x80000000u;
       const int xe = lane < 16 ? x0 - 1 : (lane >= 48 ? x0 + D3_TC : -1);
       const int ek = lane < 16 ? lane : 63 - lane;
-      exo = xe >= 0 && xe < W ? (uint32_t)ek * hw4 + (uint32_t)xe * 4u : 0x80000000u;
-      load_row(ys - 1);
+      exo = xe >= 0 && xe < W ? (uint32_t)(FRONT ? 0 : ek) * hw4 + (uint32_t)xe * 4u : 0x80000000u;
+      cin = xl < W;
+      ein = xe >= 0 && xe < W;
+      if constexpr (FRONT != 0) load_front(ys - 1, fc, fe);
+      else load_row(ys - 1);
       auto step = [&](int u, float (&F)[32], float (&A)[32]) {
-        if (u <= R + 1) feed(F, A, u >= 2 ? k * R + u - 2 : -1, u + 1 <= R + 1 ? ys + u : -1);
+        if (u <= R + 1)
+          feed(F, A, u >= 2 ? k * R + u - 2 : -1, u + 1 <= R + 1 ? ys + u : -1, ys + u - 1 >= 0 && ys + u - 1 < H);
 #if !MLIC_D3_ASYNC
         if (u >= 2) d3_barrier();
 #endif
@@ -568,20 +649,22 @@
   if (P.Cin != P.Cout || (P.Cin != 96 && P.Cin != 128 && P.Cin != 160 && P.Cin != 192)) return false;
   const int e = P.epi & ~EPI_RES;
   if (e != EPI_NONE && e != EPI_GELU) return false;
+  if (P.fx && (P.epi != EPI_NONE || P.f_cin != 3 || !P.fw || !P.fb)) return false;
   if (P.Ho != P.H || P.Wo != P.W || P.out_cs != (int64_t)P.H * P.W) return false;
   if ((int64_t)P.Cin * P.H * P.W * 4 >= (1ll << 31)) return false;
   return true;
 }
 static bool d3_args_ok(const float* dww, const float* dwb) { return dww && dwb; }
 
-template <int N, int M, bool RS>
+template <int N, int M, bool RS, int FR = 0>
 static void launch_dwpw3(const ConvParams& P, const _Float16* wh, const _Float16* wl, int cin_pad, const float* dww,
                          const float* dwb, hipStream_t st) {
   const int R = d3_rows(P.B, P.H, P.W);
   const int64_t want = (int64_t)((P.W + D3_TC - 1) / D3_TC) * ((P.H + R - 1) / R) * P.B;
   const int64_t g = std::min<int64_t>(want, (int64_t)d3_num_cus());
   const dim3 grid((unsigned)((g + 7) / 8 * 8));
-  hipLaunchKernelGGL((dwpw3_kernel<N, M, RS>), grid, dim3(N / 16 * 64), 0, st, P, R, wh, wl, cin_pad, dww, dwb);
+  hipLaunchKernelGGL((dwpw3_kernel<N, M, RS, false, 0, FR>), grid, dim3(N / 16 * 64), 0, st, P, R, wh, wl, cin_pad, dww,
+                     dwb, P.fw, P.fb);
   HIP_OK(hipGetLastError());
 }
 
@@ -591,6 +674,7 @@
   const int mode = (P.epi & EPI_GELU) ? 1 : 0, res = (P.epi & EPI_RES) ? 1 : 0;
 #define D3_RUN(NN)                                                                               \
   if (P.Cin == NN) {                                                                             \
+    if (P.fx) return launch_dwpw3<NN, 0, false, 3>(P, wh, wl, cin_pad, dww, dwb, st);            \
     if (mode == 0 && !res) return launch_dwpw3<NN, 0, false>(P, wh, wl, cin_pad, dww, dwb, st); \
     if (mode == 0 && res) return launch_dwpw3<NN, 0, true>(P, wh, wl, cin_pad, dww, dwb, st);   \
     if (mode == 1 && !res) return launch_dwpw3<NN, 1, false>(P, wh, wl, cin_pad, dww, dwb, st); \
@@ -603,6 +687,7 @@
 bool dwpw2_ok(const ConvParams& P, int cin_pad) {
   const int f = opt(OPT_DWPW2);
   if (f == 2) return dwpw3_shape_ok(P, cin_pad);
+  if (P.fx) return false;
   if (f == 1) return dwpw2_lds_ok(P, cin_pad);
   return false;
 }
@@ -642,7 +727,7 @@
   const int64_t g = std::min<int64_t>(want, (int64_t)d3_num_cus());
   const dim3 grid((unsigned)((g + 7) / 8 * 8));
   hipLaunchKernelGGL((dwpw3_kernel<N, M, RS, true, SK>), grid, dim3(N / 16 * 64), 0, st, P, R, wh, wl, cin_pad,
-                     (const float*)nullptr, (const float*)nullptr);
+                     (const float*)nullptr, (const float*)nullptr, (const float*)nullptr, (const float*)nullptr);
   HIP_OK(hipGetLastError());
 }
 void pw3_forward(const ConvParams& P, const _Float16* wh, const _Float16* wl, int cin_pad, hipStream_t st) {
diff --git a/mlic_amd/csrc/model.cpp b/mlic_amd/csrc/model.cpp
--- a/mlic_amd/csrc/model.cpp
+++ b/mlic_amd/csrc/model.cpp
@@ -754,13 +754,47 @@
   conv({x}, cw(p + ".__gdn"), 1, 0, out, EPI_SQUARE_IN | (inverse ? EPI_IGDN : EPI_GDN), &x, res);
 }
 
+bool Model::rbws_front(const View& x, const std::string& p, bool dwsep, int Ho, int Wo, View& t2) {
+  if (!dwsep || !opt(OPT_GA_FRONT) || !dwpw_on()) return false;
+  const DwW& d1 = dww(p + ".conv1.depth_conv");
+  const ConvW& p1 = cw(p + ".conv1.point_conv");
+  const DwW& d2 = dww(p + ".conv2.depth_conv");
+  const ConvW& p2 = cw(p + ".conv2.point_conv");
+  if (p1.K != 1 || p1.Cin > 4 || x.C != p1.Cin || d1.C != p1.Cin || !p1.b || p1.Cout != p2.Cin || !p2.wh || !d2.b)
+    return false;
+  static const float present = 0.0f;
+  const View geo{nullptr, p2.Cin, Ho, Wo, (int64_t)p2.Cin * Ho * Wo};
+  const View og{nullptr, p2.Cout, Ho, Wo, (int64_t)p2.Cout * Ho * Wo};
+  ConvParams P = conv_params({geo}, p2, 1, 0, og, EPI_NONE, nullptr, nullptr);
+  P.fx = &present;
+  P.f_cin = p1.Cin;
+  P.fw = p1.w;
+  P.fb = p1.b;
+  if (!dwpw_ok(P, p2.cin_pad) || !dwpw_grid_ok(P)) return false;
+  View s = alloc(p1.Cin, Ho, Wo);
+  dw({x}, d1, 2, s, false);
+  t2 = alloc(p2.Cout, Ho, Wo);
+  P.fx = s.p;
+  P.fx_bs = s.bs;
+  P.out = t2.p;
+  P.out_bs = t2.bs;
+  const double pix = (double)P.B * Ho * Wo;
+  const double flops = 2.0 * pix * P.Cin * (p1.Cin + 9 + p2.Cout);
+  const double bytes = 4.0 * (pix * (p1.Cin + p2.Cout) + (double)p2.Cout * P.Cin + (11.0 + p1.Cin) * P.Cin);
+  timed(PCAT_DWPW, flops, bytes, [&] { dwpw_forward(P, p2.wh, p2.wl, p2.cin_pad, d2.w, d2.b, L().st); }, p2.name);
+  return true;
+}
+
 View Model::rbws(const View& x, const std::string& p, bool dwsep) {
   const int Ho = (x.H - 1) / 2 + 1, Wo = (x.W - 1) / 2 + 1;
   const ConvW& sk = cw(p + ".skip");
   View out = alloc(sk.Cout, Ho, Wo);
   const size_t m = L().arena.mark();
-  View t1 = conv3x3({x}, p + ".conv1", 2, dwsep, EPI_GELU);
-  View t2 = conv3x3({t1}, p + ".conv2", 1, dwsep, EPI_NONE);
+  View t2;
+  if (!rbws_front(x, p, dwsep, Ho, Wo, t2)) {
+    View t1 = conv3x3({x}, p + ".conv1", 2, dwsep, EPI_GELU);
+    t2 = conv3x3({t1}, p + ".conv2", 1, dwsep, EPI_NONE);
+  }
   const ConvW& gw = cw(p + ".gdn.__gdn");
   ConvParams PG = conv_params({t2}, gw, 1, 0, out, EPI_SQUARE_IN | EPI_GDN, &t2, nullptr);
   PG.skx = x.p;
diff --git a/mlic_amd/csrc/model.h b/mlic_amd/csrc/model.h
--- a/mlic_amd/csrc/model.h
+++ b/mlic_amd/csrc/model.h
@@ -290,6 +290,7 @@
   View conv1x1(const View& in, const std::string& p, int stride, int epi, const View* res = nullptr);
   void gdn(const View& x, const std::string& p, bool inverse, const View& out, const View* res);
   View rbws(const View& x, const std::string& p, bool dwsep);
+  bool rbws_front(const View& x, const std::string& p, bool dwsep, int Ho, int Wo, View& t2);
   View rb(const View& x, const std::string& p, bool dwsep);
   View rbu(const View& x, const std::string& p);
   View g_a(const View& x);
diff --git a/mlic_amd/csrc/options.cpp b/mlic_amd/csrc/options.cpp
--- a/mlic_amd/csrc/options.cpp
+++ b/mlic_amd/csrc/options.cpp
@@ -39,6 +39,7 @@
     {"lrp_half", "MLIC_LRP_HALF", 0, flag},
     {"intra_half", "MLIC_INTRA_HALF", 0, raw},
     {"gdn_skip", "MLIC_GDN_SKIP", 1, flag},
+    {"ga_front", "MLIC_GA_FRONT", 1, flag},
     {nullptr, "MLIC_X4", 1, flag},           {nullptr, "MLIC_X4_K", 0, str},
     {nullptr, "MLIC_X4_BM_FOR", 0, str},     {nullptr, "MLIC_X4_BM96", 1, lead0},
     {nullptr, "MLIC_X4_BM224", 1, lead0},    {nullptr, "MLIC_X4_RS", 1, flag},
diff --git a/mlic_amd/csrc/options.h b/mlic_amd/csrc/options.h
--- a/mlic_amd/csrc/options.h
+++ b/mlic_amd/csrc/options.h
@@ -5,6 +5,7 @@
 enum Opt : int {
   OPT_X4_HALO, OPT_X4_SPLITK, OPT_LINATT_FUSED, OPT_DW_STRIP, OPT_EP_HALF, OPT_CHAIN_NJ, OPT_DWPW2, OPT_PW3,
   OPT_NARROW_LIMIT, OPT_IMAGE_IO_PATH, OPT_LRP_HALF, OPT_INTRA_HALF, OPT_GDN_SKIP,
+  OPT_GA_FRONT,
   OPT_SETTABLE,
   OPT_X4 = OPT_SETTABLE, OPT_X4_K, OPT_X4_BM_FOR, OPT_X4_BM96, OPT_X4_BM224, OPT_X4_RS, OPT_X4_DIRECT, OPT_X4_ABL,
   OPT_V2_WIDE, OPT_LOCAL_ATTN_VALU, OPT_TAPS, OPT_HOIST, OPT_DWPW, OPT_CHAIN, OPT_LA_PACKED, OPT_LANE_PRIORITY,
```

Result: no change. 116.0 images/sec, median of 3 (+0.7%).
